# Enigmatisms/cuda-pt

Hardware: AMD Instinct MI355X
Metric: Msamples/sec (whole node), 1080p modern-kitchen (higher is better)
Workload: dtype fp32; 1 GPU; model=modern-kitchen-proc, global_batch=32, seq_len=2073600, width=1920, height=1080, renderer=pt, n_prims=131444, parallelism=dp1 (sample-split, RCCL all-reduce)

## Files before the change

csrc/bind.cpp:

```cpp
#include <pybind11/pybind11.h>
#include <pybind11/numpy.h>
#include <pybind11/stl.h>
#include <algorithm>
#include <cstring>
#include <stdexcept>

#include "core/scene_view.h"
#include "core/integrator.h"
#include "cpu/bvh_build.h"
#include "hip/kernels.h"
#include "hip/lds_plan.h"

namespace py = pybind11;
using namespace hippt;

namespace hippt {
void render_cpu(const SceneView& sv, float* accum, float* var,
                int spp0, int nspp, uint32_t seed, int renderer, int n_threads,
                int y0, int y1, const uint8_t* spp_map, float* aux);
void render_lt_cpu(const SceneView& sv, float* accum, int spp0, int nspp, uint32_t seed,
                   int spec_constraint, float caustic_scaling, int n_threads);
}

namespace {

using farr = py::array_t<float, py::array::c_style | py::array::forcecast>;
using iarr = py::array_t<int32_t, py::array::c_style | py::array::forcecast>;
using uarr = py::array_t<uint32_t, py::array::c_style | py::array::forcecast>;

#define HIP_OK(expr)                                                                   \
    do {                                                                               \
        int _e = (expr);                                                               \
        if (_e != 0) throw std::runtime_error(std::string("HIP error ") +              \
                                              std::to_string(_e) + " at " #expr);      \
    } while (0)

Vec3 to_vec3(const std::vector<float>& v) { return {v[0], v[1], v[2]}; }

int super_cell_voxels() {
    static const int SUP = [] {
        const char* e = getenv("HIPPT_SUPER_N");
        int v = e ? atoi(e) : 16;
        return v < 2 ? 2 : (v > 64 ? 64 : v);
    }();
    return SUP;
}

inline void super_splat(std::vector<float>& sup, const MediumParams& m, int SUP,
                        int ix, int iy, int iz, float v) {
    int cx0 = std::max(0, (ix - 1) / SUP), cx1 = std::min(m.sx - 1, (ix + 1) / SUP);
    int cy0 = std::max(0, (iy - 1) / SUP), cy1 = std::min(m.sy - 1, (iy + 1) / SUP);
    int cz0 = std::max(0, (iz - 1) / SUP), cz1 = std::min(m.sz - 1, (iz + 1) / SUP);
    for (int cz = cz0; cz <= cz1; ++cz)
        for (int cy = cy0; cy <= cy1; ++cy)
            for (int cx = cx0; cx <= cx1; ++cx) {
                float& s = sup[(size_t(cz) * m.sy + cy) * m.sx + cx];
                s = fmaxf(s, v);
            }
}

int bvh4_tree_depth(const BVH4Node* nodes, int n) {
    if (n <= 0) return 0;
    std::vector<std::pair<int, int>> stk{{0, 1}};
    int maxd = 1;
    while (!stk.empty()) {
        auto [idx, d] = stk.back();
        stk.pop_back();
        maxd = std::max(maxd, d);
        const BVH4Node& nd = nodes[idx];
        for (int c = 0; c < 4; ++c)
            if (nd.child[c] >= 0 && !(nd.child[c] == 0 && nd.cnt[c] == 0))
                stk.push_back({nd.child[c], d + 1});
    }
    return maxd;
}

static std::vector<uint64_t> host_lds_slots(int lds_n);

struct SceneHolder {
    farr np_prims, np_attrs, np_nodes, np_nodes4, np_nodes8;
    uarr np_prim_obj;
    iarr np_objs;
    std::vector<BsdfParams> bsdfs;
    std::vector<EmitterParams> emitters;
    std::vector<PhaseParams> phases;
    std::vector<MediumParams> media;
    std::vector<farr> media_density, media_temp;
    std::vector<std::vector<float>> media_super;
    std::vector<std::vector<int32_t>> media_bricks;
    std::vector<int> media_nbricks;
    std::vector<farr> tex_data;
    std::vector<TexView> tex_host;
    std::vector<int> emitter_prims;
    std::vector<float> emitter_cdf;
    std::vector<float> env_rows_h, env_cols_h;
    int env_w = 0, env_h = 0;
    std::vector<float> emitter_sel_h;
    Camera cam{};
    MaxDepthParams md{};
    int env_emitter = -1;
    int cam_medium = -1;

    bool has_dev = false;
    int device_id = 0;
    std::vector<void*> dev_bufs;
    std::vector<TexView> tex_dev;
    std::vector<MediumParams> media_dev;
    void* dev_bsdfs = nullptr;
    void* dev_emitters = nullptr;
    void* dev_media = nullptr;

    SceneView host_sv{};
    SceneView dev_sv{};
    WfState* wf = nullptr;

    ~SceneHolder() { release(); }

    void release() {
        if (wf) { wf_destroy(wf); wf = nullptr; }
        for (void* p : dev_bufs) dev_free(p);
        dev_bufs.clear();
        has_dev = false;
    }

    void set_geometry(farr prims, farr attrs, uarr prim_obj, farr nodes, farr nodes4,
                      farr nodes8) {
        if (prims.ndim() != 2 || prims.shape(1) != 12) throw std::runtime_error("prims must be (n,12)");
        if (attrs.ndim() != 2 || attrs.shape(1) != 16) throw std::runtime_error("attrs must be (n,16)");
        if (nodes.ndim() != 2 || nodes.shape(1) != 8) throw std::runtime_error("nodes must be (m,8)");
        if (nodes4.ndim() == 2 && nodes4.shape(0) > 0 && nodes4.shape(1) != 32)
            throw std::runtime_error("nodes4 must be (m,32)");
        np_prims = std::move(prims);
        np_attrs = std::move(attrs);
        np_prim_obj = std::move(prim_obj);
        np_nodes = std::move(nodes);
        np_nodes4 = std::move(nodes4);
        if (nodes8.ndim() == 2 && nodes8.shape(0) > 0 && nodes8.shape(1) != 64)
            throw std::runtime_error("nodes8 must be (m,64)");
        np_nodes8 = std::move(nodes8);
        bvh4_depth = np_nodes4.ndim() == 2 && np_nodes4.shape(0) > 0
            ? bvh4_tree_depth((const BVH4Node*)np_nodes4.data(), (int)np_nodes4.shape(0))
            : 0;
        nodes4q = np_nodes4.ndim() == 2 && np_nodes4.shape(0) > 0
            ? quantize_bvh4((const BVH4Node*)np_nodes4.data(), (int)np_nodes4.shape(0))
            : std::vector<BVH4NodeQ>();
        nodes4t = np_nodes4.ndim() == 2 && np_nodes4.shape(0) > 0
            ? tag_bvh4((const BVH4Node*)np_nodes4.data(), (int)np_nodes4.shape(0))
            : std::vector<BVH4NodeT>();
        const Prim* pr = (const Prim*)np_prims.data();
        const uint32_t* po = np_prim_obj.data();
        int n = (int)np_prims.shape(0);
        AABB sb;
        for (int i = 0; i < n; ++i) {
            if (po[i] & PRIM_SPHERE_BIT) {
                Vec3 c = pr[i].v0.xyz();
                float rad = pr[i].v0.w;
                sb.grow(c - Vec3(rad)); sb.grow(c + Vec3(rad));
            } else {
                Vec3 v0 = pr[i].v0.xyz();
                sb.grow(v0);
                sb.grow(v0 + pr[i].e1.xyz());
                sb.grow(v0 + pr[i].e2.xyz());
            }
        }
        Vec3 c = (sb.lo + sb.hi) * 0.5f;
        float rad = n > 0 ? (sb.hi - sb.lo).length() * 0.5f : 1.f;
        scene_bound = Vec4(c, rad);
        tri_only = 1;
        for (int i = 0; i < n; ++i)
            if (po[i] & PRIM_SPHERE_BIT) { tri_only = 0; break; }
    }

    int bvh4_depth = 0;
    Vec4 scene_bound{0.f, 0.f, 0.f, 1.f};
    int cache_nodes = 0;
    int tri_only = 0;
    std::vector<BVH4NodeQ> nodes4q;
    std::vector<BVH4NodeT> nodes4t;

    void set_cache_level(int level) {
        cache_nodes = level > 0 ? (1 << (level > 12 ? 12 : level)) : 0;
    }

    void set_objects(iarr objs) {
        if (objs.ndim() != 2 || objs.shape(1) != 8) throw std::runtime_error("objs must be (n,8)");
        np_objs = std::move(objs);
    }

    int add_bsdf(int type, std::vector<float> kd, std::vector<float> ks, std::vector<float> kg,
                 float ior, float extra0, float extra1, std::vector<int> tex) {
        BsdfParams b = BsdfParams::make(type);
        b.kd = Vec4(kd[0], kd[1], kd[2], kd.size() > 3 ? kd[3] : 0.f);
        b.ks = Vec4(ks[0], ks[1], ks[2], ks.size() > 3 ? ks[3] : 0.f);
        b.kg = Vec4(kg[0], kg[1], kg[2], kg.size() > 3 ? kg[3] : 0.f);
        b.ior = ior; b.extra0 = extra0; b.extra1 = extra1;
        for (size_t i = 0; i < tex.size() && i < 8; ++i) b.tex[i] = (int16_t)tex[i];
        bsdfs.push_back(b);
        return (int)bsdfs.size() - 1;
    }

    void update_bsdf(int i, int type, std::vector<float> kd, std::vector<float> ks,
                     std::vector<float> kg, float ior, float extra0, float extra1,
                     std::vector<int> tex) {
        if (i < 0 || i >= (int)bsdfs.size()) throw std::runtime_error("bad bsdf index");
        BsdfParams b = BsdfParams::make(type);
        b.kd = Vec4(kd[0], kd[1], kd[2], kd.size() > 3 ? kd[3] : 0.f);
        b.ks = Vec4(ks[0], ks[1], ks[2], ks.size() > 3 ? ks[3] : 0.f);
        b.kg = Vec4(kg[0], kg[1], kg[2], kg.size() > 3 ? kg[3] : 0.f);
        b.ior = ior; b.extra0 = extra0; b.extra1 = extra1;
        for (size_t k = 0; k < tex.size() && k < 8; ++k) b.tex[k] = (int16_t)tex[k];
        bsdfs[i] = b;
        if (has_dev && dev_bsdfs)
            HIP_OK(dev_upload((char*)dev_bsdfs + sizeof(BsdfParams) * i, &bsdfs[i], sizeof(BsdfParams)));
    }

    int add_emitter(int type, std::vector<float> emission, float scale, std::vector<float> aux,
                    int obj_id, int tex_id, int prim_base, int prim_cnt, float inv_area) {
        EmitterParams e{};
        e.emission = Vec4(emission[0], emission[1], emission[2], scale);
        e.aux = Vec4(aux[0], aux[1], aux[2], aux.size() > 3 ? aux[3] : 0.f);
        e.type = type; e.obj_id = obj_id; e.tex_id = tex_id;
        e.prim_base = prim_base; e.prim_cnt = prim_cnt; e.inv_area = inv_area;
        emitters.push_back(e);
        if (type == EM_ENVMAP) env_emitter = (int)emitters.size() - 1;
        return (int)emitters.size() - 1;
    }

    void update_emitter(int i, std::vector<float> emission, float scale, std::vector<float> aux) {
        if (i < 0 || i >= (int)emitters.size()) throw std::runtime_error("bad emitter index");
        emitters[i].emission = Vec4(emission[0], emission[1], emission[2], scale);
        emitters[i].aux = Vec4(aux[0], aux[1], aux[2], aux.size() > 3 ? aux[3] : 0.f);
        if (has_dev && dev_emitters)
            HIP_OK(dev_upload((char*)dev_emitters + sizeof(EmitterParams) * i, &emitters[i],
                              sizeof(EmitterParams)));
    }

    void set_emitter_prims(iarr eprims, farr ecdf) {
        emitter_prims.assign(eprims.data(), eprims.data() + eprims.size());
        emitter_cdf.assign(ecdf.data(), ecdf.data() + ecdf.size());
    }

    void set_emitter_sel(farr cdf) {
        emitter_sel_h.assign(cdf.data(), cdf.data() + cdf.size());
    }

    void set_env_cdf(farr rows, farr cols) {
        if (cols.ndim() != 2) throw std::runtime_error("env cols must be (h,w)");
        env_h = (int)cols.shape(0);
        env_w = (int)cols.shape(1);
        env_rows_h.assign(rows.data(), rows.data() + rows.size());
        env_cols_h.assign(cols.data(), cols.data() + cols.size());
        if ((int)env_rows_h.size() != env_h) throw std::runtime_error("env rows/cols mismatch");
    }

    int add_phase(int type, float g1, float g2, float wmix) {
        phases.push_back({type, g1, g2, wmix});
        return (int)phases.size() - 1;
    }

    int add_medium(int type, std::vector<float> sigma_a, std::vector<float> sigma_s,
                   int phase_id, std::vector<float> grid_lo, std::vector<float> grid_hi,
                   py::object density, py::object temperature,
                   float scale, float emission_scale, float temp_scale) {
        MediumParams m{};
        m.sigma_a = Vec4(sigma_a[0], sigma_a[1], sigma_a[2], 0.f);
        m.sigma_s = Vec4(sigma_s[0], sigma_s[1], sigma_s[2], 0.f);
        m.type = type; m.phase_id = phase_id;
        m.scale = scale; m.emission_scale = emission_scale; m.temp_scale = temp_scale;
        m.density = nullptr; m.temperature = nullptr;
        m.super = nullptr;
        m.nx = m.ny = m.nz = 0;
        m.sx = m.sy = m.sz = 0;
        if (type == MED_GRID) {
            farr d = density.cast<farr>();
            if (d.ndim() != 3) throw std::runtime_error("density must be (nz,ny,nx)");
            media_density.push_back(d);
            m.nz = (int)d.shape(0); m.ny = (int)d.shape(1); m.nx = (int)d.shape(2);
            m.density = media_density.back().data();
            float mx = 0.f; double sum = 0.0;
            const float* dd = m.density;
            size_t n = (size_t)m.nx * m.ny * m.nz;
            for (size_t i = 0; i < n; ++i) { mx = fmaxf(mx, dd[i]); sum += dd[i]; }
            m.majorant = mx * scale;
            m.avg_density = (float)(sum / std::max<size_t>(n, 1)) * scale;
            const int SUP = super_cell_voxels();
            if (getenv("HIPPT_NO_SUPER")) {
                m.sx = m.sy = m.sz = 0;
                m.super = nullptr;
                goto super_done;
            }
            m.sx = (m.nx + SUP - 1) / SUP;
            m.sy = (m.ny + SUP - 1) / SUP;
            m.sz = (m.nz + SUP - 1) / SUP;
            {
            std::vector<float> sup((size_t)m.sx * m.sy * m.sz, 0.f);
            for (int iz = 0; iz < m.nz; ++iz)
                for (int iy = 0; iy < m.ny; ++iy)
                    for (int ix = 0; ix < m.nx; ++ix) {
                        float v = dd[(size_t(iz) * m.ny + iy) * m.nx + ix];
                        if (v <= 0.f) continue;
                        super_splat(sup, m, SUP, ix, iy, iz, v);
                    }
            media_super.push_back(std::move(sup));
            m.super = media_super.back().data();
            }
            super_done:;
            Vec3 lo = to_vec3(grid_lo), hi = to_vec3(grid_hi);
            m.grid_lo = Vec4(lo, 0.f);
            Vec3 ext = hi - lo;
            m.grid_inv_extent = Vec4(1.f / ext.x, 1.f / ext.y, 1.f / ext.z, 0.f);
            if (!temperature.is_none()) {
                farr t = temperature.cast<farr>();
                media_temp.push_back(t);
                m.temperature = media_temp.back().data();
            }
        }
        media.push_back(m);
        media_nbricks.push_back(-1);
        return (int)media.size() - 1;
    }

    int add_medium_sparse(std::vector<float> sigma_a, std::vector<float> sigma_s,
                          int phase_id, std::vector<float> grid_lo, std::vector<float> grid_hi,
                          std::vector<int> shape, iarr coords, farr density,
                          py::object temperature,
                          float scale, float emission_scale, float temp_scale) {
        MediumParams m{};
        m.sigma_a = Vec4(sigma_a[0], sigma_a[1], sigma_a[2], 0.f);
        m.sigma_s = Vec4(sigma_s[0], sigma_s[1], sigma_s[2], 0.f);
        m.type = MED_GRID; m.phase_id = phase_id;
        m.scale = scale; m.emission_scale = emission_scale; m.temp_scale = temp_scale;
        if (shape.size() != 3 || shape[0] <= 0 || shape[1] <= 0 || shape[2] <= 0)
            throw std::runtime_error("sparse grid shape must be three positive dims (nz,ny,nx)");
        m.nz = shape[0]; m.ny = shape[1]; m.nx = shape[2];
        m.bnx = (m.nx + 7) / 8; m.bny = (m.ny + 7) / 8; m.bnz = (m.nz + 7) / 8;
        if (coords.ndim() != 2 || coords.shape(1) != 3)
            throw std::runtime_error("brick coords must be (n,3)");
        const size_t nb = (size_t)coords.shape(0);
        if ((size_t)density.size() != nb * 512)
            throw std::runtime_error("density bricks must hold 512 floats per brick coord");
        farr temp;
        if (!temperature.is_none()) {
            temp = temperature.cast<farr>();
            if ((size_t)temp.size() != nb * 512)
                throw std::runtime_error("temperature bricks must hold 512 floats per brick coord");
        }
        const size_t cells = (size_t)m.bnx * m.bny * m.bnz;
        if (cells > (size_t)INT32_MAX) throw std::runtime_error("brick table too large");
        std::vector<int32_t> table(cells, -1);
        const int32_t* cc = coords.data();
        for (size_t b = 0; b < nb; ++b) {
            int bz = cc[3 * b], by = cc[3 * b + 1], bx = cc[3 * b + 2];
            if (bz < 0 || bz >= m.bnz || by < 0 || by >= m.bny || bx < 0 || bx >= m.bnx)
                throw std::runtime_error("brick coord outside the brick table");
            int32_t& cell = table[(size_t(bz) * m.bny + by) * m.bnx + bx];
            if (cell >= 0) throw std::runtime_error("duplicate brick coord");
            cell = (int32_t)b;
        }
        const float* pool = density.data();
        float mx = 0.f; double sum = 0.0;
        for (size_t i = 0; i < nb * 512; ++i) mx = fmaxf(mx, pool[i]);
        std::vector<int32_t> row;
        for (int bz = 0; bz < m.bnz; ++bz)
            for (int z = 0; z < 8 && bz * 8 + z < m.nz; ++z)
                for (int by = 0; by < m.bny; ++by) {
                    row.clear();
                    const int32_t* trow = &table[(size_t(bz) * m.bny + by) * m.bnx];
                    for (int bx = 0; bx < m.bnx; ++bx)
                        if (trow[bx] >= 0) row.push_back(trow[bx]);
                    if (row.empty()) continue;
                    for (int y = 0; y < 8 && by * 8 + y < m.ny; ++y)
                        for (int32_t b : row) {
                            const float* v = pool + size_t(b) * 512 + (z << 6 | y << 3);
                            for (int x = 0; x < 8; ++x) sum += v[x];
                        }
                }
        const size_t n = (size_t)m.nx * m.ny * m.nz;
        m.majorant = mx * scale;
        m.avg_density = (float)(sum / std::max<size_t>(n, 1)) * scale;
        if (!getenv("HIPPT_NO_SUPER")) {
            const int SUP = super_cell_voxels();
            m.sx = (m.nx + SUP - 1) / SUP;
            m.sy = (m.ny + SUP - 1) / SUP;
            m.sz = (m.nz + SUP - 1) / SUP;
            std::vector<float> sup((size_t)m.sx * m.sy * m.sz, 0.f);
            for (size_t b = 0; b < nb; ++b) {
                int z0 = cc[3 * b] * 8, y0 = cc[3 * b + 1] * 8, x0 = cc[3 * b + 2] * 8;
                const float* v = pool + b * 512;
                for (int z = 0; z < 8 && z0 + z < m.nz; ++z)
                    for (int y = 0; y < 8 && y0 + y < m.ny; ++y)
                        for (int x = 0; x < 8 && x0 + x < m.nx; ++x) {
                            float d = v[z << 6 | y << 3 | x];
                            if (d <= 0.f) continue;
                            super_splat(sup, m, SUP, x0 + x, y0 + y, z0 + z, d);
                        }
            }
            media_super.push_back(std::move(sup));
            m.super = media_super.back().data();
        }
        Vec3 lo = to_vec3(grid_lo), hi = to_vec3(grid_hi);
        m.grid_lo = Vec4(lo, 0.f);
        Vec3 ext = hi - lo;
        m.grid_inv_extent = Vec4(1.f / ext.x, 1.f / ext.y, 1.f / ext.z, 0.f);
        media_bricks.push_back(std::move(table));
        m.bricks = media_bricks.back().data();
        if (nb > 0) {
            media_density.push_back(density);
            m.density = media_density.back().data();
            if (!temperature.is_none()) {
                media_temp.push_back(temp);
                m.temperature = media_temp.back().data();
            }
        }
        media.push_back(m);
        media_nbricks.push_back((int)nb);
        return (int)media.size() - 1;
    }

    py::tuple medium_super(int i) {
        if (i < 0 || i >= (int)media.size()) throw std::runtime_error("bad medium index");
        const MediumParams& m = media[i];
        farr out({(py::ssize_t)(m.super ? m.sz : 0), (py::ssize_t)m.sy, (py::ssize_t)m.sx});
        if (m.super) std::memcpy(out.mutable_data(), m.super, sizeof(float) * out.size());
        return py::make_tuple(out, m.majorant, m.avg_density);
    }

    py::list media_info() {
        py::list out;
        for (size_t i = 0; i < media.size(); ++i) {
            const MediumParams& m = media[i];
            py::dict d;
            size_t vox = (size_t)m.nx * m.ny * m.nz;
            size_t pools = (m.density ? 1 : 0) + (m.temperature ? 1 : 0);
            size_t bytes = 4 * (size_t)m.sx * m.sy * m.sz * (m.super ? 1 : 0);
            if (m.type != MED_GRID) {
                d["layout"] = "homogeneous";
                d["shape"] = py::none();
                d["n_bricks"] = 0;
                d["occupancy"] = 0.0;
            } else if (m.bricks) {
                size_t cells = (size_t)m.bnx * m.bny * m.bnz;
                size_t nb = (size_t)media_nbricks[i];
                d["layout"] = "bricks";
                d["shape"] = py::make_tuple(m.nz, m.ny, m.nx);
                d["n_bricks"] = nb;
                d["occupancy"] = (double)nb / (double)cells;
                bytes += 4 * cells + 2048 * nb * pools;
            } else {
                d["layout"] = "dense";
                d["shape"] = py::make_tuple(m.nz, m.ny, m.nx);
                d["n_bricks"] = 0;
                d["occupancy"] = 1.0;
                bytes += 4 * vox * pools;
            }
            d["bytes_host"] = bytes;
            d["bytes_device"] = has_dev ? bytes : (size_t)0;
            d["bytes_dense_equiv"] = 4 * vox;
            out.append(d);
        }
        return out;
    }

    void update_medium(int i, std::vector<float> sigma_a, std::vector<float> sigma_s,
                       float scale, float emission_scale) {
        if (i < 0 || i >= (int)media.size()) throw std::runtime_error("bad medium index");
        MediumParams& m = media[i];
        float old_scale = m.scale;
        m.sigma_a = Vec4(sigma_a[0], sigma_a[1], sigma_a[2], 0.f);
        m.sigma_s = Vec4(sigma_s[0], sigma_s[1], sigma_s[2], 0.f);
        if (m.type == MED_GRID && old_scale > 0.f) {
            m.majorant *= scale / old_scale;
            m.avg_density *= scale / old_scale;
        }
        m.scale = scale; m.emission_scale = emission_scale;
        if (has_dev && dev_media) {
            MediumParams md2 = media_dev[i];
            md2.sigma_a = m.sigma_a; md2.sigma_s = m.sigma_s;
            md2.scale = m.scale; md2.majorant = m.majorant;
            md2.avg_density = m.avg_density; md2.emission_scale = m.emission_scale;
            media_dev[i] = md2;
            HIP_OK(dev_upload((char*)dev_media + sizeof(MediumParams) * i, &media_dev[i],
                              sizeof(MediumParams)));
        }
    }

    int add_texture(farr rgba) {
        if (rgba.ndim() != 3 || rgba.shape(2) != 4) throw std::runtime_error("texture must be (h,w,4)");
        tex_data.push_back(std::move(rgba));
        const farr& t = tex_data.back();
        TexView v{};
        v.tex_obj = 0;
        v.data = t.data();
        v.w = (int)t.shape(1);
        v.h = (int)t.shape(0);
        tex_host.push_back(v);
        return (int)tex_host.size() - 1;
    }

    void set_camera(std::vector<float> pos, std::vector<float> R_rows, float focal,
                    int w, int h, float aperture, float focal_dist, int ortho, float ortho_scale) {
        cam.pos = to_vec3(pos);
        cam.R = Mat3({R_rows[0], R_rows[1], R_rows[2]},
                     {R_rows[3], R_rows[4], R_rows[5]},
                     {R_rows[6], R_rows[7], R_rows[8]});
        cam.focal = focal; cam.w = w; cam.h = h;
        cam.aperture = aperture; cam.focal_dist = focal_dist;
        cam.ortho = ortho; cam.ortho_scale = ortho_scale;
    }

    void set_depths(int max_depth, int max_diffuse, int max_specular, int max_transmit,
                    int max_volume, float min_time, float max_time, int use_tof,
                    float radiance_clamp = 0.f) {
        md = {max_depth, max_diffuse, max_specular, max_transmit, max_volume,
              min_time, max_time, use_tof, radiance_clamp};
    }

    void fill_common(SceneView& sv) {
        sv.n_nodes = (int)np_nodes.shape(0) - 1;
        sv.n_nodes4 = np_nodes4.ndim() == 2 ? (int)np_nodes4.shape(0) : 0;
        sv.n_nodes8 = np_nodes8.ndim() == 2 ? (int)np_nodes8.shape(0) : 0;
        sv.n_prims = (int)np_prims.shape(0);
        sv.n_objs = np_objs.ndim() == 2 ? (int)np_objs.shape(0) : 0;
        sv.n_bsdfs = (int)bsdfs.size();
        sv.n_emitters = (int)emitters.size();
        sv.n_textures = (int)tex_host.size();
        sv.n_media = (int)media.size();
        sv.env_emitter = env_emitter;
        sv.env_w = env_w;
        sv.env_h = env_h;
        sv.cam_medium = cam_medium;
        sv.media_bricks = 0;
        for (const MediumParams& m : media) if (m.bricks) sv.media_bricks = 1;
        sv.cam = cam;
        sv.md = md;
        sv.bvh4_depth = bvh4_depth;
        sv.scene_bound = scene_bound;
        sv.cache_nodes = cache_nodes;
        sv.tri_only = tri_only;
    }

    void finalize() {
        fill_common(host_sv);
        host_sv.nodes = (const BVHNode*)np_nodes.data();
        host_sv.nodes4 = host_sv.n_nodes4 > 0 ? (const BVH4Node*)np_nodes4.data() : nullptr;
        host_sv.nodes4q = nodes4q.empty() ? nullptr : nodes4q.data();
        host_sv.nodes4t = nodes4t.empty() ? nullptr : nodes4t.data();
        host_sv.nodes8 = host_sv.n_nodes8 > 0 ? (const BVH8Node*)np_nodes8.data() : nullptr;
        host_sv.prims = (const Prim*)np_prims.data();
        host_sv.attrs = (const PrimAttr*)np_attrs.data();
        host_sv.prim_obj = np_prim_obj.data();
        host_sv.objs = (const ObjInfo*)np_objs.data();
        host_sv.bsdfs = bsdfs.data();
        host_sv.emitters = emitters.data();
        host_sv.emitter_prims = emitter_prims.data();
        host_sv.emitter_cdf = emitter_cdf.data();
        host_sv.env_rows = env_rows_h.empty() ? nullptr : env_rows_h.data();
        host_sv.env_cols = env_cols_h.empty() ? nullptr : env_cols_h.data();
        host_sv.emitter_sel_cdf = emitter_sel_h.empty() ? nullptr : emitter_sel_h.data();
        host_sv.textures = tex_host.data();
        host_sv.media = media.data();
        host_sv.phases = phases.data();
    }

    template <typename T>
    T* upload_vec(const T* src, size_t count) {
        if (count == 0) return nullptr;
        void* p = nullptr;
        HIP_OK(dev_malloc(&p, sizeof(T) * count));
        dev_bufs.push_back(p);
        HIP_OK(dev_upload(p, src, sizeof(T) * count));
        return (T*)p;
    }

    void upload(int device) {
        release();
        device_id = device;
        HIP_OK(dev_set_device(device));
        finalize();
        fill_common(dev_sv);
        dev_sv.nodes = upload_vec((const BVHNode*)np_nodes.data(), np_nodes.shape(0));
        dev_sv.nodes4 = dev_sv.n_nodes4 > 0
            ? upload_vec((const BVH4Node*)np_nodes4.data(), np_nodes4.shape(0)) : nullptr;
        dev_sv.nodes4q = nodes4q.empty() ? nullptr
            : upload_vec(nodes4q.data(), nodes4q.size());
        dev_sv.nodes4t = nodes4t.empty() ? nullptr
            : upload_vec(nodes4t.data(), nodes4t.size());
        dev_sv.nodes8 = dev_sv.n_nodes8 > 0
            ? upload_vec((const BVH8Node*)np_nodes8.data(), np_nodes8.shape(0)) : nullptr;
        dev_sv.prims = upload_vec((const Prim*)np_prims.data(), np_prims.shape(0));
        dev_sv.attrs = upload_vec((const PrimAttr*)np_attrs.data(), np_attrs.shape(0));
        dev_sv.prim_obj = upload_vec(np_prim_obj.data(), np_prim_obj.size());
        dev_sv.objs = upload_vec((const ObjInfo*)np_objs.data(), np_objs.shape(0));
        dev_sv.emitter_prims = upload_vec(emitter_prims.data(), emitter_prims.size());
        dev_sv.emitter_cdf = upload_vec(emitter_cdf.data(), emitter_cdf.size());
        dev_sv.env_rows = upload_vec(env_rows_h.data(), env_rows_h.size());
        dev_sv.env_cols = upload_vec(env_cols_h.data(), env_cols_h.size());
        dev_sv.emitter_sel_cdf = upload_vec(emitter_sel_h.data(), emitter_sel_h.size());
        tex_dev.clear();
        for (size_t i = 0; i < tex_host.size(); ++i) {
            TexView v = tex_host[i];
            v.data = upload_vec(tex_data[i].data(), (size_t)v.w * v.h * 4);
            tex_dev.push_back(v);
        }
        dev_sv.textures = upload_vec(tex_dev.data(), tex_dev.size());
        media_dev = media;
        for (size_t i = 0; i < media.size(); ++i) {
            size_t n_vox = media[i].bricks
                ? (size_t)media_nbricks[i] * 512
                : (size_t)media[i].nx * media[i].ny * media[i].nz;
            if (media[i].bricks) {
                size_t cells = (size_t)media[i].bnx * media[i].bny * media[i].bnz;
                media_dev[i].bricks = upload_vec(media[i].bricks, cells);
            }
            if (media[i].density)
                media_dev[i].density = upload_vec(media[i].density, n_vox);
            if (media[i].temperature)
                media_dev[i].temperature = upload_vec(media[i].temperature, n_vox);
            if (media[i].super) {
                size_t n = (size_t)media[i].sx * media[i].sy * media[i].sz;
                media_dev[i].super = upload_vec(media[i].super, n);
            }
        }
        dev_sv.media = upload_vec(media_dev.data(), media_dev.size());
        dev_sv.phases = upload_vec(phases.data(), phases.size());
        dev_sv.bsdfs = upload_vec(bsdfs.data(), bsdfs.size());
        dev_sv.emitters = upload_vec(emitters.data(), emitters.size());
        dev_bsdfs = (void*)dev_sv.bsdfs;
        dev_emitters = (void*)dev_sv.emitters;
        dev_media = (void*)dev_sv.media;
        has_dev = true;
    }

    void render_host(farr accum, py::object var, int spp0, int nspp, uint32_t seed,
                     int renderer, int spec_constraint, float caustic_scaling, int n_threads,
                     int y0 = 0, int y1 = 0, py::object spp_map = py::none(),
                     py::object aux = py::none()) {
        finalize();
        float* vp = nullptr;
        farr var_arr;
        if (!var.is_none()) { var_arr = var.cast<farr>(); vp = var_arr.mutable_data(); }
        float* auxp = nullptr;
        farr aux_arr;
        if (!aux.is_none()) { aux_arr = aux.cast<farr>(); auxp = aux_arr.mutable_data(); }
        const uint8_t* smp = nullptr;
        py::array_t<uint8_t, py::array::c_style | py::array::forcecast> smp_arr;
        if (!spp_map.is_none()) {
            smp_arr = spp_map.cast<py::array_t<uint8_t, py::array::c_style | py::array::forcecast>>();
            smp = smp_arr.data();
        }
        py::gil_scoped_release rel;
        if (renderer == R_LIGHT_TRACE)
            render_lt_cpu(host_sv, accum.mutable_data(), spp0, nspp, seed,
                          spec_constraint, caustic_scaling, n_threads);
        else
            render_cpu(host_sv, accum.mutable_data(), vp, spp0, nspp, seed, renderer, n_threads,
                       y0, y1, smp, auxp);
    }

    void render_device(uintptr_t accum_ptr, uintptr_t var_ptr, int spp0, int nspp,
                       uint32_t seed, int renderer, int spec_constraint,
                       float caustic_scaling, uintptr_t stream, int y0 = 0, int y1 = 0,
                       uintptr_t spp_map_ptr = 0, uintptr_t aux_ptr = 0) {
        if (!has_dev) throw std::runtime_error("scene not uploaded to device");
        dev_sv.cam = cam;
        dev_sv.md = md;
        dev_sv.cam_medium = cam_medium;
        if (renderer == R_WAVEFRONT_PT) {
            if (!wf) {
                if ((long long)cam.w * cam.h > WF_MAX_PIXELS)
                    throw std::runtime_error(
                        "wavefront renderer: " + std::to_string(cam.w) + "x" +
                        std::to_string(cam.h) + " exceeds the limit of " +
                        std::to_string(WF_MAX_PIXELS) +
                        " pixels (2^24, the 24-bit payload id of a sort entry)");
                wf = wf_create(cam.w, cam.h);
                if (!wf) throw std::runtime_error("wavefront state allocation failed");
            }
            py::gil_scoped_release rel;
            HIP_OK(launch_render_wavefront(wf, dev_sv, (float*)accum_ptr, (float*)var_ptr,
                                           spp0, nspp, seed, 0, (void*)stream));
            return;
        }
        HIP_OK(launch_render(dev_sv, (float*)accum_ptr, (float*)var_ptr, spp0, nspp, seed,
                             renderer, spec_constraint, caustic_scaling, (void*)stream, y0, y1,
                             (const uint8_t*)spp_map_ptr, (float*)aux_ptr));
    }

    py::tuple trace_rays(farr o, farr d, farr tmax, int device, int lds_n, int n_cached) {
        if (o.ndim() != 2 || o.shape(1) != 3 || d.ndim() != 2 || d.shape(1) != 3 ||
            tmax.ndim() != 1 || d.shape(0) != o.shape(0) || tmax.shape(0) != o.shape(0))
            throw std::runtime_error("trace_rays: o (n,3), d (n,3), tmax (n,)");
        const int n = (int)o.shape(0);
        farr t_out(n), u_out(n), v_out(n);
        iarr p_out(n), occ_out(n);
        int plan[2] = {0, 0};
        if (n == 0) return py::make_tuple(t_out, p_out, u_out, v_out, occ_out,
                                          py::make_tuple(0, 0));
        if (device < 0) {
            finalize();
            if (host_sv.n_nodes4 <= 0) throw std::runtime_error("trace_rays: empty scene");
            std::vector<uint64_t> slots = host_lds_slots(lds_n > 0 ? lds_n : 0);
            TravCtx tc;
            if (lds_n > 0) { tc.lds_slot = bvh_host_slot(slots.data()); tc.lds_n = lds_n; }
            plan[0] = tc.lds_n;
            for (int i = 0; i < n; ++i) {
                Ray r;
                r.o = {o.at(i, 0), o.at(i, 1), o.at(i, 2)};
                r.d = {d.at(i, 0), d.at(i, 1), d.at(i, 2)};
                HitRecord h = scene_intersect(host_sv, r, tmax.at(i), tc);
                t_out.mutable_at(i) = h.t;
                u_out.mutable_at(i) = h.u;
                v_out.mutable_at(i) = h.v;
                p_out.mutable_at(i) = h.prim_idx;
                occ_out.mutable_at(i) = scene_occluded(host_sv, r, tmax.at(i), tc) ? 1 : 0;
            }
        } else {
            if (!has_dev) throw std::runtime_error("scene not uploaded to device");
            std::vector<float> ro((size_t)n * 4), rd((size_t)n * 4, 0.f), hit((size_t)n * 4);
            for (int i = 0; i < n; ++i) {
                for (int c = 0; c < 3; ++c) {
                    ro[(size_t)i * 4 + c] = o.at(i, c);
                    rd[(size_t)i * 4 + c] = d.at(i, c);
                }
                ro[(size_t)i * 4 + 3] = tmax.at(i);
            }
            HIP_OK(wf_trace_probe(dev_sv, ro.data(), rd.data(), n, lds_n, n_cached,
                                  hit.data(), occ_out.mutable_data(), plan));
            for (int i = 0; i < n; ++i) {
                t_out.mutable_at(i) = hit[(size_t)i * 4 + 0];
                u_out.mutable_at(i) = hit[(size_t)i * 4 + 1];
                v_out.mutable_at(i) = hit[(size_t)i * 4 + 2];
                int32_t pi;
                std::memcpy(&pi, &hit[(size_t)i * 4 + 3], 4);
                p_out.mutable_at(i) = pi;
            }
        }
        return py::make_tuple(t_out, p_out, u_out, v_out, occ_out,
                              py::make_tuple(plan[0], plan[1]));
    }

    py::dict info() {
        py::dict d;
        d["n_prims"] = np_prims.ndim() == 2 ? (int)np_prims.shape(0) : 0;
        d["n_nodes"] = np_nodes.ndim() == 2 ? (int)np_nodes.shape(0) : 0;
        d["n_bsdfs"] = (int)bsdfs.size();
        d["n_emitters"] = (int)emitters.size();
        d["n_media"] = (int)media.size();
        d["n_textures"] = (int)tex_host.size();
        d["has_dev"] = has_dev;
        return d;
    }
};

py::tuple py_build_bvh(farr prims, uarr prim_obj, int max_leaf, float overlap_w,
                       bool use_sbvh, bool ref_unsplit, float trav_cost) {
    int n = (int)prims.shape(0);
    BVHBuildConfig cfg;
    cfg.max_leaf_prims = max_leaf;
    cfg.overlap_w = overlap_w;
    cfg.use_sbvh = use_sbvh;
    cfg.ref_unsplit = ref_unsplit;
    cfg.trav_cost = trav_cost;
    BVHBuildResult res;
    {
        py::gil_scoped_release rel;
        res = use_sbvh ? build_sbvh((const Prim*)prims.data(), prim_obj.data(), n, cfg)
                       : build_bvh((const Prim*)prims.data(), prim_obj.data(), n, cfg);
    }
    farr nodes({(py::ssize_t)res.nodes.size(), (py::ssize_t)8});
    std::memcpy(nodes.mutable_data(), res.nodes.data(), res.nodes.size() * sizeof(BVHNode));
    iarr order((py::ssize_t)res.prim_order.size());
    std::memcpy(order.mutable_data(), res.prim_order.data(), res.prim_order.size() * sizeof(int));
    py::dict stats;
    stats["n_leaves"] = res.n_leaves;
    stats["max_depth"] = res.max_depth;
    stats["sah_cost"] = res.sah_cost;
    return py::make_tuple(nodes, order, stats);
}

py::tuple py_collapse_bvh8(farr nodes) {
    if (nodes.ndim() != 2 || nodes.shape(1) != 8) throw std::runtime_error("nodes must be (m,8)");
    std::vector<BVHNode> bin((size_t)nodes.shape(0));
    std::memcpy(bin.data(), nodes.data(), bin.size() * sizeof(BVHNode));
    int depth8 = 0;
    std::vector<BVH8Node> n8;
    {
        py::gil_scoped_release rel;
        n8 = collapse_bvh8(bin, &depth8);
    }
    if (7 * depth8 > BVH4_STACK)
        throw std::runtime_error("BVH8 depth exceeds traversal stack bound");
    farr out({(py::ssize_t)n8.size(), (py::ssize_t)64});
    std::memcpy(out.mutable_data(), n8.data(), n8.size() * sizeof(BVH8Node));
    return py::make_tuple(out, depth8);
}

py::tuple py_collapse_bvh4(farr nodes) {
    if (nodes.ndim() != 2 || nodes.shape(1) != 8) throw std::runtime_error("nodes must be (m,8)");
    std::vector<BVHNode> bin((size_t)nodes.shape(0));
    std::memcpy(bin.data(), nodes.data(), bin.size() * sizeof(BVHNode));
    int depth4 = 0;
    std::vector<BVH4Node> n4;
    {
        py::gil_scoped_release rel;
        n4 = collapse_bvh4(bin, &depth4);
    }
    if (3 * depth4 > BVH4_STACK)
        throw std::runtime_error("BVH4 depth exceeds traversal stack bound");
    farr out({(py::ssize_t)n4.size(), (py::ssize_t)32});
    std::memcpy(out.mutable_data(), n4.data(), n4.size() * sizeof(BVH4Node));
    return py::make_tuple(out, depth4);
}

static bool same_hit(const HitRecord& ref, const HitRecord& h) {
    return (h.prim_idx < 0) == (ref.prim_idx < 0) &&
           (ref.prim_idx < 0 || fabsf(h.t - ref.t) <= 1e-5f * fmaxf(1.f, ref.t));
}

static std::vector<uint64_t> host_lds_slots(int lds_n) {
    if (lds_n < 0) throw std::runtime_error("lds_n must be >= 0");
    return std::vector<uint64_t>((size_t)lds_n * BVH4_LDS_STRIDE);
}

int py_bvh4_selftest(farr prims, uarr prim_obj, farr nodes, farr nodes4,
                     farr ray_o, farr ray_d, float tmax, farr nodes8, int lds_n) {
    const BVH8Node* n8p = (nodes8.ndim() == 2 && nodes8.shape(0) > 0)
        ? (const BVH8Node*)nodes8.data() : nullptr;
    int n_nodes = (int)nodes.shape(0);
    const BVHNode* bn = (const BVHNode*)nodes.data();
    const BVH4Node* n4 = (const BVH4Node*)nodes4.data();
    const std::vector<BVH4NodeT> t4v = tag_bvh4(n4, (int)nodes4.shape(0));
    const BVH4NodeT* t4 = t4v.data();
    const Prim* pr = (const Prim*)prims.data();
    const uint32_t* po = prim_obj.data();
    std::vector<uint64_t> slots = host_lds_slots(lds_n);
    LdsSlot lds = bvh_host_slot(lds_n ? slots.data() : nullptr);
    const int lds_half = lds_n / 2;
    LdsSlot lds1 = lds_n ? lds + (size_t)lds_half * BVH4_LDS_STRIDE : nullptr;
    int bad = 0;
    int nr = (int)ray_o.shape(0);
    for (int i = 0; i < nr; ++i) {
        Ray r;
        r.o = {ray_o.at(i, 0), ray_o.at(i, 1), ray_o.at(i, 2)};
        r.d = {ray_d.at(i, 0), ray_d.at(i, 1), ray_d.at(i, 2)};
        HitRecord a = ray_intersect_bvh(bn, n_nodes, pr, po, r, tmax);
        HitRecord b = ray_intersect_bvh4(n4, pr, po, r, tmax, lds, lds_n);
        HitRecord w = ray_intersect_bvh4_ww(t4, pr, po, r, tmax, lds, lds_n);
        if (!same_hit(b, w)) { ++bad; continue; }
        {
            Bvh4Walk wk0, wk1;
            bvh4_walk_init(wk0, r, tmax);
            bvh4_walk_init(wk1, r, tmax);
            bool r0 = true, r1 = true;
            while (r0 || r1) {
                if (r0) r0 = bvh4_walk_step(wk0, t4, pr, po, lds, lds_half);
                if (r1) r1 = bvh4_walk_step(wk1, t4, pr, po, lds1, lds_half);
            }
            if (wk0.rec.prim_idx < 0) wk0.rec.t = MAX_DIST;
            if (wk1.rec.prim_idx < 0) wk1.rec.t = MAX_DIST;
            if (!same_hit(b, wk0.rec) || !same_hit(b, wk1.rec)) { ++bad; continue; }
        }
        if (n8p) {
            HitRecord w8 = ray_intersect_bvh8_ww(n8p, pr, po, r, tmax, lds, lds_n);
            bool occ8 = occlusion_test_bvh8(n8p, pr, po, r, tmax, lds, lds_n);
            bool occ_ref = occlusion_test_bvh4(n4, pr, po, r, tmax, lds, lds_n);
            if (!same_hit(b, w8) || occ8 != occ_ref) { ++bad; continue; }
        }
        bool occ_a = occlusion_test_bvh(bn, n_nodes, pr, po, r, tmax);
        bool occ_b = occlusion_test_bvh4(n4, pr, po, r, tmax, lds, lds_n);
        if (occlusion_test_bvh4_ww(t4, pr, po, r, tmax, lds, lds_n) != occ_b) { ++bad; continue; }
        if (!same_hit(a, b) || occ_a != occ_b) ++bad;
    }
    return bad;
}

int py_bvh4q_selftest(farr prims, uarr prim_obj, farr nodes4,
                      farr ray_o, farr ray_d, float tmax, int lds_n) {
    const BVH4Node* n4 = (const BVH4Node*)nodes4.data();
    int nn = (int)nodes4.shape(0);
    std::vector<BVH4NodeQ> q = quantize_bvh4(n4, nn);
    const std::vector<BVH4NodeT> t4v = tag_bvh4(n4, nn);
    const BVH4NodeT* t4 = t4v.data();
    const Prim* pr = (const Prim*)prims.data();
    const uint32_t* po = prim_obj.data();
    std::vector<uint64_t> slots = host_lds_slots(lds_n);
    LdsSlot lds = bvh_host_slot(lds_n ? slots.data() : nullptr);
    int bad = 0;
    int nr = (int)ray_o.shape(0);
    for (int i = 0; i < nr; ++i) {
        Ray r;
        r.o = {ray_o.at(i, 0), ray_o.at(i, 1), ray_o.at(i, 2)};
        r.d = {ray_d.at(i, 0), ray_d.at(i, 1), ray_d.at(i, 2)};
        HitRecord a = ray_intersect_bvh4_ww(t4, pr, po, r, tmax, lds, lds_n);
        HitRecord b = ray_intersect_bvh4q_ww(q.data(), pr, po, r, tmax, lds, lds_n);
        if (!same_hit(a, b)) { ++bad; continue; }
        bool oa = occlusion_test_bvh4_ww(t4, pr, po, r, tmax, lds, lds_n);
        bool ob = occlusion_test_bvh4q_ww(q.data(), pr, po, r, tmax, lds, lds_n);
        if (oa != ob) ++bad;
    }
    return bad;
}

uarr py_bvh4_tag(farr nodes4) {
    if (nodes4.ndim() != 2 || nodes4.shape(1) != 32) throw std::runtime_error("nodes4 must be (m,32)");
    const std::vector<BVH4NodeT> t4 =
        tag_bvh4((const BVH4Node*)nodes4.data(), (int)nodes4.shape(0));
    uarr out({(py::ssize_t)t4.size(), (py::ssize_t)32});
    std::memcpy(out.mutable_data(), t4.data(), t4.size() * sizeof(BVH4NodeT));
    return out;
}

int py_bvh4_visit_selftest(farr nodes4, farr ray_o, farr ray_d, float tmax) {
    if (nodes4.ndim() != 2 || nodes4.shape(1) != 32) throw std::runtime_error("nodes4 must be (m,32)");
    const BVH4Node* n4 = (const BVH4Node*)nodes4.data();
    const int nn = (int)nodes4.shape(0);
    const std::vector<BVH4NodeT> t4 = tag_bvh4(n4, nn);
    const LdsSlot no_lds = nullptr;
    int bad = 0;
    const int nr = (int)ray_o.shape(0);
    for (int i = 0; i < nr; ++i) {
        Ray r;
        r.o = {ray_o.at(i, 0), ray_o.at(i, 1), ray_o.at(i, 2)};
        r.d = {ray_d.at(i, 0), ray_d.at(i, 1), ray_d.at(i, 2)};
        const Vec3 inv_d = safe_rcp_dir(r.d);
        const Vec3 o_div = r.o * inv_d;
        for (int j = 0; j < nn; ++j) {
            uint64_t sa[4] = {0, 0, 0, 0}, sb[4] = {0, 0, 0, 0};
            int spa = 0, spb = 0;
            uint32_t na, nb;
            {
                const BVH4Node nd = n4[j];
                BVH_VISIT_ORDERED(BVH4Node, na, nd, inv_d, o_div, tmax, sa, spa, no_lds, 0)
            }
            {
                const BVH4NodeT nd = t4[j];
                BVH_VISIT_TAGGED4(nb, nd, inv_d, o_div, tmax, sb, spb, no_lds, 0)
            }
            if (na != nb || spa != spb || std::memcmp(sa, sb, sizeof(sa)) != 0) ++bad;
        }
    }
    return bad;
}

int py_bvh4_any_visit_selftest(farr nodes4, farr ray_o, farr ray_d, float tmax) {
    if (nodes4.ndim() != 2 || nodes4.shape(1) != 32) throw std::runtime_error("nodes4 must be (m,32)");
    const BVH4Node* n4 = (const BVH4Node*)nodes4.data();
    const int nn = (int)nodes4.shape(0);
    const std::vector<BVH4NodeT> t4 = tag_bvh4(n4, nn);
    const LdsSlot no_lds = nullptr;
    auto collect = [](uint32_t next, const uint64_t* st, int sp, uint32_t* out, int& n) {
        n = 0;
        if (next != BVH4_NONE_W) out[n++] = next;
        for (int k = 0; k < sp; ++k) {
            if (st[k] >> 32) return false;
            const uint32_t w = (uint32_t)st[k];
            if (w == BVH4_NONE_W || w == BVH4_ANY_MISS_W) return false;
            out[n++] = w;
        }
        std::sort(out, out + n);
        return std::adjacent_find(out, out + n) == out + n;
    };
    int bad = 0;
    const int nr = (int)ray_o.shape(0);
    for (int i = 0; i < nr; ++i) {
        Ray r;
        r.o = {ray_o.at(i, 0), ray_o.at(i, 1), ray_o.at(i, 2)};
        r.d = {ray_d.at(i, 0), ray_d.at(i, 1), ray_d.at(i, 2)};
        const Vec3 inv_d = safe_rcp_dir(r.d);
        const Vec3 o_div = r.o * inv_d;
        for (int j = 0; j < nn; ++j) {
            uint64_t sa[4] = {0, 0, 0, 0}, sb[4] = {0, 0, 0, 0};
            int spa = 0, spb = 0;
            uint32_t na = BVH4_NONE_W, nb = BVH4_NONE_W;
            {
                const BVH4Node nd = n4[j];
                BVH_VISIT_ANY_EACH(BVH4Node, na, nd, inv_d, o_div, tmax, sa, spa, no_lds, 0)
            }
            {
                const BVH4NodeT nd = t4[j];
                BVH_VISIT_ANY4(nb, nd, inv_d, o_div, tmax, sb, spb, no_lds, 0)
            }
            uint32_t wa[4], wb[4];
            int ca, cb;
            const bool oka = collect(na, sa, spa, wa, ca);
            const bool okb = collect(nb, sb, spb, wb, cb);
            const bool shape = (na != BVH4_NONE_W || spa == 0) && (nb != BVH4_NONE_W || spb == 0);
            if (!oka || !okb || !shape || ca != cb || !std::equal(wa, wa + ca, wb)) ++bad;
        }
    }
    return bad;
}

py::tuple py_bvh4_hit(farr prims, uarr prim_obj, farr nodes4,
                      farr ray_o, farr ray_d) {
    const std::vector<BVH4NodeT> t4v =
        tag_bvh4((const BVH4Node*)nodes4.data(), (int)nodes4.shape(0));
    const BVH4NodeT* n4 = t4v.data();
    const Prim* pr = (const Prim*)prims.data();
    const uint32_t* po = prim_obj.data();
    int nr = (int)ray_o.shape(0);
    farr t_out(nr);
    iarr p_out(nr);
    for (int i = 0; i < nr; ++i) {
        Ray r;
        r.o = {ray_o.at(i, 0), ray_o.at(i, 1), ray_o.at(i, 2)};
        r.d = {ray_d.at(i, 0), ray_d.at(i, 1), ray_d.at(i, 2)};
        HitRecord h = ray_intersect_bvh4_ww(n4, pr, po, r, MAX_DIST);
        t_out.mutable_at(i) = h.t;
        p_out.mutable_at(i) = h.prim_idx;
    }
    return py::make_tuple(t_out, p_out);
}

py::tuple py_bsdf_check(SceneHolder& h, int i, float cos_o, uint32_t seed, int n) {
    if (i < 0 || i >= (int)h.bsdfs.size()) throw std::runtime_error("bad bsdf index");
    h.finalize();
    const BsdfParams& b = h.bsdfs[i];
    Interaction it{};
    it.shading_n = Vec3(0.f, 0.f, 1.f);
    float so = sqrtf(fmaxf(0.f, 1.f - cos_o * cos_o));
    Vec3 wo(so, 0.f, cos_o);
    Sampler sp(911u, seed);
    Vec3 A(0.f), B(0.f);
    double Cp = 0.0;
    for (int k = 0; k < n; ++k) {
        BsdfSample s = bsdf_sample(b, wo, it, sp, h.host_sv.textures);
        if (s.pdf > 0.f) A += s.weight;
        Vec2 u = sp.next2f();
        float z = u.x, r = sqrtf(fmaxf(0.f, 1.f - z * z)), phi = 2.f * PI * u.y;
        Vec3 wi(r * cosf(phi), r * sinf(phi), z);
        B += bsdf_eval(b, wo, wi, it, h.host_sv.textures);
        Cp += (double)bsdf_pdf(b, wo, wi, it, h.host_sv.textures);
    }
    float inv_n = 1.f / (float)n;
    Vec3 a = A * inv_n;
    Vec3 bb = B * (2.f * PI * inv_n);
    double c = Cp * 2.0 * PI * inv_n;
    return py::make_tuple(py::make_tuple(a.x, a.y, a.z),
                          py::make_tuple(bb.x, bb.y, bb.z), c);
}

py::tuple py_env_check(SceneHolder& h, uint32_t seed, int n) {
    h.finalize();
    if (h.env_emitter < 0) throw std::runtime_error("no envmap emitter");
    const EmitterParams& e = h.emitters[h.env_emitter];
    EmitterGeom g = h.host_sv.emitter_geom();
    Sampler sp(417u, seed);
    Vec3 A(0.f), B(0.f);
    Vec3 sp_n(0.f, 0.f, 1.f), sp_pos(0.f);
    for (int k = 0; k < n; ++k) {
        EmitterSampleRec r = emitter_sample(e, g, sp_pos, sp_n, sp);
        if (r.pdf > 0.f) {
            Vec3 dir = (r.pos - sp_pos).normalized();
            if (dir.z > 0.f) A += r.radiance / r.pdf;
        }
        Vec2 u = sp.next2f();
        float z = u.x, rr = sqrtf(fmaxf(0.f, 1.f - z * z)), phi = 2.f * PI * u.y;
        Vec3 wi(rr * cosf(phi), rr * sinf(phi), z);
        B += envmap_eval(e, wi, h.host_sv.textures);
    }
    float inv_n = 1.f / (float)n;
    Vec3 a = A * inv_n;
    Vec3 b = B * (2.f * PI * inv_n);
    return py::make_tuple(py::make_tuple(a.x, a.y, a.z),
                          py::make_tuple(b.x, b.y, b.z));
}

}

PYBIND11_MODULE(_C, m) {
    m.doc() = "hippt native core: MI355X path tracing kernels + scene runtime";

    py::class_<SceneHolder>(m, "Scene")
        .def(py::init<>())
        .def("set_geometry", &SceneHolder::set_geometry)
        .def("set_objects", &SceneHolder::set_objects)
        .def("add_bsdf", &SceneHolder::add_bsdf)
        .def("update_bsdf", &SceneHolder::update_bsdf)
        .def("add_emitter", &SceneHolder::add_emitter)
        .def("update_emitter", &SceneHolder::update_emitter)
        .def("set_emitter_prims", &SceneHolder::set_emitter_prims)
        .def("set_env_cdf", &SceneHolder::set_env_cdf)
        .def("set_emitter_sel", &SceneHolder::set_emitter_sel)
        .def("add_phase", &SceneHolder::add_phase)
        .def("add_medium", &SceneHolder::add_medium)
        .def("add_medium_sparse", &SceneHolder::add_medium_sparse)
        .def("media_info", &SceneHolder::media_info)
        .def("medium_super", &SceneHolder::medium_super)
        .def("update_medium", &SceneHolder::update_medium)
        .def("add_texture", &SceneHolder::add_texture)
        .def("set_camera", &SceneHolder::set_camera)
        .def("set_depths", &SceneHolder::set_depths,
             py::arg("max_depth"), py::arg("max_diffuse"), py::arg("max_specular"),
             py::arg("max_transmit"), py::arg("max_volume"), py::arg("min_time"),
             py::arg("max_time"), py::arg("use_tof"), py::arg("radiance_clamp") = 0.f)
        .def("set_cache_level", &SceneHolder::set_cache_level)
        .def_readwrite("cam_medium", &SceneHolder::cam_medium)
        .def_readwrite("env_emitter", &SceneHolder::env_emitter)
        .def("finalize", &SceneHolder::finalize)
        .def("upload", &SceneHolder::upload)
        .def("release", &SceneHolder::release)
        .def("render_host", &SceneHolder::render_host,
             py::arg("accum"), py::arg("var"), py::arg("spp0"), py::arg("nspp"),
             py::arg("seed"), py::arg("renderer"), py::arg("spec_constraint"),
             py::arg("caustic_scaling"), py::arg("n_threads"),
             py::arg("y0") = 0, py::arg("y1") = 0, py::arg("spp_map") = py::none(),
             py::arg("aux") = py::none())
        .def("render_device", &SceneHolder::render_device,
             py::arg("accum_ptr"), py::arg("var_ptr"), py::arg("spp0"), py::arg("nspp"),
             py::arg("seed"), py::arg("renderer"), py::arg("spec_constraint"),
             py::arg("caustic_scaling"), py::arg("stream"),
             py::arg("y0") = 0, py::arg("y1") = 0, py::arg("spp_map_ptr") = 0,
             py::arg("aux_ptr") = 0)
        .def("trace_rays", &SceneHolder::trace_rays, py::arg("o"), py::arg("d"),
             py::arg("tmax"), py::arg("device"), py::arg("lds_n") = -1,
             py::arg("n_cached") = -1)
        .def("info", &SceneHolder::info);

    m.def("build_bvh", &py_build_bvh, py::arg("prims"), py::arg("prim_obj"),
          py::arg("max_leaf") = 4, py::arg("overlap_w") = 0.f,
          py::arg("use_sbvh") = false, py::arg("ref_unsplit") = true,
          py::arg("trav_cost") = 0.f);
    m.def("collapse_bvh4", &py_collapse_bvh4, py::arg("nodes"));
    m.def("collapse_bvh8", &py_collapse_bvh8, py::arg("nodes"));
    m.def("bvh4_hit", &py_bvh4_hit);
    m.def("bvh4_tag", &py_bvh4_tag, py::arg("nodes4"));
    m.def("bvh4_visit_selftest", &py_bvh4_visit_selftest, py::arg("nodes4"),
          py::arg("ray_o"), py::arg("ray_d"), py::arg("tmax"));
    m.def("bvh4_any_visit_selftest", &py_bvh4_any_visit_selftest, py::arg("nodes4"),
          py::arg("ray_o"), py::arg("ray_d"), py::arg("tmax"));
    m.def("bsdf_check", &py_bsdf_check);
    m.def("env_check", &py_env_check);
    m.def("bvh4q_selftest", &py_bvh4q_selftest,
          py::arg("prims"), py::arg("prim_obj"), py::arg("nodes4"),
          py::arg("ray_o"), py::arg("ray_d"), py::arg("tmax"), py::arg("lds_n") = 0);
    m.def("bvh4_selftest", &py_bvh4_selftest,
          py::arg("prims"), py::arg("prim_obj"), py::arg("nodes"), py::arg("nodes4"),
          py::arg("ray_o"), py::arg("ray_d"), py::arg("tmax"),
          py::arg("nodes8") = farr(), py::arg("lds_n") = 0);

    m.def("wf_sort_probe", [](uarr status, uarr gather, int mode) {
        if (status.ndim() != 1 || gather.ndim() != 1)
            throw std::runtime_error("wf_sort_probe: status (n,), gather (m,) or empty");
        const int n = (int)status.shape(0), m = (int)gather.shape(0);
        uarr out(n);
        int live = -1;
        HIP_OK(wf_sort_probe(status.data(), n, gather.data(), m, mode,
                             out.mutable_data(), &live));
        return py::make_tuple(out, live);
    }, py::arg("status"), py::arg("gather"), py::arg("mode"));
    m.def("lds_plan", [](int occ, bool stack_in_lds, bool scratch_drops_cache, int n_nodes4,
                         int node_bytes, int cache_req, int lds_req) {
        if (n_nodes4 < 0 || node_bytes <= 0) throw std::runtime_error("lds_plan: bad sizes");
        const LdsPlan p = lds_plan(occ, stack_in_lds, scratch_drops_cache, n_nodes4,
                                   node_bytes, cache_req, lds_req);
        return py::make_tuple(p.lds_n, p.n_cached, p.shmem);
    }, py::arg("occ"), py::arg("stack_in_lds"), py::arg("scratch_drops_cache"),
       py::arg("n_nodes4"), py::arg("node_bytes"), py::arg("cache_req"),
       py::arg("lds_req") = -1);
    m.def("dev_synchronize", [] { HIP_OK(dev_synchronize()); });
    m.def("dev_set_device", [](int d) { HIP_OK(dev_set_device(d)); });

    m.def("struct_sizes", [] {
        py::dict d;
        d["BVHNode"] = (int)sizeof(BVHNode);
        d["Prim"] = (int)sizeof(Prim);
        d["PrimAttr"] = (int)sizeof(PrimAttr);
        d["ObjInfo"] = (int)sizeof(ObjInfo);
        d["BsdfParams"] = (int)sizeof(BsdfParams);
        d["EmitterParams"] = (int)sizeof(EmitterParams);
        d["MediumParams"] = (int)sizeof(MediumParams);
        d["PhaseParams"] = (int)sizeof(PhaseParams);
        d["TexView"] = (int)sizeof(TexView);
        d["Camera"] = (int)sizeof(Camera);
        d["SceneView"] = (int)sizeof(SceneView);
        return d;
    });

    m.attr("R_MEGAKERNEL_PT") = (int)R_MEGAKERNEL_PT;
    m.attr("R_WAVEFRONT_PT") = (int)R_WAVEFRONT_PT;
    m.attr("R_VOLUME_PT") = (int)R_VOLUME_PT;
    m.attr("R_LIGHT_TRACE") = (int)R_LIGHT_TRACE;
    m.attr("R_DEPTH") = (int)R_DEPTH;
    m.attr("R_BVH_COST") = (int)R_BVH_COST;
    m.attr("R_MEGAKERNEL_PT_DYN") = (int)R_MEGAKERNEL_PT_DYN;
    m.attr("WAVE_SIZE") = 64;
}
```

csrc/core/emitter.h:

```cpp
#pragma once
#include "geometry.h"
#include "texture.h"
#include "rng.h"
#include "sampling.h"

namespace hippt {

enum EmitterType : int {
    EM_NONE = 0,
    EM_POINT,
    EM_AREA,
    EM_AREA_SPOT,
    EM_ENVMAP,
};

struct alignas(16) EmitterParams {
    Vec4 emission;
    Vec4 aux;
    int32_t type;
    int32_t obj_id;
    int32_t tex_id;
    int32_t prim_base;
    int32_t prim_cnt;
    float inv_area;
    float extra0, extra1;
};

struct EmitterSampleRec {
    Vec3 pos;
    Vec3 normal;
    Vec3 radiance;
    float pdf;
    bool delta;
};

struct EmitterGeom {
    const Prim* prims;
    const PrimAttr* attrs;
    const uint32_t* prim_obj;
    const int* emitter_prims;
    const float* emitter_cdf;
    const TexView* textures;
    const float* env_rows;
    const float* env_cols;
    int env_w, env_h;
    Vec3 scene_center;
    float scene_radius;
};

HD int cdf_find(const float* cdf, int n, float u) {
    int lo = 0, hi = n - 1;
    while (lo < hi) {
        int mid = (lo + hi) >> 1;
        if (cdf[mid] > u) hi = mid;
        else lo = mid + 1;
    }
    return lo;
}

HD Vec3 emitter_radiance_tex(const EmitterParams& e, const TexView* textures, Vec2 uv) {
    Vec3 rad = e.emission.xyz() * e.emission.w;
    if (e.tex_id >= 0) rad *= textures[e.tex_id].sample(uv).xyz();
    return rad;
}

HD Vec3 emitter_eval_le(const EmitterParams& e, const Vec3& light_n, const Vec3& to_viewer,
                        Vec2 uv, const TexView* textures) {
    float c = light_n.dot(to_viewer);
    if (c <= 0.f) return Vec3(0.f);
    if (e.type == EM_AREA_SPOT) {
        if (c < e.aux.w) return Vec3(0.f);
    }
    return emitter_radiance_tex(e, textures, uv);
}

HD Vec3 envmap_eval(const EmitterParams& e, const Vec3& dir, const TexView* textures) {
    Vec3 d = dir;
    float az = e.aux.x, ze = e.aux.y;
    if (az != 0.f || ze != 0.f) {
        Quat q = Quat::angle_axis(-az, Vec3(0.f, 1.f, 0.f)) * Quat::angle_axis(-ze, Vec3(1.f, 0.f, 0.f));
        d = q.rotate(d);
    }
    Vec3 rad = e.emission.xyz() * e.emission.w;
    if (e.tex_id >= 0) rad *= textures[e.tex_id].sample(dir_to_latlong(d)).xyz();
    return rad;
}

HD Vec3 envmap_sample_dir(const EmitterParams& e, const EmitterGeom& g,
                          Sampler& sampler, float& pdf) {
    const int w = g.env_w, h = g.env_h;
    int row = cdf_find(g.env_rows, h, sampler.next1f());
    const float* crow = g.env_cols + (size_t)row * w;
    int col = cdf_find(crow, w, sampler.next1f());
    float pr = g.env_rows[row] - (row ? g.env_rows[row - 1] : 0.f);
    float pc = crow[col] - (col ? crow[col - 1] : 0.f);
    float uu = (col + sampler.next1f()) / w;
    float vv = (row + sampler.next1f()) / h;
    float theta = vv * PI, phi = (uu - 0.5f) * 2.f * PI;
    float st = sinf(theta);
    Vec3 dl(st * sinf(phi), cosf(theta), -st * cosf(phi));
    Vec3 dir = dl;
    float az = e.aux.x, ze = e.aux.y;
    if (az != 0.f || ze != 0.f) {
        Quat qi = Quat::angle_axis(ze, Vec3(1.f, 0.f, 0.f)) *
                  Quat::angle_axis(az, Vec3(0.f, 1.f, 0.f));
        dir = qi.rotate(dl);
    }
    pdf = pr * pc * (float)w * (float)h / (2.f * PI * PI * fmaxf(st, 1e-5f));
    return dir;
}

HD EmitterSampleRec emitter_sample(const EmitterParams& e, const EmitterGeom& g,
                                   const Vec3& sp_pos, const Vec3& sp_n, Sampler& sampler) {
    EmitterSampleRec r{};
    switch (e.type) {
    case EM_POINT: {
        r.pos = e.aux.xyz();
        Vec3 d = r.pos - sp_pos;
        float d2 = fmaxf(d.length2(), 1e-8f);
        r.normal = (sp_pos - r.pos) * (1.f / sqrtf(d2));
        r.radiance = e.emission.xyz() * (e.emission.w / d2);
        r.pdf = 1.f;
        r.delta = true;
        return r;
    }
    case EM_AREA:
    case EM_AREA_SPOT: {
        int cnt = e.prim_cnt;
        if (cnt <= 0) { r.pdf = 0.f; return r; }
        float xi = sampler.next1f();
        const float* cdf = g.emitter_cdf + e.prim_base;
        int lo = 0, hi = cnt - 1;
        while (lo < hi) { int mid = (lo + hi) >> 1; if (cdf[mid] < xi) lo = mid + 1; else hi = mid; }
        int pid = g.emitter_prims[e.prim_base + lo];
        const Prim p = g.prims[pid];
        bool sph = (g.prim_obj[pid] & PRIM_SPHERE_BIT) != 0;
        Vec3 lpos, ln; Vec2 uv{0.f, 0.f};
        if (sph) {
            float pdf_dir;
            Vec3 dir = sample_uniform_sphere(sampler.next2f(), pdf_dir);
            lpos = p.v0.xyz() + dir * p.v0.w;
            ln = dir;
        } else {
            Vec3 bc = sample_triangle_bary(sampler.next2f());
            lpos = p.v0.xyz() + p.e1.xyz() * bc.y + p.e2.xyz() * bc.z;
            const PrimAttr a = g.attrs[pid];
            Vec3 nsum = a.n0.xyz() * bc.x + a.n1.xyz() * bc.y + a.n2.xyz() * bc.z;
            ln = nsum.length2() > 1e-16f ? nsum.normalized()
                                         : p.e1.xyz().cross(p.e2.xyz()).normalized();
            Vec2 uv0{a.n0.w, a.n1.w}, uv1{a.n2.w, a.uvrest.x}, uv2{a.uvrest.y, a.uvrest.z};
            uv = uv0 * bc.x + uv1 * bc.y + uv2 * bc.z;
        }
        Vec3 to_sp = sp_pos - lpos;
        float d2 = fmaxf(to_sp.length2(), 1e-9f);
        float dist = sqrtf(d2);
        Vec3 wo_light = to_sp * (1.f / dist);
        float cos_l = ln.dot(wo_light);
        r.pos = lpos;
        r.normal = ln;
        r.radiance = emitter_eval_le(e, ln, wo_light, uv, g.textures);
        r.pdf = cos_l > 1e-6f ? e.inv_area * d2 / cos_l : 0.f;
        r.delta = false;
        return r;
    }
    case EM_ENVMAP: {
        if (g.env_rows && e.tex_id >= 0) {
            float pdf;
            Vec3 dir = envmap_sample_dir(e, g, sampler, pdf);
            r.pos = sp_pos + dir * ENVMAP_DIST;
            r.normal = -dir;
            r.radiance = envmap_eval(e, dir, g.textures);
            r.pdf = pdf;
            r.delta = false;
            return r;
        }
        float pdf;
        Vec3 nn = sp_n;
        Vec3 local = sample_cosine_hemisphere(sampler.next2f(), pdf);
        Vec3 dir = Frame::from_n(nn).to_world(local);
        r.pos = sp_pos + dir * ENVMAP_DIST;
        r.normal = -dir;
        r.radiance = envmap_eval(e, dir, g.textures);
        r.pdf = pdf;
        r.delta = false;
        return r;
    }
    default:
        r.pdf = 0.f;
        return r;
    }
}

HD float emitter_pdf_hit(const EmitterParams& e, const Vec3& dir, float dist,
                         const Vec3& light_n, const Vec3& sp_n,
                         const EmitterGeom& g) {
    if (e.type == EM_AREA || e.type == EM_AREA_SPOT) {
        float cos_l = light_n.dot(-dir);
        if (cos_l <= 1e-6f) return 0.f;
        return e.inv_area * dist * dist / cos_l;
    }
    if (e.type == EM_ENVMAP) {
        if (g.env_rows && e.tex_id >= 0) {
            Vec3 d = dir;
            float az = e.aux.x, ze = e.aux.y;
            if (az != 0.f || ze != 0.f) {
                Quat q = Quat::angle_axis(-az, Vec3(0.f, 1.f, 0.f)) *
                         Quat::angle_axis(-ze, Vec3(1.f, 0.f, 0.f));
                d = q.rotate(d);
            }
            Vec2 uv = dir_to_latlong(d);
            const int w = g.env_w, h = g.env_h;
            int col = (int)(uv.x * w);
            int row = (int)(uv.y * h);
            col = col < 0 ? 0 : (col >= w ? w - 1 : col);
            row = row < 0 ? 0 : (row >= h ? h - 1 : row);
            const float* crow = g.env_cols + (size_t)row * w;
            float pr = g.env_rows[row] - (row ? g.env_rows[row - 1] : 0.f);
            float pc = crow[col] - (col ? crow[col - 1] : 0.f);
            float st = sinf(uv.y * PI);
            return pr * pc * (float)w * (float)h /
                   (2.f * PI * PI * fmaxf(st, 1e-5f));
        }
        float c = sp_n.dot(dir);
        return c > 0.f ? c * INV_PI : 0.f;
    }
    return 0.f;
}

struct EmitterLeRec {
    Ray ray;
    Vec3 normal;
    Vec3 throughput;
    Vec2 uv;
    bool valid;
};

HD EmitterLeRec emitter_sample_le(const EmitterParams& e, const EmitterGeom& g, Sampler& sampler) {
    EmitterLeRec r{};
    switch (e.type) {
    case EM_POINT: {
        float pdf_dir;
        Vec3 d = sample_uniform_sphere(sampler.next2f(), pdf_dir);
        r.ray = Ray(e.aux.xyz(), d);
        r.normal = d;
        r.throughput = e.emission.xyz() * (e.emission.w / pdf_dir);
        r.valid = true;
        return r;
    }
    case EM_AREA:
    case EM_AREA_SPOT: {
        int cnt = e.prim_cnt;
        if (cnt <= 0) return r;
        float xi = sampler.next1f();
        const float* cdf = g.emitter_cdf + e.prim_base;
        int lo = 0, hi = cnt - 1;
        while (lo < hi) { int mid = (lo + hi) >> 1; if (cdf[mid] < xi) lo = mid + 1; else hi = mid; }
        int pid = g.emitter_prims[e.prim_base + lo];
        const Prim p = g.prims[pid];
        bool sph = (g.prim_obj[pid] & PRIM_SPHERE_BIT) != 0;
        Vec3 lpos, ln; Vec2 uv{0.f, 0.f};
        if (sph) {
            float pdf_sph;
            Vec3 dirn = sample_uniform_sphere(sampler.next2f(), pdf_sph);
            lpos = p.v0.xyz() + dirn * p.v0.w;
            ln = dirn;
        } else {
            Vec3 bc = sample_triangle_bary(sampler.next2f());
            lpos = p.v0.xyz() + p.e1.xyz() * bc.y + p.e2.xyz() * bc.z;
            const PrimAttr a = g.attrs[pid];
            Vec3 nsum = a.n0.xyz() * bc.x + a.n1.xyz() * bc.y + a.n2.xyz() * bc.z;
            ln = nsum.length2() > 1e-16f ? nsum.normalized()
                                         : p.e1.xyz().cross(p.e2.xyz()).normalized();
        }
        float pdf_dir;
        Vec3 local = (e.type == EM_AREA_SPOT)
                         ? sample_uniform_cone(sampler.next2f(), e.aux.w, pdf_dir)
                         : sample_cosine_hemisphere(sampler.next2f(), pdf_dir);
        Vec3 dir = Frame::from_n(ln).to_world(local);
        float cos_l = ln.dot(dir);
        if (cos_l <= 0.f || pdf_dir <= 0.f) return r;
        r.ray = Ray(fmadd(ln, EPSILON, lpos), dir);
        r.normal = ln;
        r.uv = uv;
        Vec3 rad = emitter_radiance_tex(e, g.textures, uv);
        r.throughput = rad * (cos_l / fmaxf(e.inv_area * pdf_dir, 1e-12f));
        r.valid = true;
        return r;
    }
    case EM_ENVMAP: {
        float pdf_dir;
        Vec3 dir;
        if (g.env_rows && e.tex_id >= 0) {
            dir = envmap_sample_dir(e, g, sampler, pdf_dir);
        } else {
            dir = sample_uniform_sphere(sampler.next2f(), pdf_dir);
        }
        if (pdf_dir <= 0.f) return r;
        float R = fmaxf(g.scene_radius, 1e-4f);
        Vec2 u = sampler.next2f();
        float rr = sqrtf(u.x), phi = 2.f * PI * u.y;
        Frame f = Frame::from_n(dir);
        Vec3 offset = f.to_world(Vec3(rr * cosf(phi), rr * sinf(phi), 0.f)) * R;
        Vec3 origin = g.scene_center + dir * (2.f * R) + offset;
        r.ray = Ray(origin, -dir);
        r.normal = -dir;
        r.throughput = envmap_eval(e, dir, g.textures) * (PI * R * R / pdf_dir);
        r.valid = true;
        return r;
    }
    default:
        return r;
    }
}

}
```

csrc/core/hd.h:

```cpp
#pragma once

#include <cstdint>
#include <cmath>
#include <cstring>

#if defined(__HIPCC__)
#include <hip/hip_runtime.h>
#define HD __host__ __device__ __forceinline__
#define HOSTFN __host__ inline
#else
#define HD inline
#define HOSTFN inline
#endif

#if defined(__HIP_DEVICE_COMPILE__)
#define HIPPT_ON_DEVICE 1
#else
#define HIPPT_ON_DEVICE 0
#endif

namespace hippt {

constexpr float EPSILON      = 1e-3f;
constexpr float THP_EPS      = 1e-5f;
constexpr float MAX_DIST     = 1e7f;
constexpr float ENVMAP_DIST  = 5e3f;
constexpr float PI           = 3.14159265358979323846f;
constexpr float INV_PI       = 0.31830988618379067154f;
constexpr float TWO_PI       = 6.28318530717958647692f;
constexpr uint32_t WAVE_SIZE = 64;

HD float f_as_u(float f, uint32_t* u) {
    std::memcpy(u, &f, 4); return f;
}
HD uint32_t float_as_uint(float f) { uint32_t u; std::memcpy(&u, &f, 4); return u; }
HD float uint_as_float(uint32_t u) { float f; std::memcpy(&f, &u, 4); return f; }
HD int32_t float_as_int(float f) { int32_t i; std::memcpy(&i, &f, 4); return i; }
HD float int_as_float(int32_t i) { float f; std::memcpy(&f, &i, 4); return f; }

template <typename T> HD T clampv(T v, T lo, T hi) { return v < lo ? lo : (v > hi ? hi : v); }
HD float saturatef(float v) { return clampv(v, 0.f, 1.f); }

template <typename T> HD T select(bool c, T a, T b) { return c ? a : b; }

}
```

csrc/core/integrator.h:

```cpp
#pragma once
#include "scene_view.h"

namespace hippt {

struct PathStats {
    int n_diffuse = 0, n_specular = 0, n_transmit = 0, n_volume = 0;
};

HD bool tof_in_range(const MaxDepthParams& md, float time) {
    return !md.use_tof || (time >= md.min_time && time <= md.max_time);
}

struct PathState {
    Ray ray;
    Vec3 L, thp;
    float prev_pdf;
    bool prev_delta;
    Vec3 prev_n;
    float path_time;
    PathStats st;
    int b, iter;
    Vec3 aov_n, aov_alb;
    float aov_t;
    float lambda;

    HD void reset(const Ray& r) {
        ray = r;
        L = Vec3(0.f); thp = Vec3(1.f);
        prev_pdf = 0.f;
        prev_delta = true;
        prev_n = Vec3(0.f, 0.f, 1.f);
        path_time = 0.f;
        st = PathStats();
        b = 0; iter = 0;
        aov_n = Vec3(0.f); aov_alb = Vec3(0.f); aov_t = 0.f;
        lambda = 0.f;
    }
};

HD Vec3 bsdf_aov_albedo(const BsdfParams& b, Vec2 uv, const TexView* textures) {
    switch (b.type) {
    case BSDF_LAMBERTIAN:
    case BSDF_PLASTIC:
    case BSDF_PLASTIC_FORWARD:
        return bsdf_albedo(b, uv, textures);
    case BSDF_GGX_CONDUCTOR:
        return tex_or(textures, b.tex[TEX_SPECULAR], uv, b.kg.xyz());
    case BSDF_SPECULAR:
    case BSDF_TRANSLUCENT:
    case BSDF_DISPERSION:
        return tex_or(textures, b.tex[TEX_SPECULAR], uv, b.ks.xyz());
    default:
        return Vec3(1.f);
    }
}

HD bool path_shade_hit(const SceneView& sv, PathState& ps, Sampler& sp, TravCtx tc,
                       const HitRecord& hit) {
    Ray& ray = ps.ray;
    Vec3& L = ps.L;
    Vec3& thp = ps.thp;
    float& prev_pdf = ps.prev_pdf;
    bool& prev_delta = ps.prev_delta;
    Vec3& prev_n = ps.prev_n;
    float& path_time = ps.path_time;
    PathStats& st = ps.st;
    int& b = ps.b;
    {
        if (hit.prim_idx < 0) {
            if (sv.env_emitter >= 0) {
                const EmitterParams& env = sv.emitters[sv.env_emitter];
                Vec3 le = envmap_eval(env, ray.d, sv.textures);
                float w = 1.f;
                if (!prev_delta) {
                    float light_pdf = emitter_pdf_hit(env, ray.d, ENVMAP_DIST, ray.d, prev_n, sv.emitter_geom()) *
                                      emitter_sel_pdf(sv, sv.env_emitter);
                    w = mis_weight(prev_pdf, light_pdf);
                }
                if (tof_in_range(sv.md, path_time + ENVMAP_DIST)) L += thp * le * w;
            }
            return true;
        }
        Vec3 pos = ray.at(hit.t);
        path_time += hit.t;
        uint32_t po = sv.prim_obj[hit.prim_idx];
        bool is_sphere = (po & PRIM_SPHERE_BIT) != 0;
        const ObjInfo& obj = sv.objs[po & PRIM_OBJ_MASK];
        const Prim prim = sv.prims[hit.prim_idx];
        Interaction it = get_interaction(prim, sv.attrs[hit.prim_idx], is_sphere, pos, hit.u, hit.v);
        const BsdfParams& bsdf = sv.bsdfs[obj.bsdf_id];
        if (bsdf.tex[TEX_NORMAL] >= 0)
            it.shading_n = apply_normal_map(sv.textures, bsdf.tex[TEX_NORMAL], it.uv, it.shading_n);
        if (ps.iter == 1) {
            ps.aov_n = it.shading_n;
            ps.aov_t = hit.t;
            ps.aov_alb = bsdf_aov_albedo(bsdf, it.uv, sv.textures);
        }

        if (obj.emitter_id >= 0) {
            const EmitterParams& em = sv.emitters[obj.emitter_id];
            Vec3 le = emitter_eval_le(em, it.shading_n, -ray.d, it.uv, sv.textures);
            if (!le.is_zero()) {
                float w = 1.f;
                if (!prev_delta) {
                    float light_pdf = emitter_pdf_hit(em, ray.d, hit.t, it.shading_n, prev_n, sv.emitter_geom()) *
                                   emitter_sel_pdf(sv, obj.emitter_id);
                    w = mis_weight(prev_pdf, light_pdf);
                }
                if (tof_in_range(sv.md, path_time)) L += thp * le * w;
            }
        }

        if (!bsdf_is_delta(bsdf) && sv.n_emitters > 0) {
            float epdf;
            int ei = pick_emitter(sv, sp, epdf);
            EmitterSampleRec er = emitter_sample(sv.emitters[ei], sv.emitter_geom(), pos, it.shading_n, sp);
            if (er.pdf > 0.f && !er.radiance.is_zero()) {
                Vec3 to_l = er.pos - pos;
                float dist = to_l.length();
                Vec3 wi = to_l * (1.f / fmaxf(dist, 1e-9f));
                Vec3 f = bsdf_eval(bsdf, -ray.d, wi, it, sv.textures);
                if (!f.is_zero()) {
                    Ray sh_ray(fmadd(wi, EPSILON, pos), wi);
                    float sh_max = (sv.emitters[ei].type == EM_ENVMAP ? ENVMAP_DIST : dist) - 2.f * EPSILON;
                    if (!scene_occluded(sv, sh_ray, sh_max, tc)) {
                        float light_pdf = er.pdf * epdf;
                        float w = er.delta ? 1.f
                                           : mis_weight(light_pdf, bsdf_pdf(bsdf, -ray.d, wi, it, sv.textures));
                        if (tof_in_range(sv.md, path_time + dist))
                            L += thp * f * er.radiance * (w / light_pdf);
                    }
                }
            }
        }

        BsdfSample bs = bsdf_sample(bsdf, -ray.d, it, sp, sv.textures, &ps.lambda);
        if (bs.pdf <= 0.f || bs.weight.is_zero()) return true;
        if (bs.weight.has_nan() || bs.wi.has_nan()) return true;
        thp *= bs.weight;

        if (!(bs.lobe & LOBE_NULL)) {
            if (bs.lobe & LOBE_DIFFUSE)  { if (++st.n_diffuse  > sv.md.max_diffuse)  return true; }
            if (bs.lobe & LOBE_SPECULAR) { if (++st.n_specular > sv.md.max_specular) return true; }
            if (bs.lobe & LOBE_TRANSMIT) { if (++st.n_transmit > sv.md.max_transmit) return true; }
            ++b;
        }
        prev_delta = (bs.lobe & LOBE_DELTA) != 0;
        prev_pdf = bs.pdf;
        prev_n = it.shading_n;
        ray = Ray(fmadd(bs.wi, EPSILON, pos), bs.wi);

        if (b > 1) {
            float p = clampv(thp.max_elem(), 0.f, 1.f);
            if (p < 0.1f) {
                if (sp.next1f() >= p * 10.f) return true;
                thp *= (1.f / (p * 10.f));
            }
        }
    }
    return false;
}

HD bool path_step(const SceneView& sv, PathState& ps, Sampler& sp, TravCtx tc) {
    if (ps.iter >= sv.md.max_depth * 2 + 8 || ps.b >= sv.md.max_depth) return true;
    ++ps.iter;
    HitRecord hit = scene_intersect(sv, ps.ray, MAX_DIST, tc);
    return path_shade_hit(sv, ps, sp, tc, hit);
}

HD Vec3 clamp_radiance(const SceneView& sv, Vec3 L) {
    float c = sv.md.radiance_clamp;
    if (c > 0.f) L = L.minv(Vec3(c));
    return L;
}

HD Vec3 trace_path(const SceneView& sv, Ray ray, Sampler& sp, TravCtx tc = {}) {
    PathState ps;
    ps.reset(ray);
    while (!path_step(sv, ps, sp, tc)) {}
    if (ps.L.has_nan()) return Vec3(0.f);
    return clamp_radiance(sv, ps.L);
}

HD float trace_depth(const SceneView& sv, const Ray& ray, TravCtx tc = {}) {
    HitRecord hit = scene_intersect(sv, ray, MAX_DIST, tc);
    return hit.prim_idx >= 0 ? hit.t : 0.f;
}

HD Vec2 trace_bvh_cost(const SceneView& sv, const Ray& ray) {
    return bvh4_cost(sv.nodes4, sv.prims, sv.prim_obj, ray);
}
HD Vec2 trace_bvh_cost_binary(const SceneView& sv, const Ray& ray) {
    Vec3 inv_d = safe_rcp_dir(ray.d);
    Vec3 o_div = ray.o * inv_d;
    float best_t = MAX_DIST;
    int node_visits = 0, prim_tests = 0;
    int i = 0;
    while (i < sv.n_nodes) {
        const BVHNode nd = sv.nodes[i];
        ++node_visits;
        float t_near;
        bool hit_box = nd.aabb().intersect(inv_d, o_div, best_t, t_near);
        int cnt = float_as_int(nd.hi.w);
        if (hit_box) {
            if (cnt > 0) {
                int base = nd.prim_base();
                for (int k = 0; k < cnt; ++k) {
                    ++prim_tests;
                    float u, v;
                    bool sph = (sv.prim_obj[base + k] & PRIM_SPHERE_BIT) != 0;
                    float t = intersect_prim(sv.prims[base + k], sph, ray, u, v);
                    if (t > EPSILON && t < best_t) best_t = t;
                }
            }
            ++i;
        } else {
            i = cnt > 0 ? i + 1 : -cnt;
        }
    }
    return {(float)node_visits, (float)prim_tests};
}

}
```

csrc/core/light_tracer.h:

```cpp
#pragma once
#include "scene_view.h"
#include "integrator.h"

namespace hippt {

template <typename SPLAT_FN>
HD void trace_light_path_impl(const SceneView& sv, Sampler& sp, SPLAT_FN&& splat, TravCtx tc,
                              int spec_constraint, float caustic_scaling) {
    if (sv.n_emitters <= 0) return;
    float epdf;
    int ei = pick_emitter(sv, sp, epdf);
    const EmitterParams& em = sv.emitters[ei];
    EmitterLeRec le = emitter_sample_le(em, sv.emitter_geom(), sp);
    if (!le.valid) return;

    const float inv_npix = 1.f / (float(sv.cam.w) * float(sv.cam.h));
    float path_lambda = 0.f;
    const Vec3 cam_fwd = sv.cam.R * Vec3(0.f, 0.f, 1.f);

    auto connect = [&](const Vec3& pos, const Vec3& f_times_cos, int n_spec) {
        if (f_times_cos.is_zero()) return;
        if (n_spec < spec_constraint) return;
        int px, py;
        if (!sv.cam.get_splat_pixel(pos, px, py)) return;
        Vec3 to_cam = sv.cam.pos - pos;
        float d2 = fmaxf(to_cam.length2(), 1e-9f);
        float dist = sqrtf(d2);
        Vec3 wc = to_cam * (1.f / dist);
        float cos_c = fmaxf(1e-6f, (-wc).dot(cam_fwd));
        Ray sh(fmadd(wc, EPSILON, pos), wc);
        if (scene_occluded(sv, sh, dist - 2.f * EPSILON, tc))
            return;
        float W = sv.cam.focal * sv.cam.focal / (cos_c * cos_c * cos_c);
        Vec3 val = f_times_cos * (W / d2) * inv_npix * caustic_scaling;
        if (!val.has_nan()) splat(py * sv.cam.w + px, val);
    };

    if (em.type == EM_AREA || em.type == EM_AREA_SPOT) {
        Vec3 to_cam = sv.cam.pos - le.ray.o;
        float dist = to_cam.length();
        Vec3 wc = to_cam * (1.f / fmaxf(dist, 1e-9f));
        Vec3 l_emit = emitter_eval_le(em, le.normal, wc, le.uv, sv.textures);
        float cos_l = le.normal.dot(wc);
        if (cos_l > 0.f && !l_emit.is_zero())
            connect(le.ray.o, l_emit * (cos_l / fmaxf(em.inv_area * epdf, 1e-12f)), 0);
    }

    Vec3 thp = le.throughput / epdf;
    Ray ray = le.ray;
    int n_spec = 0;
    PathStats st;
    int b = 0;
    for (int iter = 0; iter < sv.md.max_depth * 2 + 8 && b < sv.md.max_depth; ++iter) {
        HitRecord hit = scene_intersect(sv, ray, MAX_DIST, tc);
        if (hit.prim_idx < 0) break;
        Vec3 pos = ray.at(hit.t);
        uint32_t po = sv.prim_obj[hit.prim_idx];
        bool is_sphere = (po & PRIM_SPHERE_BIT) != 0;
        const ObjInfo& obj = sv.objs[po & PRIM_OBJ_MASK];
        const Prim prim = sv.prims[hit.prim_idx];
        Interaction it = get_interaction(prim, sv.attrs[hit.prim_idx], is_sphere, pos, hit.u, hit.v);
        const BsdfParams& bsdf = sv.bsdfs[obj.bsdf_id];

        if (!bsdf_is_delta(bsdf)) {
            Vec3 to_cam = (sv.cam.pos - pos).normalized();
            Vec3 f = bsdf_eval(bsdf, -ray.d, to_cam, it, sv.textures);
            connect(pos, thp * f, n_spec);
        }

        BsdfSample bs = bsdf_sample(bsdf, -ray.d, it, sp, sv.textures, &path_lambda);
        if (bs.pdf <= 0.f || bs.weight.is_zero() || bs.weight.has_nan() || bs.wi.has_nan()) break;
        thp *= bs.weight;
        if (bs.lobe & (LOBE_SPECULAR | LOBE_TRANSMIT)) ++n_spec;
        if (!(bs.lobe & LOBE_NULL)) {
            if (bs.lobe & LOBE_DIFFUSE)  { if (++st.n_diffuse  > sv.md.max_diffuse)  break; }
            if (bs.lobe & LOBE_SPECULAR) { if (++st.n_specular > sv.md.max_specular) break; }
            if (bs.lobe & LOBE_TRANSMIT) { if (++st.n_transmit > sv.md.max_transmit) break; }
            ++b;
        }
        ray = Ray(fmadd(bs.wi, EPSILON, pos), bs.wi);
        if (b > 1) {
            float p = clampv(thp.max_elem(), 0.f, 1.f);
            if (p < 0.1f) {
                if (sp.next1f() >= p * 10.f) break;
                thp *= (1.f / (p * 10.f));
            }
        }
    }
}

inline void trace_light_path(const SceneView& sv, Sampler& sp, float* img, int w, int h,
                             int spec_constraint, float caustic_scaling) {
    trace_light_path_impl(sv, sp, [&](int pix, Vec3 v) {
        img[pix * 4 + 0] += v.x;
        img[pix * 4 + 1] += v.y;
        img[pix * 4 + 2] += v.z;
    }, TravCtx{}, spec_constraint, caustic_scaling);
}

}
```

csrc/core/scene_view.h:

```cpp
#pragma once
#include "bvh.h"
#include "bvh4.h"
#include "bvh8.h"
#include "bsdf.h"
#include "emitter.h"
#include "camera.h"
#include "medium.h"

namespace hippt {

struct alignas(16) ObjInfo {
    int32_t prim_base;
    int32_t prim_cnt;
    int32_t bsdf_id;
    int32_t emitter_id;
    int32_t medium_in;
    int32_t medium_out;
    uint32_t flags;
    float inv_area;
};
constexpr uint32_t OBJ_CULLABLE = 1u;

struct MaxDepthParams {
    int max_depth;
    int max_diffuse;
    int max_specular;
    int max_transmit;
    int max_volume;
    float min_time;
    float max_time;
    int use_tof;
    float radiance_clamp;
};

struct SceneView {
    const BVHNode* nodes; int n_nodes;
    const BVH4Node* nodes4; int n_nodes4;
    const BVH4NodeT* nodes4t;
    const BVH4NodeQ* nodes4q;
    const BVH8Node* nodes8; int n_nodes8;
    const Prim* prims; const PrimAttr* attrs; const uint32_t* prim_obj; int n_prims;
    const ObjInfo* objs; int n_objs;
    const BsdfParams* bsdfs; int n_bsdfs;
    const EmitterParams* emitters; int n_emitters;
    const int* emitter_prims;
    const float* emitter_cdf;
    const float* env_rows; const float* env_cols; int env_w, env_h;
    const float* emitter_sel_cdf;
    const TexView* textures; int n_textures;
    int env_emitter;
    const MediumParams* media; int n_media;
    const PhaseParams* phases;
    int cam_medium;
    int media_bricks;
    Camera cam;
    MaxDepthParams md;
    int bvh4_depth;
    Vec4 scene_bound;
    int tri_only;
    int cache_nodes;

    HD EmitterGeom emitter_geom() const {
        return {prims, attrs, prim_obj, emitter_prims, emitter_cdf, textures,
                env_rows, env_cols, env_w, env_h,
                scene_bound.xyz(), scene_bound.w};
    }
    HD uint32_t obj_of_prim(int pid) const { return prim_obj[pid] & PRIM_OBJ_MASK; }
    HD bool prim_is_sphere(int pid) const { return (prim_obj[pid] & PRIM_SPHERE_BIT) != 0; }
};

HD float emitter_sel_pdf(const SceneView& sv, int i) {
    if (sv.n_emitters <= 0) return 0.f;
    if (!sv.emitter_sel_cdf) return 1.f / sv.n_emitters;
    return sv.emitter_sel_cdf[i] - (i ? sv.emitter_sel_cdf[i - 1] : 0.f);
}

HD int pick_emitter(const SceneView& sv, Sampler& sp, float& pdf) {
    if (sv.n_emitters <= 0) { pdf = 0.f; return -1; }
    if (sv.emitter_sel_cdf) {
        int i = cdf_find(sv.emitter_sel_cdf, sv.n_emitters, sp.next1f());
        pdf = emitter_sel_pdf(sv, i);
        return i;
    }
    int i = (int)(sp.next1f() * sv.n_emitters);
    i = i >= sv.n_emitters ? sv.n_emitters - 1 : i;
    pdf = 1.f / sv.n_emitters;
    return i;
}

#ifdef HIPPT_QBVH
using TravNode = BVH4NodeQ;
#else
using TravNode = BVH4NodeT;
#endif

struct TravCtx {
    LdsSlot lds_slot = nullptr;
    int lds_n = 0;
    const TravNode* top_cache = nullptr;
    int n_cached = 0;
};

HD const TravNode* trav_nodes(const SceneView& sv) {
#ifdef HIPPT_QBVH
    return sv.nodes4q;
#else
    return sv.nodes4t;
#endif
}

HD HitRecord scene_intersect(const SceneView& sv, const Ray& ray,
                             float tmax = MAX_DIST, TravCtx tc = {}) {
#ifdef HIPPT_QBVH
    return ray_intersect_bvh4q_ww(sv.nodes4q, sv.prims, sv.prim_obj, ray, tmax,
                                  tc.lds_slot, tc.lds_n, tc.top_cache, tc.n_cached);
#else
    return ray_intersect_bvh4_ww(sv.nodes4t, sv.prims, sv.prim_obj, ray, tmax,
                                 tc.lds_slot, tc.lds_n, tc.top_cache, tc.n_cached,
                                 sv.tri_only != 0);
#endif
}
HD bool scene_occluded(const SceneView& sv, const Ray& ray, float tmax,
                       TravCtx tc = {}) {
#ifdef HIPPT_QBVH
    return occlusion_test_bvh4q_ww(sv.nodes4q, sv.prims, sv.prim_obj, ray, tmax,
                                   tc.lds_slot, tc.lds_n, tc.top_cache, tc.n_cached);
#else
    return occlusion_test_bvh4_ww(sv.nodes4t, sv.prims, sv.prim_obj, ray, tmax,
                                  tc.lds_slot, tc.lds_n, tc.top_cache, tc.n_cached,
                                  sv.tri_only != 0);
#endif
}

}
```

csrc/hip/kernels.h:

```cpp
#pragma once
#include <cstdint>
#include "../core/scene_view.h"

namespace hippt {

enum RendererKind : int {
    R_MEGAKERNEL_PT = 0,
    R_WAVEFRONT_PT = 1,
    R_VOLUME_PT = 2,
    R_LIGHT_TRACE = 3,
    R_DEPTH = 4,
    R_BVH_COST = 5,
    R_MEGAKERNEL_PT_DYN = 6,
};

int launch_render(const SceneView& sv, float* accum, float* var,
                  int spp0, int nspp, uint32_t seed, int renderer,
                  int spec_constraint, float caustic_scaling,
                  void* stream, int y0 = 0, int y1 = 0,
                  const uint8_t* spp_map = nullptr,
                  float* aux = nullptr);

struct WfState;
constexpr int WF_MAX_PIXELS = 1 << 24;
WfState* wf_create(int width, int height);
void wf_destroy(WfState* s);
int launch_render_wavefront(WfState* st, const SceneView& sv, float* accum, float* var,
                            int spp0, int nspp, uint32_t seed, int sort_mode, void* stream);

int wf_sort_probe(const uint32_t* status, int n, const uint32_t* gather, int m,
                  int mode, uint32_t* out, int* live);
int wf_trace_probe(const SceneView& sv, const float* ray_o_tmax, const float* ray_d,
                   int n, int lds_n, int n_cached, float* hit_out, int* occ_out,
                   int* plan_out);

int dev_malloc(void** p, size_t n);
int dev_free(void* p);
int dev_upload(void* dst, const void* src, size_t n);
int dev_memset(void* dst, int v, size_t n, void* stream);
int dev_synchronize();
int dev_set_device(int d);

}
```

csrc/hip/wf_kernels.hip:

```cpp
#include <hip/hip_runtime.h>
#include "kernels.h"
#include "trav_lds.h"
#include "../core/integrator.h"

namespace hippt {

constexpr int WF_BLOCK = 256;
constexpr int SORT_BLOCK = 256;
constexpr int SORT_ITEMS = 16;
constexpr uint32_t DEAD = 0x80u;

struct WfState {
    int w = 0, h = 0, n = 0;
    int nb_sort = 0;
    float4* ray_o = nullptr;
    float4* ray_d = nullptr;
    float4* thp = nullptr;
    float4* L = nullptr;
    float4* hit = nullptr;
    float4* prevn = nullptr;
    unsigned long long* rng = nullptr;
    uint32_t* status = nullptr;
    uint32_t* order = nullptr;
    uint32_t* order2 = nullptr;
    uint32_t* hist = nullptr;
    int* live_dev = nullptr;
    int* live_host = nullptr;
    float4* sh_od = nullptr;
    float4* sh_dir = nullptr;
    float4* sh_val = nullptr;
    int* sh_cnt = nullptr;
};

__device__ __forceinline__ uint32_t pack_counts(int d, int s, int t, int b) {
    return (uint32_t)(d | (s << 8) | (t << 16) | (b << 24));
}

template <int MINW>
__global__ __launch_bounds__(256)
__attribute__((amdgpu_waves_per_eu(MINW, MINW)))
void k_wf_raygen(SceneView sv, WfState st, int spp_idx, uint32_t seed, int lds_n,
                 int n_cached) {
    extern __shared__ uint64_t s_stk[];
    TravCtx tc = trav_lds_ctx(sv, s_stk, threadIdx.x, lds_n, n_cached);
    int i = blockIdx.x * blockDim.x + threadIdx.x;
    if (i >= st.n) return;
    int px = i % st.w, py = i / st.w;
    Sampler sp(uint32_t(i), uint32_t(spp_idx) * SEED_SCALER + seed);
    Ray ray = sv.cam.gen_ray(px, py, sp, spp_idx);
    HitRecord hit = scene_intersect(sv, ray, MAX_DIST, tc);
    st.ray_o[i] = make_float4(ray.o.x, ray.o.y, ray.o.z, 0.f);
    st.ray_d[i] = make_float4(ray.d.x, ray.d.y, ray.d.z, 0.f);
    st.thp[i] = make_float4(1.f, 1.f, 1.f, uint_as_float(1u));
    st.L[i] = make_float4(0.f, 0.f, 0.f, 0.f);
    st.hit[i] = make_float4(hit.t, hit.u, hit.v, int_as_float(hit.prim_idx));
    st.prevn[i] = make_float4(0.f, 0.f, 1.f, uint_as_float(pack_counts(0, 0, 0, 0)));
    st.rng[i] = sp.state;
    uint32_t status;
    if (hit.prim_idx < 0) {
        status = DEAD;
        if (sv.env_emitter >= 0) {
            Vec3 le = envmap_eval(sv.emitters[sv.env_emitter], ray.d, sv.textures);
            st.L[i] = make_float4(le.x, le.y, le.z, 0.f);
        }
    } else {
        uint32_t oi = sv.prim_obj[hit.prim_idx] & PRIM_OBJ_MASK;
        status = (uint32_t)(sv.objs[oi].bsdf_id & 0x3F);
    }
    st.status[i] = (status << 24) | (uint32_t)i;
}

__device__ inline uint32_t sort_key(uint32_t status, int mode) {
    uint32_t b = status >> 24;
    return mode ? (b >= DEAD ? (uint32_t)DEAD : 0u) : b;
}

__device__ __forceinline__ uint32_t sort_load(const uint32_t* in, const uint32_t* gather, int i) {
    return gather ? in[gather[i] & 0x00FFFFFFu] : in[i];
}

__global__ __launch_bounds__(SORT_BLOCK)
void k_sort_hist(const uint32_t* __restrict__ in, const uint32_t* __restrict__ gather,
                 int n, uint32_t* __restrict__ hist, int mode) {
    __shared__ uint32_t lh[256];
    for (int t = threadIdx.x; t < 256; t += blockDim.x) lh[t] = 0;
    __syncthreads();
    int base = blockIdx.x * SORT_BLOCK * SORT_ITEMS;
    for (int k = 0; k < SORT_ITEMS; ++k) {
        int i = base + k * SORT_BLOCK + threadIdx.x;
        if (i < n) atomicAdd(&lh[sort_key(sort_load(in, gather, i), mode)], 1u);
    }
    __syncthreads();
    for (int t = threadIdx.x; t < 256; t += blockDim.x)
        if (lh[t]) atomicAdd(&hist[t], lh[t]);
}

__global__ __launch_bounds__(256)
void k_sort_scan(uint32_t* __restrict__ hist, int* __restrict__ live_out) {
    __shared__ uint32_t base[256];
    int b = threadIdx.x;
    uint32_t x = hist[b];
    base[b] = x;
    __syncthreads();
    for (int off = 1; off < 256; off <<= 1) {
        uint32_t v = (b >= off) ? base[b - off] : 0;
        __syncthreads();
        base[b] += v;
        __syncthreads();
    }
    uint32_t excl = base[b] - x;
    hist[b] = excl;
    if (b == (int)DEAD - 1 && live_out) *live_out = (int)base[b];
}

__global__ __launch_bounds__(SORT_BLOCK)
void k_sort_scatter(const uint32_t* __restrict__ in, const uint32_t* __restrict__ gather,
                    int n, uint32_t* __restrict__ hist, uint32_t* __restrict__ out, int mode) {
    __shared__ uint32_t lbase[256];
    __shared__ uint32_t lcnt[256];
    for (int t = threadIdx.x; t < 256; t += blockDim.x) lcnt[t] = 0;
    __syncthreads();
    int base = blockIdx.x * SORT_BLOCK * SORT_ITEMS;
    uint32_t rank[SORT_ITEMS];
    uint32_t ent[SORT_ITEMS];
    for (int k = 0; k < SORT_ITEMS; ++k) {
        int i = base + k * SORT_BLOCK + threadIdx.x;
        if (i < n) {
            ent[k] = sort_load(in, gather, i);
            rank[k] = atomicAdd(&lcnt[sort_key(ent[k], mode)], 1u);
        }
    }
    __syncthreads();
    for (int t = threadIdx.x; t < 256; t += blockDim.x)
        lbase[t] = lcnt[t] ? atomicAdd(&hist[t], lcnt[t]) : 0;
    __syncthreads();
    for (int k = 0; k < SORT_ITEMS; ++k) {
        int i = base + k * SORT_BLOCK + threadIdx.x;
        if (i < n) {
            uint32_t key = sort_key(ent[k], mode);
            if (key < DEAD) out[lbase[key] + rank[k]] = ent[k];
        }
    }
}

static void wf_sort_launch(const uint32_t* status, const uint32_t* gather, int scan_n,
                           uint32_t* hist, int* live_dev, uint32_t* out, int sort_mode,
                           hipStream_t hs) {
    const int nb = (scan_n + SORT_BLOCK * SORT_ITEMS - 1) / (SORT_BLOCK * SORT_ITEMS);
    (void)hipMemsetAsync(hist, 0, 256 * sizeof(uint32_t), hs);
    hipLaunchKernelGGL(k_sort_hist, dim3(nb), dim3(SORT_BLOCK), 0, hs,
                       status, gather, scan_n, hist, sort_mode);
    hipLaunchKernelGGL(k_sort_scan, dim3(1), dim3(256), 0, hs, hist, live_dev);
    hipLaunchKernelGGL(k_sort_scatter, dim3(nb), dim3(SORT_BLOCK), 0, hs,
                       status, gather, scan_n, hist, out, sort_mode);
}

__global__ __launch_bounds__(256)
void k_wf_shade(SceneView sv, WfState st, const uint32_t* __restrict__ order,
                int live, int bounce) {
    int k = blockIdx.x * blockDim.x + threadIdx.x;
    if (k >= live) return;
    uint32_t entry = order[k];
    int i = (int)(entry & 0x00FFFFFFu);
    float4 h4 = st.hit[i];
    int prim_idx = float_as_int(h4.w);
    float4 ro4 = st.ray_o[i], rd4 = st.ray_d[i], thp4 = st.thp[i], l4 = st.L[i];
    Ray ray(Vec3(ro4.x, ro4.y, ro4.z), Vec3(rd4.x, rd4.y, rd4.z));
    Vec3 thp(thp4.x, thp4.y, thp4.z), L(l4.x, l4.y, l4.z);
    float prev_pdf = rd4.w;
    bool prev_delta = (float_as_uint(thp4.w) & 1u) != 0;
    float4 pn4 = st.prevn[i];
    Vec3 prev_n(pn4.x, pn4.y, pn4.z);
    uint32_t counts = float_as_uint(pn4.w);
    Sampler sp(st.rng[i]);

    Vec3 pos = ray.at(h4.x);
    uint32_t po = sv.prim_obj[prim_idx];
    bool is_sphere = (po & PRIM_SPHERE_BIT) != 0;
    const ObjInfo& obj = sv.objs[po & PRIM_OBJ_MASK];
    const Prim prim = sv.prims[prim_idx];
    Interaction it = get_interaction(prim, sv.attrs[prim_idx], is_sphere, pos, h4.y, h4.z);
    const BsdfParams& bsdf = sv.bsdfs[obj.bsdf_id];
    if (bsdf.tex[TEX_NORMAL] >= 0)
        it.shading_n = apply_normal_map(sv.textures, bsdf.tex[TEX_NORMAL], it.uv, it.shading_n);

    if (obj.emitter_id >= 0) {
        const EmitterParams& em = sv.emitters[obj.emitter_id];
        Vec3 le = emitter_eval_le(em, it.shading_n, -ray.d, it.uv, sv.textures);
        if (!le.is_zero()) {
            float w = 1.f;
            if (!prev_delta) {
                float light_pdf = emitter_pdf_hit(em, ray.d, h4.x, it.shading_n, prev_n, sv.emitter_geom()) *
                                emitter_sel_pdf(sv, obj.emitter_id);
                w = mis_weight(prev_pdf, light_pdf);
            }
            L += thp * le * w;
        }
    }

    if (!bsdf_is_delta(bsdf) && sv.n_emitters > 0) {
        float epdf;
        int ei = pick_emitter(sv, sp, epdf);
        EmitterSampleRec er = emitter_sample(sv.emitters[ei], sv.emitter_geom(), pos,
                                             it.shading_n, sp);
        if (er.pdf > 0.f && !er.radiance.is_zero()) {
            Vec3 to_l = er.pos - pos;
            float dist = to_l.length();
            Vec3 wi = to_l * (1.f / fmaxf(dist, 1e-9f));
            Vec3 f = bsdf_eval(bsdf, -ray.d, wi, it, sv.textures);
            if (!f.is_zero()) {
                float sh_max = (sv.emitters[ei].type == EM_ENVMAP ? ENVMAP_DIST : dist) - 2.f * EPSILON;
                float light_pdf = er.pdf * epdf;
                float w = er.delta ? 1.f
                                   : mis_weight(light_pdf, bsdf_pdf(bsdf, -ray.d, wi, it, sv.textures));
                Vec3 val = thp * f * er.radiance * (w / light_pdf);
                if (!val.is_zero() && !val.has_nan()) {
                    int slot = atomicAdd(st.sh_cnt, 1);
                    Vec3 so = fmadd(wi, EPSILON, pos);
                    st.sh_od[slot] = make_float4(so.x, so.y, so.z, sh_max);
                    st.sh_dir[slot] = make_float4(wi.x, wi.y, wi.z, uint_as_float((uint32_t)i));
                    st.sh_val[slot] = make_float4(val.x, val.y, val.z, 0.f);
                }
            }
        }
    }

    uint32_t status = DEAD;
    float path_lambda = ro4.w;
    BsdfSample bs = bsdf_sample(bsdf, -ray.d, it, sp, sv.textures, &path_lambda);
    if (bs.pdf > 0.f && !bs.weight.is_zero() && !bs.weight.has_nan() && !bs.wi.has_nan()) {
        thp *= bs.weight;
        int nd = counts & 0xFF, ns = (counts >> 8) & 0xFF, nt = (counts >> 16) & 0xFF,
            nb = (counts >> 24) & 0xFF;
        bool over = false;
        if (!(bs.lobe & LOBE_NULL)) {
            if (bs.lobe & LOBE_DIFFUSE)  over |= (++nd > sv.md.max_diffuse);
            if (bs.lobe & LOBE_SPECULAR) over |= (++ns > sv.md.max_specular);
            if (bs.lobe & LOBE_TRANSMIT) over |= (++nt > sv.md.max_transmit);
            ++nb;
        }
        over |= (nb >= sv.md.max_depth);
        if (!over && nb > 1) {
            float p = clampv(thp.max_elem(), 0.f, 1.f);
            if (p < 0.1f) {
                if (sp.next1f() >= p * 10.f) over = true;
                else thp *= (1.f / (p * 10.f));
            }
        }
        if (!over) {
            status = 0;
            counts = pack_counts(nd, ns, nt, nb);
            prev_delta = (bs.lobe & LOBE_DELTA) != 0;
            prev_pdf = bs.pdf;
            prev_n = it.shading_n;
            Vec3 no = fmadd(bs.wi, EPSILON, pos);
            st.ray_o[i] = make_float4(no.x, no.y, no.z, path_lambda);
            st.ray_d[i] = make_float4(bs.wi.x, bs.wi.y, bs.wi.z, prev_pdf);
        }
    }
    st.thp[i] = make_float4(thp.x, thp.y, thp.z, uint_as_float(prev_delta ? 1u : 0u));
    st.L[i] = make_float4(L.x, L.y, L.z, l4.w);
    st.prevn[i] = make_float4(prev_n.x, prev_n.y, prev_n.z, uint_as_float(counts));
    st.rng[i] = sp.state;
    st.status[i] = (status << 24) | (uint32_t)i;
}

template <int MINW>
__global__ __launch_bounds__(256)
__attribute__((amdgpu_waves_per_eu(MINW, MINW)))
void k_wf_shadow(SceneView sv, WfState st, int lds_n, int n_cached) {
    extern __shared__ uint64_t s_stk[];
    TravCtx tc = trav_lds_ctx(sv, s_stk, threadIdx.x, lds_n, n_cached);
    int k = blockIdx.x * blockDim.x + threadIdx.x;
    if (k >= *st.sh_cnt) return;
    float4 od = st.sh_od[k];
    float4 dir = st.sh_dir[k];
    Ray ray(Vec3(od.x, od.y, od.z), Vec3(dir.x, dir.y, dir.z));
    if (scene_occluded(sv, ray, od.w, tc)) return;
    int i = (int)float_as_uint(dir.w);
    float4 v = st.sh_val[k];
    float4 l4 = st.L[i];
    st.L[i] = make_float4(l4.x + v.x, l4.y + v.y, l4.z + v.z, l4.w);
}

__device__ inline void wf_trace_finish(const SceneView& sv, WfState& st, int i,
                                       const Ray& ray, float prev_pdf,
                                       HitRecord hit) {
    if (hit.prim_idx < 0) hit.t = MAX_DIST;
    st.hit[i] = make_float4(hit.t, hit.u, hit.v, int_as_float(hit.prim_idx));
    uint32_t status;
    if (hit.prim_idx < 0) {
        status = DEAD;
        if (sv.env_emitter >= 0) {
            float4 thp4 = st.thp[i];
            float4 pn4 = st.prevn[i];
            bool prev_delta = (float_as_uint(thp4.w) & 1u) != 0;
            const EmitterParams& env = sv.emitters[sv.env_emitter];
            Vec3 le = envmap_eval(env, ray.d, sv.textures);
            float w = 1.f;
            if (!prev_delta) {
                float light_pdf = emitter_pdf_hit(env, ray.d, ENVMAP_DIST, ray.d,
                                                  Vec3(pn4.x, pn4.y, pn4.z),
                                                  sv.emitter_geom()) *
                                  emitter_sel_pdf(sv, sv.env_emitter);
                w = mis_weight(prev_pdf, light_pdf);
            }
            float4 l4 = st.L[i];
            Vec3 L = Vec3(l4.x, l4.y, l4.z) + Vec3(thp4.x, thp4.y, thp4.z) * le * w;
            st.L[i] = make_float4(L.x, L.y, L.z, l4.w);
        }
    } else {
        uint32_t oi = sv.prim_obj[hit.prim_idx] & PRIM_OBJ_MASK;
        status = (uint32_t)(sv.objs[oi].bsdf_id & 0x3F);
    }
    st.status[i] = (status << 24) | (uint32_t)i;
}

template <int MINW>
__global__ __launch_bounds__(256)
__attribute__((amdgpu_waves_per_eu(MINW, MINW)))
void k_wf_trace(SceneView sv, WfState st, const uint32_t* __restrict__ order,
                int live, int lds_n, int n_cached) {
    extern __shared__ uint64_t s_stk[];
    TravCtx tc = trav_lds_ctx(sv, s_stk, threadIdx.x, lds_n, n_cached);
    int k = blockIdx.x * blockDim.x + threadIdx.x;
    if (k >= live) return;
    int i = (int)(order[k] & 0x00FFFFFFu);
    if (st.status[i] >> 24 >= DEAD) return;
    float4 ro4 = st.ray_o[i], rd4 = st.ray_d[i];
    Ray ray(Vec3(ro4.x, ro4.y, ro4.z), Vec3(rd4.x, rd4.y, rd4.z));
    HitRecord hit = scene_intersect(sv, ray, MAX_DIST, tc);
    wf_trace_finish(sv, st, i, ray, rd4.w, hit);
}

__global__ __launch_bounds__(256)
__attribute__((amdgpu_waves_per_eu(4, 4)))
void k_wf_trace_dual(SceneView sv, WfState st, const uint32_t* __restrict__ order,
                     int live, int lds_n) {
    extern __shared__ uint64_t s_stk[];
    const int tid = threadIdx.x;
    const int half = (live + 1) >> 1;
    const int k0 = blockIdx.x * blockDim.x + tid;
    const int k1 = k0 + half;
    const int lds_half = lds_n >> 1;
    LdsSlot slot0 = (LdsSlot)&s_stk[tid];
    LdsSlot slot1 = (LdsSlot)&s_stk[tid + (size_t)lds_half * BVH4_LDS_STRIDE];
    const int i0 = k0 < half ? (int)(order[k0] & 0x00FFFFFFu) : 0;
    const int i1 = k1 < live ? (int)(order[k1] & 0x00FFFFFFu) : 0;
    bool a0 = k0 < half && (st.status[i0] >> 24) < DEAD;
    bool a1 = k1 < live && (st.status[i1] >> 24) < DEAD;
    if (!a0 && !a1) return;
    Ray ray0, ray1;
    float pdf0 = 0.f, pdf1 = 0.f;
    Bvh4Walk w0, w1;
    if (a0) {
        float4 ro = st.ray_o[i0], rd = st.ray_d[i0];
        ray0 = Ray(Vec3(ro.x, ro.y, ro.z), Vec3(rd.x, rd.y, rd.z));
        pdf0 = rd.w;
        bvh4_walk_init(w0, ray0, MAX_DIST);
    }
    if (a1) {
        float4 ro = st.ray_o[i1], rd = st.ray_d[i1];
        ray1 = Ray(Vec3(ro.x, ro.y, ro.z), Vec3(rd.x, rd.y, rd.z));
        pdf1 = rd.w;
        bvh4_walk_init(w1, ray1, MAX_DIST);
    }
    bool r0 = a0, r1 = a1;
    while (r0 | r1) {
        if (r0) r0 = bvh4_walk_step(w0, sv.nodes4t, sv.prims, sv.prim_obj, slot0, lds_half);
        if (r1) r1 = bvh4_walk_step(w1, sv.nodes4t, sv.prims, sv.prim_obj, slot1, lds_half);
    }
    if (a0) wf_trace_finish(sv, st, i0, ray0, pdf0, w0.rec);
    if (a1) wf_trace_finish(sv, st, i1, ray1, pdf1, w1.rec);
}

__device__ __forceinline__ void wf_load_ps(const WfState& st, int i, PathState& ps,
                                           Sampler& sp, HitRecord& hit) {
    float4 ro4 = st.ray_o[i], rd4 = st.ray_d[i], thp4 = st.thp[i], l4 = st.L[i];
    float4 h4 = st.hit[i], pn4 = st.prevn[i];
    ps.ray = Ray(Vec3(ro4.x, ro4.y, ro4.z), Vec3(rd4.x, rd4.y, rd4.z));
    ps.L = Vec3(l4.x, l4.y, l4.z);
    ps.thp = Vec3(thp4.x, thp4.y, thp4.z);
    ps.prev_pdf = rd4.w;
    ps.prev_delta = (float_as_uint(thp4.w) & 1u) != 0;
    ps.prev_n = Vec3(pn4.x, pn4.y, pn4.z);
    ps.path_time = 0.f;
    uint32_t counts = float_as_uint(pn4.w);
    ps.st.n_diffuse = (int)(counts & 0xFF);
    ps.st.n_specular = (int)((counts >> 8) & 0xFF);
    ps.st.n_transmit = (int)((counts >> 16) & 0xFF);
    ps.st.n_volume = 0;
    ps.b = (int)((counts >> 24) & 0xFF);
    ps.iter = ps.b + 1;
    ps.aov_n = Vec3(0.f); ps.aov_alb = Vec3(0.f); ps.aov_t = 0.f;
    ps.lambda = ro4.w;
    sp = Sampler(st.rng[i]);
    hit.t = h4.x; hit.u = h4.y; hit.v = h4.z;
    hit.prim_idx = float_as_int(h4.w);
}

__device__ __forceinline__ void wf_store_ps(WfState& st, int i, const PathState& ps,
                                            const Sampler& sp) {
    st.ray_o[i] = make_float4(ps.ray.o.x, ps.ray.o.y, ps.ray.o.z, ps.lambda);
    st.ray_d[i] = make_float4(ps.ray.d.x, ps.ray.d.y, ps.ray.d.z, ps.prev_pdf);
    st.thp[i] = make_float4(ps.thp.x, ps.thp.y, ps.thp.z,
                            uint_as_float(ps.prev_delta ? 1u : 0u));
    st.L[i] = make_float4(ps.L.x, ps.L.y, ps.L.z, 0.f);
    st.prevn[i] = make_float4(ps.prev_n.x, ps.prev_n.y, ps.prev_n.z,
                              uint_as_float(pack_counts(ps.st.n_diffuse, ps.st.n_specular,
                                                        ps.st.n_transmit, ps.b)));
    st.rng[i] = sp.state;
}

__device__ __forceinline__ void wf_step_core(const SceneView& sv, WfState& st, int i,
                                             PathState& ps, Sampler& sp, TravCtx tc,
                                             const HitRecord& hit, int extra_bounces,
                                             int do_trace) {
    bool done = path_shade_hit(sv, ps, sp, tc, hit);
    for (int b = 0; b < extra_bounces && !done; ++b)
        done = path_step(sv, ps, sp, tc);
    if (!done && ps.b >= sv.md.max_depth) done = true;
    uint32_t status = DEAD;
    if (!done && do_trace) {
        HitRecord nh = scene_intersect(sv, ps.ray, MAX_DIST, tc);
        if (nh.prim_idx < 0) {
            nh.t = MAX_DIST;
            path_shade_hit(sv, ps, sp, tc, nh);
        } else {
            uint32_t oi = sv.prim_obj[nh.prim_idx] & PRIM_OBJ_MASK;
            status = (uint32_t)(sv.objs[oi].bsdf_id & 0x3F);
        }
        st.hit[i] = make_float4(nh.t, nh.u, nh.v, int_as_float(nh.prim_idx));
    }
    wf_store_ps(st, i, ps, sp);
    st.status[i] = (status << 24) | (uint32_t)i;
}

template <int MINW>
__global__ __launch_bounds__(256)
__attribute__((amdgpu_waves_per_eu(MINW, MINW)))
void k_wf_step(SceneView sv, WfState st, const uint32_t* __restrict__ order,
               int live, int extra_bounces, int do_trace, int lds_n, int n_cached) {
    extern __shared__ uint64_t s_stk[];
    TravCtx tc = trav_lds_ctx(sv, s_stk, threadIdx.x, lds_n, n_cached);
    int k = blockIdx.x * blockDim.x + threadIdx.x;
    if (k >= live) return;
    int i = (int)(order[k] & 0x00FFFFFFu);
    PathState ps;
    Sampler sp(0, 0);
    HitRecord hit;
    wf_load_ps(st, i, ps, sp, hit);
    wf_step_core(sv, st, i, ps, sp, tc, hit, extra_bounces, do_trace);
}

template <int MINW>
__global__ __launch_bounds__(256)
__attribute__((amdgpu_waves_per_eu(MINW, MINW)))
void k_wf_primary(SceneView sv, WfState st, int spp_idx, uint32_t seed,
                  int extra_bounces, int do_trace, int lds_n, int n_cached) {
    extern __shared__ uint64_t s_stk[];
    TravCtx tc = trav_lds_ctx(sv, s_stk, threadIdx.x, lds_n, n_cached);
    int i = blockIdx.x * blockDim.x + threadIdx.x;
    if (i >= st.n) return;
    int px = i % st.w, py = i / st.w;
    Sampler sp(uint32_t(i), uint32_t(spp_idx) * SEED_SCALER + seed);
    Ray ray = sv.cam.gen_ray(px, py, sp, spp_idx);
    PathState ps;
    ps.reset(ray);
    ps.iter = 1;
    HitRecord hit = scene_intersect(sv, ray, MAX_DIST, tc);
    if (hit.prim_idx < 0) hit.t = MAX_DIST;
    wf_step_core(sv, st, i, ps, sp, tc, hit, extra_bounces, do_trace);
}

template <int MINW>
__global__ __launch_bounds__(256)
__attribute__((amdgpu_waves_per_eu(MINW, MINW)))
void k_wf_tail(SceneView sv, WfState st, const uint32_t* __restrict__ order,
               int live, int lds_n, int n_cached) {
    extern __shared__ uint64_t s_stk[];
    TravCtx tc = trav_lds_ctx(sv, s_stk, threadIdx.x, lds_n, n_cached);
    int k = blockIdx.x * blockDim.x + threadIdx.x;
    if (k >= live) return;
    int i = (int)(order[k] & 0x00FFFFFFu);
    PathState ps;
    Sampler sp(0, 0);
    HitRecord hit;
    wf_load_ps(st, i, ps, sp, hit);
    bool done = path_shade_hit(sv, ps, sp, tc, hit);
    while (!done) done = path_step(sv, ps, sp, tc);
    float lw = st.L[i].w;
    st.L[i] = make_float4(ps.L.x, ps.L.y, ps.L.z, lw);
    st.status[i] = (DEAD << 24) | (uint32_t)i;
}

__global__ __launch_bounds__(256)
void k_wf_splat(SceneView sv, WfState st, float* __restrict__ accum, float* __restrict__ var, int nspp_done) {
    int i = blockIdx.x * blockDim.x + threadIdx.x;
    if (i >= st.n) return;
    float4 l4 = st.L[i];
    Vec3 L(l4.x, l4.y, l4.z);
    if (L.has_nan()) L = Vec3(0.f);
    L = clamp_radiance(sv, L);
    float* a = accum + (size_t)i * 4;
    a[0] += L.x; a[1] += L.y; a[2] += L.z; a[3] += 1.f;
    if (var) {
        float lum = (L.x + L.y + L.z) * (1.f / 3.f);
        var[(size_t)i * 2 + 0] += lum;
        var[(size_t)i * 2 + 1] += lum * lum;
    }
    (void)nspp_done;
}

template <typename T>
static int wf_alloc(T** p, size_t count) { return (int)hipMalloc((void**)p, count * sizeof(T)); }

WfState* wf_create(int width, int height) {
    if ((long long)width * height > WF_MAX_PIXELS) return nullptr;
    WfState* s = new WfState();
    s->w = width; s->h = height; s->n = width * height;
    s->nb_sort = (s->n + SORT_BLOCK * SORT_ITEMS - 1) / (SORT_BLOCK * SORT_ITEMS);
    int e = 0;
    e |= wf_alloc(&s->ray_o, s->n);
    e |= wf_alloc(&s->ray_d, s->n);
    e |= wf_alloc(&s->thp, s->n);
    e |= wf_alloc(&s->L, s->n);
    e |= wf_alloc(&s->hit, s->n);
    e |= wf_alloc(&s->prevn, s->n);
    e |= wf_alloc(&s->rng, s->n);
    e |= wf_alloc(&s->status, s->n);
    e |= wf_alloc(&s->order, s->n);
    e |= wf_alloc(&s->order2, s->n);
    e |= wf_alloc(&s->hist, (size_t)s->nb_sort * 256);
    e |= wf_alloc(&s->live_dev, 1);
    e |= wf_alloc(&s->sh_od, s->n);
    e |= wf_alloc(&s->sh_dir, s->n);
    e |= wf_alloc(&s->sh_val, s->n);
    e |= wf_alloc(&s->sh_cnt, 1);
    e |= (int)hipHostMalloc((void**)&s->live_host, sizeof(int));
    if (e) { wf_destroy(s); return nullptr; }
    return s;
}

void wf_destroy(WfState* s) {
    if (!s) return;
    (void)hipFree(s->ray_o); (void)hipFree(s->ray_d); (void)hipFree(s->thp); (void)hipFree(s->L);
    (void)hipFree(s->hit); (void)hipFree(s->prevn); (void)hipFree(s->rng);
    (void)hipFree(s->status); (void)hipFree(s->order); (void)hipFree(s->order2);
    (void)hipFree(s->hist);
    (void)hipFree(s->live_dev);
    (void)hipFree(s->sh_od); (void)hipFree(s->sh_dir); (void)hipFree(s->sh_val); (void)hipFree(s->sh_cnt);
    if (s->live_host) (void)hipHostFree(s->live_host);
    delete s;
}

static int wf_occ() {
    static const int occ = env_int("HIPPT_WF_OCC", 4);
    return occ < 3 ? 3 : (occ > 6 ? 6 : occ);
}
#define WF_BY_OCC(k) (wf_occ() == 3 ? k<3> : wf_occ() == 4 ? k<4> : wf_occ() == 5 ? k<5> : k<6>)

static LdsPlan wf_lds_plan(const SceneView& sv, int lds_req = -1, int cache_in = -1) {
    static const bool stack_in_lds = !env_is("HIPPT_WF_STACK", "scratch");
    return lds_plan(wf_occ(), stack_in_lds, true, sv.n_nodes4, (int)sizeof(TravNode),
                    top_cache_request(sv, cache_in), lds_req);
}

int launch_render_wavefront(WfState* st, const SceneView& sv, float* accum, float* var,
                            int spp0, int nspp, uint32_t seed, int sort_mode, void* stream) {
    if (sort_mode < 0 || sort_mode > 1) sort_mode = 0;
    static const int env_mode = env_is("HIPPT_WF_SORT", "compact") ? 1 : -1;
    if (env_mode >= 0) sort_mode = env_mode;
    hipStream_t hs = (hipStream_t)stream;
    const int n = st->n;
    dim3 blk(WF_BLOCK);
    dim3 grd_n((n + WF_BLOCK - 1) / WF_BLOCK);
    static const auto f_raygen = WF_BY_OCC(k_wf_raygen);
    static const auto f_primary = WF_BY_OCC(k_wf_primary);
    static const auto f_trace = WF_BY_OCC(k_wf_trace);
    static const auto f_tail = WF_BY_OCC(k_wf_tail);
    static const auto f_step = WF_BY_OCC(k_wf_step);
    static const auto f_shadow = WF_BY_OCC(k_wf_shadow);
    static const int prim_fuse = env_int("HIPPT_WF_PRIMARY_FUSE", 1);
    static const int wf_fuse = env_int("HIPPT_WF_FUSE", 1);
    static const int span_env = env_int("HIPPT_WF_SPAN", 8);
    static const int wf_span = span_env < 1 ? 1 : (span_env > 16 ? 16 : span_env);
    const LdsPlan plan = wf_lds_plan(sv);
    const int n_cached = plan.n_cached;
    const int lds_n = plan.lds_n;
    const uint32_t shmem = plan.shmem;
    static int wf_dual = env_int("HIPPT_WF_DUAL", 0);
    if (wf_dual && 3 * sv.bvh4_depth > BVH4_STACK / 2 + lds_n / 2) wf_dual = 0;
    static const int tail_thresh = env_int("HIPPT_WF_TAIL", 1500 * 1024);
    static const int wf_log = env_int("HIPPT_WF_LOG", 0);
    for (int s = 0; s < nspp; ++s) {
        int bounce0;
        const int n_stage = sv.md.max_depth + 1;
        if (prim_fuse && wf_fuse) {
            int cnt = wf_span < n_stage ? wf_span : n_stage;
            hipLaunchKernelGGL(f_primary, grd_n, blk, shmem, hs, sv, *st, spp0 + s,
                               seed, cnt - 1, cnt < n_stage ? 1 : 0, lds_n, n_cached);
            bounce0 = cnt;
        } else {
            hipLaunchKernelGGL(f_raygen, grd_n, blk, shmem, hs, sv, *st, spp0 + s, seed,
                               lds_n, n_cached);
            bounce0 = 0;
        }
        const uint32_t* gather = nullptr;
        int prev_live = n;
        uint32_t* order_cur = st->order;
        uint32_t* order_prev = st->order2;
        for (int bounce = bounce0; bounce < n_stage; bounce += (wf_fuse ? wf_span : 1)) {
            const int scan_n = prev_live;
            wf_sort_launch(st->status, gather, scan_n, st->hist, st->live_dev,
                           order_cur, sort_mode, hs);
            (void)hipMemcpyAsync(st->live_host, st->live_dev, sizeof(int),
                                 hipMemcpyDeviceToHost, hs);
            int err = (int)hipStreamSynchronize(hs);
            if (err) return err;
            const int live = *st->live_host;
            if (wf_log && s == 0)
                printf("[wf] spp %d bounce %d live %d (%.1f%%)\n", spp0 + s, bounce,
                       live, 100.0 * live / n);
            if (live == 0) break;
            dim3 grd_live((live + WF_BLOCK - 1) / WF_BLOCK);
            if (live <= tail_thresh) {
                hipLaunchKernelGGL(f_tail, grd_live, blk, shmem, hs, sv, *st,
                                   order_cur, live, lds_n, n_cached);
                break;
            }
            if (wf_fuse) {
                int cnt = wf_span < n_stage - bounce ? wf_span : n_stage - bounce;
                hipLaunchKernelGGL(f_step, grd_live, blk, shmem, hs, sv, *st, order_cur,
                                   live, cnt - 1, bounce + cnt < n_stage ? 1 : 0,
                                   lds_n, n_cached);
            } else {
            (void)hipMemsetAsync(st->sh_cnt, 0, sizeof(int), hs);
            hipLaunchKernelGGL(k_wf_shade, grd_live, blk, 0, hs, sv, *st, order_cur,
                               live, bounce);
            hipLaunchKernelGGL(f_shadow, grd_live, blk, shmem, hs, sv, *st,
                               lds_n, n_cached);
            if (bounce < sv.md.max_depth) {
                if (wf_dual) {
                    dim3 grd_h(((live + 1) / 2 + WF_BLOCK - 1) / WF_BLOCK);
                    hipLaunchKernelGGL(k_wf_trace_dual, grd_h, blk,
                                       (uint32_t)(lds_n * WF_BLOCK * 8), hs, sv, *st,
                                       order_cur, live, lds_n);
                } else {
                    hipLaunchKernelGGL(f_trace, grd_live, blk, shmem, hs, sv, *st,
                                       order_cur, live, lds_n, n_cached);
                }
            }
            }
            gather = order_cur;
            prev_live = live;
            uint32_t* t = order_cur; order_cur = order_prev; order_prev = t;
        }
        hipLaunchKernelGGL(k_wf_splat, grd_n, blk, 0, hs, sv, *st, accum, var, 1);
    }
    return (int)hipGetLastError();
}

template <typename T>
struct DevBuf {
    T* p = nullptr;
    ~DevBuf() { if (p) (void)hipFree(p); }
    int alloc(size_t count) { return (int)hipMalloc((void**)&p, (count ? count : 1) * sizeof(T)); }
};

int wf_sort_probe(const uint32_t* status, int n, const uint32_t* gather, int m,
                  int mode, uint32_t* out, int* live) {
    if (n <= 0 || n > WF_MAX_PIXELS || m < 0 || m > n || (mode != 0 && mode != 1))
        return (int)hipErrorInvalidValue;
    for (int k = 0; k < m; ++k)
        if ((gather[k] & 0x00FFFFFFu) >= (uint32_t)n) return (int)hipErrorInvalidValue;
    DevBuf<uint32_t> d_status, d_gather, d_out, d_hist;
    DevBuf<int> d_live;
    int e = 0;
    e |= d_status.alloc(n);
    e |= d_gather.alloc(m);
    e |= d_out.alloc(n);
    e |= d_hist.alloc(256);
    e |= d_live.alloc(1);
    if (e) return e;
    e |= (int)hipMemcpy(d_status.p, status, (size_t)n * 4, hipMemcpyHostToDevice);
    if (m > 0) e |= (int)hipMemcpy(d_gather.p, gather, (size_t)m * 4, hipMemcpyHostToDevice);
    e |= (int)hipMemset(d_out.p, 0xFF, (size_t)n * 4);
    e |= (int)hipMemset(d_live.p, 0xFF, sizeof(int));
    if (e) return e;
    wf_sort_launch(d_status.p, m > 0 ? d_gather.p : nullptr, m > 0 ? m : n, d_hist.p,
                   d_live.p, d_out.p, mode, nullptr);
    e |= (int)hipGetLastError();
    e |= (int)hipDeviceSynchronize();
    if (e) return e;
    e |= (int)hipMemcpy(out, d_out.p, (size_t)n * 4, hipMemcpyDeviceToHost);
    e |= (int)hipMemcpy(live, d_live.p, sizeof(int), hipMemcpyDeviceToHost);
    return e;
}

__global__ __launch_bounds__(256)
void k_wf_ray_probe(SceneView sv, const float4* __restrict__ ray_o,
                    const float4* __restrict__ ray_d, int n,
                    float4* __restrict__ hit_out, int* __restrict__ occ_out,
                    int lds_n, int n_cached) {
    extern __shared__ uint64_t s_stk[];
    TravCtx tc = trav_lds_ctx(sv, s_stk, threadIdx.x, lds_n, n_cached);
    int i = blockIdx.x * blockDim.x + threadIdx.x;
    if (i >= n) return;
    float4 o4 = ray_o[i], d4 = ray_d[i];
    Ray ray(Vec3(o4.x, o4.y, o4.z), Vec3(d4.x, d4.y, d4.z));
    HitRecord hit = scene_intersect(sv, ray, o4.w, tc);
    hit_out[i] = make_float4(hit.t, hit.u, hit.v, int_as_float(hit.prim_idx));
    occ_out[i] = scene_occluded(sv, ray, o4.w, tc) ? 1 : 0;
}

int wf_trace_probe(const SceneView& sv, const float* ray_o_tmax, const float* ray_d,
                   int n, int lds_n, int n_cached, float* hit_out, int* occ_out,
                   int* plan_out) {
    if (n <= 0 || sv.n_nodes4 <= 0) return (int)hipErrorInvalidValue;
    const LdsPlan plan = wf_lds_plan(sv, lds_n, n_cached);
    plan_out[0] = plan.lds_n;
    plan_out[1] = plan.n_cached;
    DevBuf<float4> d_o, d_d, d_hit;
    DevBuf<int> d_occ;
    int e = 0;
    e |= d_o.alloc(n);
    e |= d_d.alloc(n);
    e |= d_hit.alloc(n);
    e |= d_occ.alloc(n);
    if (e) return e;
    e |= (int)hipMemcpy(d_o.p, ray_o_tmax, (size_t)n * 16, hipMemcpyHostToDevice);
    e |= (int)hipMemcpy(d_d.p, ray_d, (size_t)n * 16, hipMemcpyHostToDevice);
    if (e) return e;
    hipLaunchKernelGGL(k_wf_ray_probe, dim3((n + WF_BLOCK - 1) / WF_BLOCK), dim3(WF_BLOCK),
                       plan.shmem, nullptr, sv, d_o.p, d_d.p, n, d_hit.p, d_occ.p,
                       plan.lds_n, plan.n_cached);
    e |= (int)hipGetLastError();
    e |= (int)hipDeviceSynchronize();
    if (e) return e;
    e |= (int)hipMemcpy(hit_out, d_hit.p, (size_t)n * 16, hipMemcpyDeviceToHost);
    e |= (int)hipMemcpy(occ_out, d_occ.p, (size_t)n * 4, hipMemcpyDeviceToHost);
    return e;
}

}
```

hippt/scene/scene.py:

```python
from __future__ import annotations

import math
import os
from dataclasses import dataclass, field
from typing import Dict, List, Optional, Tuple

import numpy as np

from .. import C
from .sparse_grid import SparseGrid, union_coords

BSDF_TYPES = {
    "lambertian": 0, "diffuse": 0,
    "specular": 1, "mirror": 1,
    "translucent": 2, "glass": 2, "dielectric": 2,
    "plastic": 3,
    "plastic-forward": 4, "plastic_forward": 4,
    "ggx": 5, "conductor": 5, "metal": 5, "roughconductor": 5,
    "dispersion": 6,
    "forward": 7, "null": 7,
}
EM_POINT, EM_AREA, EM_AREA_SPOT, EM_ENVMAP = 1, 2, 3, 4
PHASE_TYPES = {"isotropic": 0, "hg": 1, "duo-hg": 2, "duohg": 2, "rayleigh": 3, "sggx": 4}
PRIM_SPHERE_BIT = np.uint32(0x80000000)

METALS = {
    "Au": ((0.143, 0.375, 1.442), (3.983, 2.386, 1.603)),
    "Ag": ((0.155, 0.116, 0.138), (4.818, 3.115, 2.140)),
    "Al": ((1.345, 0.965, 0.617), (7.475, 6.400, 5.303)),
    "Cu": ((0.200, 0.924, 1.102), (3.910, 2.447, 2.137)),
    "Cr": ((4.361, 2.910, 1.650), (5.198, 4.222, 3.560)),
    "W":  ((3.660, 3.480, 3.310), (2.950, 2.710, 2.560)),
    "Ni": ((2.361, 1.663, 1.467), (4.498, 3.051, 2.344)),
    "TiO2": ((2.741, 2.542, 2.267), (0.001, 0.001, 0.001)),
    "MgO": ((1.737, 1.737, 1.737), (0.0, 0.0, 0.0)),
    "Na": ((0.048, 0.054, 0.063), (2.610, 2.214, 1.867)),
    "SiC": ((2.649, 2.676, 2.744), (0.0, 0.0, 0.0)),
    "V":  ((3.512, 3.671, 3.219), (2.902, 3.064, 3.303)),
    "CuO": ((2.955, 2.608, 2.385), (0.617, 0.557, 0.736)),
    "Hg": ((1.864, 1.442, 1.104), (5.120, 4.613, 3.968)),
    "Ir": ((2.540, 2.170, 1.870), (4.690, 4.240, 3.790)),
}
DISPERSION_PRESETS = {
    "diamond": (2.3818, 0.0121),
    "sapphire": (1.7522, 0.0055),
    "fused-silica": (1.4580, 0.00354),
    "bk7": (1.5046, 0.0042),
    "sf11": (1.7377, 0.0138),
    "dense-flint": (1.7280, 0.01342),
    "moissanite": (2.5610, 0.0340),
    "water-ice": (1.3049, 0.00317),
}


@dataclass
class BsdfDesc:
    type: str = "lambertian"
    kd: Tuple[float, ...] = (0.8, 0.8, 0.8)
    ks: Tuple[float, ...] = (1.0, 1.0, 1.0)
    kg: Tuple[float, ...] = (0.0, 0.0, 0.0)
    ior: float = 1.5
    roughness_x: float = 0.1
    roughness_y: float = 0.1
    trans_scaler: float = 1.0
    thickness: float = 0.0
    metal: Optional[str] = None
    preset: Optional[str] = None
    textures: Dict[str, int] = field(default_factory=dict)


@dataclass
class EmitterDesc:
    type: str = "area"
    emission: Tuple[float, ...] = (1.0, 1.0, 1.0)
    scale: float = 1.0
    pos: Tuple[float, ...] = (0.0, 0.0, 0.0)
    cos_max: float = 0.5
    azimuth: float = 0.0
    zenith: float = 0.0
    tex_id: int = -1


@dataclass
class MediumDesc:
    type: str = "homogeneous"
    sigma_a: Tuple[float, ...] = (0.1, 0.1, 0.1)
    sigma_s: Tuple[float, ...] = (1.0, 1.0, 1.0)
    phase: str = "isotropic"
    g1: float = 0.0
    g2: float = 0.0
    wmix: float = 0.5
    density: Optional[object] = None
    temperature: Optional[object] = None
    grid_lo: Tuple[float, ...] = (0, 0, 0)
    grid_hi: Tuple[float, ...] = (1, 1, 1)
    scale: float = 1.0
    emission_scale: float = 0.0
    temp_scale: float = 1.0


@dataclass
class ObjectDesc:
    tris: Optional[np.ndarray] = None
    normals: Optional[np.ndarray] = None
    uvs: Optional[np.ndarray] = None
    spheres: Optional[np.ndarray] = None
    bsdf: int = 0
    emitter: int = -1
    medium_in: int = -1
    medium_out: int = -1
    cullable: bool = False


@dataclass
class CameraDesc:
    pos: Tuple[float, ...] = (0.0, 0.0, 0.0)
    lookat: Tuple[float, ...] = (0.0, 0.0, 1.0)
    up: Tuple[float, ...] = (0.0, 1.0, 0.0)
    fov: float = 60.0
    width: int = 512
    height: int = 512
    aperture: float = 0.0
    focal_dist: float = 1.0
    ortho: bool = False
    ortho_scale: float = 0.01
    hflip: bool = False


@dataclass
class RenderConfig:
    spp: int = 64
    max_depth: int = 16
    max_diffuse: int = 8
    max_specular: int = 16
    max_transmit: int = 16
    max_volume: int = 16
    min_time: float = 0.0
    max_time: float = 0.0
    use_tof: bool = False
    renderer: str = "pt"
    max_leaf: int = 8
    overlap_w: float = 0.6
    bvh_trav_cost: float = 1.0
    use_sbvh: bool = False
    ref_unsplit: bool = True
    cache_level: int = 6
    radiance_clamp: float = 0.0
    spec_constraint: int = 0
    caustic_scaling: float = 1.0
    bidirectional: bool = False


@dataclass
class SceneDesc:
    objects: List[ObjectDesc] = field(default_factory=list)
    bsdfs: List[BsdfDesc] = field(default_factory=list)
    emitters: List[EmitterDesc] = field(default_factory=list)
    media: List[MediumDesc] = field(default_factory=list)
    textures: List[np.ndarray] = field(default_factory=list)
    camera: CameraDesc = field(default_factory=CameraDesc)
    config: RenderConfig = field(default_factory=RenderConfig)
    cam_medium: int = -1
    env_emitter_id: int = -1


def camera_matrix(desc: CameraDesc) -> np.ndarray:
    f = np.asarray(desc.lookat, np.float64) - np.asarray(desc.pos, np.float64)
    f = f / np.linalg.norm(f)
    u = np.asarray(desc.up, np.float64)
    r = np.cross(u, f)
    r = r / np.linalg.norm(r)
    if desc.hflip:
        r = -r
    tu = np.cross(f, r if not desc.hflip else -r)
    R = np.stack([r, tu, f], axis=1)
    return R.astype(np.float32)


def _tex_slots(b: BsdfDesc) -> List[int]:
    slots = [-1] * 8
    names = {"diffuse": 0, "specular": 1, "glossy": 2, "normal": 3, "roughness": 4}
    for k, v in b.textures.items():
        slots[names[k]] = v
    return slots


class Scene:

    def __init__(self, desc: SceneDesc):
        self.desc = desc
        self.native = C.Scene()
        self._uploaded_device = None
        self._build()

    def _build(self):
        d = self.desc
        cfg = d.config

        for t in d.textures:
            t4 = np.ascontiguousarray(t, np.float32)
            assert t4.ndim == 3 and t4.shape[2] == 4
            self.native.add_texture(t4)

        for b in d.bsdfs:
            ty = BSDF_TYPES[b.type]
            kd, ks, kg = list(b.kd), list(b.ks), list(b.kg)
            ior, e0, e1 = b.ior, 0.0, 0.0
            if ty == 5:
                eta, kk = METALS.get(b.metal or "Au", METALS["Au"])
                kd, ks = list(eta), list(kk)
                if not any(kg):
                    kg = [1.0, 1.0, 1.0]
                e0, e1 = b.roughness_x, b.roughness_y
            elif ty == 3 or ty == 4:
                e0, e1 = b.trans_scaler, b.thickness
            elif ty == 6:
                A, B = DISPERSION_PRESETS.get(b.preset or "diamond", DISPERSION_PRESETS["diamond"])
                e0, e1 = A, B
            self.native.add_bsdf(ty, kd, ks, kg, ior, e0, e1, _tex_slots(b))

        force_bricks = os.environ.get("HIPPT_SPARSE_GRID", "0") not in ("", "0")
        for m in d.media:
            pid = self.native.add_phase(PHASE_TYPES[m.phase], m.g1, m.g2, m.wmix)
            mty = 0 if m.type == "homogeneous" else 1
            if mty == 1 and m.density is not None and (
                    force_bricks or isinstance(m.density, SparseGrid)
                    or isinstance(m.temperature, SparseGrid)):
                self._add_medium_bricks(m, pid)
                continue
            dens = None if m.density is None else np.ascontiguousarray(m.density, np.float32)
            temp = None if m.temperature is None else np.ascontiguousarray(m.temperature, np.float32)
            self.native.add_medium(mty, list(m.sigma_a), list(m.sigma_s), pid,
                                   list(m.grid_lo), list(m.grid_hi), dens, temp,
                                   m.scale, m.emission_scale, m.temp_scale)

        prim_blocks, attr_blocks, pobj_blocks = [], [], []
        obj_rows = []
        obj_prim_ranges = []
        base = 0
        for oi, o in enumerate(d.objects):
            if o.spheres is not None:
                s = np.asarray(o.spheres, np.float32).reshape(-1, 4)
                n = len(s)
                pr = np.zeros((n, 12), np.float32)
                pr[:, 0:4] = s
                at = np.zeros((n, 16), np.float32)
                po = np.full(n, oi, np.uint32) | PRIM_SPHERE_BIT
                areas = 4.0 * math.pi * s[:, 3] ** 2
            else:
                v = np.asarray(o.tris, np.float32).reshape(-1, 3, 3)
                n = len(v)
                pr = np.zeros((n, 12), np.float32)
                pr[:, 0:3] = v[:, 0]
                pr[:, 4:7] = v[:, 1] - v[:, 0]
                pr[:, 8:11] = v[:, 2] - v[:, 0]
                at = np.zeros((n, 16), np.float32)
                if o.normals is not None:
                    nm = np.asarray(o.normals, np.float32).reshape(-1, 3, 3)
                else:
                    gn = np.cross(pr[:, 4:7], pr[:, 8:11])
                    gl = np.linalg.norm(gn, axis=1, keepdims=True)
                    gn = gn / np.maximum(gl, 1e-20)
                    nm = np.repeat(gn[:, None, :], 3, axis=1)
                at[:, 0:3] = nm[:, 0]
                at[:, 4:7] = nm[:, 1]
                at[:, 8:11] = nm[:, 2]
                if o.uvs is not None:
                    uv = np.asarray(o.uvs, np.float32).reshape(-1, 3, 2)
                    at[:, 3] = uv[:, 0, 0]; at[:, 7] = uv[:, 0, 1]
                    at[:, 11] = uv[:, 1, 0]; at[:, 12] = uv[:, 1, 1]
                    at[:, 13] = uv[:, 2, 0]; at[:, 14] = uv[:, 2, 1]
                po = np.full(n, oi, np.uint32)
                areas = 0.5 * np.linalg.norm(np.cross(pr[:, 4:7], pr[:, 8:11]), axis=1)
            prim_blocks.append(pr)
            attr_blocks.append(at)
            pobj_blocks.append(po)
            total_area = float(areas.sum())
            inv_area = 1.0 / total_area if total_area > 0 else 0.0
            flags = 1 if o.cullable else 0
            row = np.zeros(8, np.int32)
            row[0] = base; row[1] = n
            row[2] = o.bsdf; row[3] = o.emitter
            row[4] = o.medium_in; row[5] = o.medium_out
            row[6] = flags
            row.view(np.float32)[7] = inv_area
            obj_rows.append(row)
            obj_prim_ranges.append((base, n, areas))
            base += n

        prims = np.concatenate(prim_blocks, axis=0) if prim_blocks else np.zeros((0, 12), np.float32)
        attrs = np.concatenate(attr_blocks, axis=0) if attr_blocks else np.zeros((0, 16), np.float32)
        prim_obj = np.concatenate(pobj_blocks, axis=0) if pobj_blocks else np.zeros(0, np.uint32)
        objs = np.stack(obj_rows, axis=0) if obj_rows else np.zeros((0, 8), np.int32)

        import os as _os
        max_leaf = int(_os.environ.get("HIPPT_MAX_LEAF", cfg.max_leaf))
        overlap_w = float(_os.environ.get("HIPPT_OVERLAP_W", cfg.overlap_w))
        trav_cost = float(_os.environ.get("HIPPT_BVH_CT", cfg.bvh_trav_cost))
        nodes, order, stats = C.build_bvh(prims, prim_obj, max_leaf, overlap_w,
                                          cfg.use_sbvh, cfg.ref_unsplit, trav_cost)
        self.bvh_stats = stats
        nodes4, depth4 = C.collapse_bvh4(nodes)
        nodes8 = np.zeros((0, 64), np.float32)
        self.bvh_stats = dict(stats, n_nodes4=int(nodes4.shape[0]), depth4=int(depth4))
        nodes = np.concatenate([nodes, np.zeros((1, 8), np.float32)])
        prims = np.ascontiguousarray(prims[order])
        attrs = np.ascontiguousarray(attrs[order])
        prim_obj = np.ascontiguousarray(prim_obj[order])
        new_of_old = np.empty(len(order), np.int64)
        new_of_old[order] = np.arange(len(order))

        self.native.set_geometry(prims, attrs, prim_obj, nodes, nodes4, nodes8)
        self.native.set_objects(objs)
        self._np = dict(prims=prims, attrs=attrs, prim_obj=prim_obj, nodes=nodes,
                        nodes4=nodes4, objs=objs, order=np.asarray(order))

        eprims: List[int] = []
        ecdf: List[float] = []
        emitter_areas = {}
        for ei, e in enumerate(d.emitters):
            etype = {"point": EM_POINT, "area": EM_AREA, "area-spot": EM_AREA_SPOT,
                     "envmap": EM_ENVMAP}[e.type]
            aux = [0.0, 0.0, 0.0, 0.0]
            obj_id, prim_base, prim_cnt, inv_area = -1, 0, 0, 0.0
            if etype == EM_POINT:
                aux[:3] = list(e.pos)
            elif etype == EM_ENVMAP:
                aux[0], aux[1] = e.azimuth, e.zenith
            else:
                for oi, o in enumerate(d.objects):
                    if o.emitter == ei:
                        obj_id = oi
                        b0, n, areas = obj_prim_ranges[oi]
                        prim_base = len(eprims)
                        prim_cnt = n
                        old_ids = np.arange(b0, b0 + n)
                        eprims.extend(new_of_old[old_ids].tolist())
                        tot = float(areas.sum())
                        emitter_areas[ei] = tot
                        inv_area = 1.0 / tot if tot > 0 else 0.0
                        cdf = np.cumsum(areas) / max(tot, 1e-30)
                        ecdf.extend(cdf.tolist())
                        break
                if etype == EM_AREA_SPOT:
                    aux[3] = e.cos_max
            self.native.add_emitter(etype, list(e.emission), e.scale, aux, obj_id,
                                    -1 if e.tex_id is None else e.tex_id,
                                    prim_base, prim_cnt, inv_area)
        self.native.set_emitter_prims(np.asarray(eprims, np.int32),
                                      np.asarray(ecdf, np.float32))

        if len(d.emitters) > 1 and os.environ.get("HIPPT_LIGHT_POWER") != "0":
            powers = []
            for ei, e in enumerate(d.emitters):
                mean_e = float(np.mean(e.emission)) * float(e.scale)
                if e.type == "point":
                    p_ = mean_e * 4.0 * math.pi
                elif e.type == "envmap":
                    lum = 1.0
                    if e.tex_id is not None and 0 <= e.tex_id < len(d.textures):
                        lum = float(d.textures[e.tex_id][..., :3].mean())
                    p_ = mean_e * lum * 4.0 * math.pi
                else:
                    area = emitter_areas.get(ei, 1.0)
                    p_ = mean_e * area * math.pi
                    if e.type == "area-spot":
                        p_ *= max(1.0 - e.cos_max, 1e-3)
                powers.append(max(p_, 1e-9))
            w = np.asarray(powers, np.float64)
            w = np.maximum(w, 0.05 * w.mean())
            cdf = np.cumsum(w) / w.sum()
            self.native.set_emitter_sel(cdf.astype(np.float32))

        for e in d.emitters:
            if os.environ.get("HIPPT_ENV_IS") == "0":
                break
            if e.type == "envmap" and e.tex_id is not None and e.tex_id >= 0 \
                    and e.tex_id < len(d.textures):
                img = d.textures[e.tex_id]
                lum = img[..., :3].mean(axis=2).astype(np.float64)
                h, w = lum.shape
                sin_t = np.sin((np.arange(h) + 0.5) * np.pi / h)[:, None]
                wgt = np.maximum(lum * sin_t, 1e-12)
                row_sum = wgt.sum(axis=1)
                rows = np.cumsum(row_sum)
                rows /= rows[-1]
                cols = np.cumsum(wgt, axis=1)
                cols /= cols[:, -1:]
                self.native.set_env_cdf(rows.astype(np.float32),
                                        np.ascontiguousarray(cols, np.float32))
                break

        self._set_camera_native()
        self.native.set_depths(cfg.max_depth, cfg.max_diffuse, cfg.max_specular,
                               cfg.max_transmit, cfg.max_volume,
                               cfg.min_time, cfg.max_time, int(cfg.use_tof),
                               cfg.radiance_clamp)
        self.native.set_cache_level(int(cfg.cache_level))
        self.native.cam_medium = d.cam_medium
        self.native.finalize()

    def _add_medium_bricks(self, m: MediumDesc, pid: int):
        def as_sparse(g):
            return g if isinstance(g, SparseGrid) else SparseGrid.from_dense(g)
        dens = as_sparse(m.density)
        temp = None if m.temperature is None else as_sparse(m.temperature)
        coords, dvals, tvals = dens.coords, dens.values, None
        if temp is not None:
            if temp.shape != dens.shape:
                raise ValueError(f"density grid {dens.shape} and temperature grid "
                                 f"{temp.shape} must have the same shape")
            coords = union_coords(dens, temp)
            dvals, tvals = dens.reindexed(coords), temp.reindexed(coords)
            tvals = tvals.reshape(-1, 512)
        self.native.add_medium_sparse(list(m.sigma_a), list(m.sigma_s), pid,
                                      list(m.grid_lo), list(m.grid_hi),
                                      list(dens.shape), coords, dvals.reshape(-1, 512),
                                      tvals, m.scale, m.emission_scale, m.temp_scale)

    def _set_camera_native(self):
        c = self.desc.camera
        R = camera_matrix(c)
        focal = 0.5 * c.width / math.tan(0.5 * math.radians(c.fov))
        self.native.set_camera(list(np.asarray(c.pos, np.float32)),
                               [float(x) for x in R.reshape(-1)], float(focal),
                               c.width, c.height, c.aperture, c.focal_dist,
                               int(c.ortho), c.ortho_scale)

    def upload(self, device: int = 0):
        self.native.upload(device)
        self._uploaded_device = device

    def trace_rays(self, o, d, tmax, device: int = -1, lds_n: int = -1,
                   n_cached: int = -1):
        o = np.ascontiguousarray(o, np.float32).reshape(-1, 3)
        d = np.ascontiguousarray(d, np.float32).reshape(-1, 3)
        tmax = np.ascontiguousarray(tmax, np.float32).reshape(-1)
        if device >= 0 and self._uploaded_device != device:
            self.upload(device)
        t, prim, u, v, occ, plan = self.native.trace_rays(o, d, tmax, device,
                                                          lds_n, n_cached)
        self.last_trace_plan = tuple(plan)
        return t, prim, u, v, occ.astype(bool)

    def update_camera(self, pos=None, lookat=None, up=None, fov=None):
        c = self.desc.camera
        if pos is not None:
            c.pos = tuple(pos)
        if lookat is not None:
            c.lookat = tuple(lookat)
        if up is not None:
            c.up = tuple(up)
        if fov is not None:
            c.fov = fov
        self._set_camera_native()
        self.native.finalize()

    def set_bsdf(self, i: int, b: BsdfDesc):
        from .scene import BSDF_TYPES
        self.desc.bsdfs[i] = b
        ty = BSDF_TYPES[b.type]
        kd, ks, kg = list(b.kd), list(b.ks), list(b.kg)
        ior, e0, e1 = b.ior, 0.0, 0.0
        if ty == 5:
            eta, kk = METALS.get(b.metal or "Au", METALS["Au"])
            kd, ks = list(eta), list(kk)
            if not any(kg):
                kg = [1.0, 1.0, 1.0]
            e0, e1 = b.roughness_x, b.roughness_y
        elif ty in (3, 4):
            e0, e1 = b.trans_scaler, b.thickness
        elif ty == 6:
            A, B = DISPERSION_PRESETS.get(b.preset or "diamond",
                                          DISPERSION_PRESETS["diamond"])
            e0, e1 = A, B
        self.native.update_bsdf(i, ty, kd, ks, kg, ior, e0, e1, _tex_slots(b))
        self.native.finalize()

    def set_emitter(self, i: int, emission=None, scale=None, cos_max=None,
                    azimuth=None, zenith=None, pos=None):
        e = self.desc.emitters[i]
        if emission is not None:
            e.emission = tuple(emission)
        if scale is not None:
            e.scale = float(scale)
        if cos_max is not None:
            e.cos_max = float(cos_max)
        if azimuth is not None:
            e.azimuth = float(azimuth)
        if zenith is not None:
            e.zenith = float(zenith)
        if pos is not None:
            e.pos = tuple(pos)
        aux = [0.0, 0.0, 0.0, 0.0]
        if e.type == "point":
            aux[:3] = list(e.pos)
        elif e.type == "envmap":
            aux[0], aux[1] = e.azimuth, e.zenith
        elif e.type == "area-spot":
            aux[3] = e.cos_max
        self.native.update_emitter(i, list(e.emission), e.scale, aux)
        self.native.finalize()

    def set_medium(self, i: int, sigma_a=None, sigma_s=None, scale=None,
                   emission_scale=None):
        m = self.desc.media[i]
        if sigma_a is not None:
            m.sigma_a = tuple(sigma_a)
        if sigma_s is not None:
            m.sigma_s = tuple(sigma_s)
        if scale is not None:
            m.scale = float(scale)
        if emission_scale is not None:
            m.emission_scale = float(emission_scale)
        self.native.update_medium(i, list(m.sigma_a), list(m.sigma_s), m.scale,
                                  m.emission_scale)
        self.native.finalize()

    def set_depths(self, **kw):
        cfg = self.desc.config
        for k, v in kw.items():
            setattr(cfg, k, v)
        self.native.set_depths(cfg.max_depth, cfg.max_diffuse, cfg.max_specular,
                               cfg.max_transmit, cfg.max_volume,
                               cfg.min_time, cfg.max_time, int(cfg.use_tof),
                               cfg.radiance_clamp)
        self.native.finalize()

    @property
    def width(self):
        return self.desc.camera.width

    @property
    def height(self):
        return self.desc.camera.height

    def info(self):
        i = dict(self.native.info())
        i.update(self.bvh_stats)
        i["renderer"] = self.desc.config.renderer
        i["resolution"] = (self.width, self.height)
        i["media"] = [dict(mi) for mi in self.native.media_info()]
        return i
```

Baseline: 294.1 Msamples/s.

## Pack per-primitive shading word and contiguous light-primitive records for shading

Precomputes a packed per-primitive shading word (bsdf id, emitter id, sphere bit) so hit shading reads one word instead of chasing prim_obj and then the object table. It also builds 128-byte LightPrim records holding prim, attributes and the sphere flag, so emitter sampling does one contiguous load instead of indirecting through emitter_prims into the prims, attrs and prim_obj arrays. Shading now goes through load_hit_shade, load_bsdf and load_emitter helpers, and the device copy uses asm register pinning to keep the loads wide. In exchange it adds host preprocessing, extra device memory, and limits on the bsdf and emitter counts that fit in the packed word.

```diff
diff --git a/csrc/bind.cpp b/csrc/bind.cpp
--- a/csrc/bind.cpp
+++ b/csrc/bind.cpp
@@ -76,6 +76,18 @@
 }
 
 static std::vector<uint64_t> host_lds_slots(int lds_n);
+
+std::vector<uint32_t> make_prim_shade(const uint32_t* prim_obj, size_t n_prims,
+                                      const int32_t* objs, size_t n_objs) {
+    std::vector<uint32_t> out(n_prims);
+    int bad = -1;
+    if (!build_prim_shade(prim_obj, (int)n_prims, objs, (int)n_objs, out.data(), &bad))
+        throw std::runtime_error(
+            "build_prim_shade: primitive " + std::to_string(bad) +
+            " needs object < n_objs, 0 <= bsdf_id < " + std::to_string(SHADE_MAX_BSDFS) +
+            " and emitter_id < " + std::to_string(SHADE_MAX_EMITTERS));
+    return out;
+}
 
 struct SceneHolder {
     farr np_prims, np_attrs, np_nodes, np_nodes4, np_nodes8;
@@ -93,6 +105,9 @@
     std::vector<TexView> tex_host;
     std::vector<int> emitter_prims;
     std::vector<float> emitter_cdf;
+    std::vector<uint32_t> prim_shade;
+    std::vector<LightPrim> light_prims;
+    bool shade_stale = true;
     std::vector<float> env_rows_h, env_cols_h;
     int env_w = 0, env_h = 0;
     std::vector<float> emitter_sel_h;
@@ -133,6 +148,7 @@
         np_prims = std::move(prims);
         np_attrs = std::move(attrs);
         np_prim_obj = std::move(prim_obj);
+        shade_stale = true;
         np_nodes = std::move(nodes);
         np_nodes4 = std::move(nodes4);
         if (nodes8.ndim() == 2 && nodes8.shape(0) > 0 && nodes8.shape(1) != 64)
@@ -185,6 +201,7 @@
     void set_objects(iarr objs) {
         if (objs.ndim() != 2 || objs.shape(1) != 8) throw std::runtime_error("objs must be (n,8)");
         np_objs = std::move(objs);
+        shade_stale = true;
     }
 
     int add_bsdf(int type, std::vector<float> kd, std::vector<float> ks, std::vector<float> kg,
@@ -237,6 +254,7 @@
 
     void set_emitter_prims(iarr eprims, farr ecdf) {
         emitter_prims.assign(eprims.data(), eprims.data() + eprims.size());
+        shade_stale = true;
         emitter_cdf.assign(ecdf.data(), ecdf.data() + ecdf.size());
     }
 
@@ -540,6 +558,20 @@
     }
 
     void finalize() {
+        if (shade_stale) {
+            prim_shade = make_prim_shade(np_prim_obj.data(), (size_t)np_prim_obj.size(),
+                                         np_objs.data(),
+                                         np_objs.ndim() == 2 ? (size_t)np_objs.shape(0) : 0);
+            const int n_prims = np_prims.ndim() == 2 ? (int)np_prims.shape(0) : 0;
+            for (int pid : emitter_prims)
+                if (pid < 0 || pid >= n_prims)
+                    throw std::runtime_error("emitter_prims entry outside the primitive array");
+            light_prims.resize(emitter_prims.size());
+            build_light_prims((const Prim*)np_prims.data(), (const PrimAttr*)np_attrs.data(),
+                              np_prim_obj.data(), emitter_prims.data(), emitter_prims.size(),
+                              light_prims.data());
+            shade_stale = false;
+        }
         fill_common(host_sv);
         host_sv.nodes = (const BVHNode*)np_nodes.data();
         host_sv.nodes4 = host_sv.n_nodes4 > 0 ? (const BVH4Node*)np_nodes4.data() : nullptr;
@@ -550,10 +582,12 @@
         host_sv.attrs = (const PrimAttr*)np_attrs.data();
         host_sv.prim_obj = np_prim_obj.data();
         host_sv.objs = (const ObjInfo*)np_objs.data();
+        host_sv.prim_shade = prim_shade.data();
         host_sv.bsdfs = bsdfs.data();
         host_sv.emitters = emitters.data();
         host_sv.emitter_prims = emitter_prims.data();
         host_sv.emitter_cdf = emitter_cdf.data();
+        host_sv.light_prims = light_prims.data();
         host_sv.env_rows = env_rows_h.empty() ? nullptr : env_rows_h.data();
         host_sv.env_cols = env_cols_h.empty() ? nullptr : env_cols_h.data();
         host_sv.emitter_sel_cdf = emitter_sel_h.empty() ? nullptr : emitter_sel_h.data();
@@ -591,8 +625,10 @@
         dev_sv.attrs = upload_vec((const PrimAttr*)np_attrs.data(), np_attrs.shape(0));
         dev_sv.prim_obj = upload_vec(np_prim_obj.data(), np_prim_obj.size());
         dev_sv.objs = upload_vec((const ObjInfo*)np_objs.data(), np_objs.shape(0));
+        dev_sv.prim_shade = upload_vec(prim_shade.data(), prim_shade.size());
         dev_sv.emitter_prims = upload_vec(emitter_prims.data(), emitter_prims.size());
         dev_sv.emitter_cdf = upload_vec(emitter_cdf.data(), emitter_cdf.size());
+        dev_sv.light_prims = upload_vec(light_prims.data(), light_prims.size());
         dev_sv.env_rows = upload_vec(env_rows_h.data(), env_rows_h.size());
         dev_sv.env_cols = upload_vec(env_cols_h.data(), env_cols_h.size());
         dev_sv.emitter_sel_cdf = upload_vec(emitter_sel_h.data(), emitter_sel_h.size());
@@ -737,6 +773,53 @@
         }
         return py::make_tuple(t_out, p_out, u_out, v_out, occ_out,
                               py::make_tuple(plan[0], plan[1]));
+    }
+
+    py::tuple shade_probe_py(iarr prim_idx, int device) {
+        const int n = (int)prim_idx.size();
+        finalize();
+        const int n_prims = host_sv.n_prims;
+        for (int i = 0; i < n; ++i)
+            if (prim_idx.data()[i] < 0 || prim_idx.data()[i] >= n_prims)
+                throw std::runtime_error("shade_probe: primitive index out of range");
+        std::vector<uint32_t> raw((size_t)n * SHADE_PROBE_WORDS, 0u);
+        if (n > 0) {
+            if (device < 0) {
+                for (int i = 0; i < n; ++i)
+                    shade_probe_record(host_sv, prim_idx.data()[i],
+                                       raw.data() + (size_t)i * SHADE_PROBE_WORDS);
+            } else {
+                if (!has_dev) throw std::runtime_error("scene not uploaded to device");
+                HIP_OK(shade_probe(dev_sv, prim_idx.data(), n, raw.data()));
+            }
+        }
+        uarr attr({n, 16}), word(n), bsdf({n, 20}), em({n, 16});
+        for (int i = 0; i < n; ++i) {
+            const uint32_t* r = raw.data() + (size_t)i * SHADE_PROBE_WORDS;
+            std::memcpy(attr.mutable_data() + (size_t)i * 16, r, 64);
+            word.mutable_data()[i] = r[16];
+            std::memcpy(bsdf.mutable_data() + (size_t)i * 20, r + 17, 80);
+            std::memcpy(em.mutable_data() + (size_t)i * 16, r + 37, 64);
+        }
+        return py::make_tuple(attr, word, bsdf, em);
+    }
+
+    py::dict tables() {
+        finalize();
+        auto rows = [](const void* src, size_t n, int words) {
+            uarr a({(py::ssize_t)n, (py::ssize_t)words});
+            if (n) std::memcpy(a.mutable_data(), src, n * words * 4);
+            return a;
+        };
+        py::dict d;
+        d["bsdfs"] = rows(bsdfs.data(), bsdfs.size(), sizeof(BsdfParams) / 4);
+        d["emitters"] = rows(emitters.data(), emitters.size(), sizeof(EmitterParams) / 4);
+        d["light_prims"] = rows(light_prims.data(), light_prims.size(), sizeof(LightPrim) / 4);
+        uarr w((py::ssize_t)prim_shade.size());
+        if (!prim_shade.empty())
+            std::memcpy(w.mutable_data(), prim_shade.data(), prim_shade.size() * 4);
+        d["prim_shade"] = w;
+        return d;
     }
 
     py::dict info() {
@@ -1115,6 +1198,9 @@
         .def("trace_rays", &SceneHolder::trace_rays, py::arg("o"), py::arg("d"),
              py::arg("tmax"), py::arg("device"), py::arg("lds_n") = -1,
              py::arg("n_cached") = -1)
+        .def("shade_probe", &SceneHolder::shade_probe_py, py::arg("prim_idx"),
+             py::arg("device"))
+        .def("tables", &SceneHolder::tables)
         .def("info", &SceneHolder::info);
 
     m.def("build_bvh", &py_build_bvh, py::arg("prims"), py::arg("prim_obj"),
@@ -1129,6 +1215,30 @@
           py::arg("ray_o"), py::arg("ray_d"), py::arg("tmax"));
     m.def("bvh4_any_visit_selftest", &py_bvh4_any_visit_selftest, py::arg("nodes4"),
           py::arg("ray_o"), py::arg("ray_d"), py::arg("tmax"));
+    m.def("build_prim_shade", [](uarr prim_obj, iarr objs) {
+        if (objs.ndim() != 2 || objs.shape(1) != 8) throw std::runtime_error("objs must be (n,8)");
+        std::vector<uint32_t> w = make_prim_shade(prim_obj.data(), (size_t)prim_obj.size(),
+                                                  objs.data(), (size_t)objs.shape(0));
+        uarr out((py::ssize_t)w.size());
+        if (!w.empty()) std::memcpy(out.mutable_data(), w.data(), w.size() * 4);
+        return out;
+    }, py::arg("prim_obj"), py::arg("objs"));
+    m.def("build_light_prims", [](farr prims, farr attrs, uarr prim_obj, iarr emitter_prims) {
+        if (prims.ndim() != 2 || prims.shape(1) != 12) throw std::runtime_error("prims must be (n,12)");
+        if (attrs.ndim() != 2 || attrs.shape(1) != 16) throw std::runtime_error("attrs must be (n,16)");
+        const py::ssize_t n_prims = prims.shape(0);
+        if (attrs.shape(0) != n_prims || prim_obj.size() != n_prims)
+            throw std::runtime_error("prims, attrs and prim_obj must have one row per primitive");
+        const py::ssize_t n = emitter_prims.size();
+        for (py::ssize_t k = 0; k < n; ++k)
+            if (emitter_prims.data()[k] < 0 || emitter_prims.data()[k] >= n_prims)
+                throw std::runtime_error("emitter_prims entry outside the primitive array");
+        uarr out({n, (py::ssize_t)32});
+        build_light_prims((const Prim*)prims.data(), (const PrimAttr*)attrs.data(),
+                          prim_obj.data(), emitter_prims.data(), (size_t)n,
+                          (LightPrim*)out.mutable_data());
+        return out;
+    }, py::arg("prims"), py::arg("attrs"), py::arg("prim_obj"), py::arg("emitter_prims"));
     m.def("bsdf_check", &py_bsdf_check);
     m.def("env_check", &py_env_check);
     m.def("bvh4q_selftest", &py_bvh4q_selftest,
diff --git a/csrc/core/emitter.h b/csrc/core/emitter.h
--- a/csrc/core/emitter.h
+++ b/csrc/core/emitter.h
@@ -34,11 +34,42 @@
     bool delta;
 };
 
+struct alignas(16) LightPrim {
+    Prim prim;
+    PrimAttr attr;
+    uint32_t sphere;
+    uint32_t pad[3];
+};
+static_assert(sizeof(LightPrim) == 128, "LightPrim is one 128-byte record");
+
+inline void build_light_prims(const Prim* prims, const PrimAttr* attrs,
+                              const uint32_t* prim_obj, const int32_t* emitter_prims,
+                              size_t n, LightPrim* out) {
+    for (size_t k = 0; k < n; ++k) {
+        const int32_t pid = emitter_prims[k];
+        LightPrim& lp = out[k];
+        lp.prim = prims[pid];
+        lp.attr = attrs[pid];
+        lp.sphere = prim_obj[pid] & PRIM_SPHERE_BIT;
+        lp.pad[0] = lp.pad[1] = lp.pad[2] = 0u;
+    }
+}
+
+#if !HIPPT_ON_DEVICE
+HD const LightPrim& load_light_prim(const LightPrim* light_prims, int k) { return light_prims[k]; }
+#else
+HD LightPrim load_light_prim(const LightPrim* light_prims, int k) {
+    const LightPrim lp = light_prims[k];
+    asm volatile("" :: HIPPT_LANDED_VEC4(lp.prim.v0), HIPPT_LANDED_VEC4(lp.prim.e1),
+                       HIPPT_LANDED_VEC4(lp.prim.e2), HIPPT_LANDED_VEC4(lp.attr.n0),
+                       HIPPT_LANDED_VEC4(lp.attr.n1), HIPPT_LANDED_VEC4(lp.attr.n2),
+                       HIPPT_LANDED_VEC4(lp.attr.uvrest), "v"(lp.sphere));
+    return lp;
+}
+#endif
+
 struct EmitterGeom {
-    const Prim* prims;
-    const PrimAttr* attrs;
-    const uint32_t* prim_obj;
-    const int* emitter_prims;
+    const LightPrim* light_prims;
     const float* emitter_cdf;
     const TexView* textures;
     const float* env_rows;
@@ -132,9 +163,9 @@
         const float* cdf = g.emitter_cdf + e.prim_base;
         int lo = 0, hi = cnt - 1;
         while (lo < hi) { int mid = (lo + hi) >> 1; if (cdf[mid] < xi) lo = mid + 1; else hi = mid; }
-        int pid = g.emitter_prims[e.prim_base + lo];
-        const Prim p = g.prims[pid];
-        bool sph = (g.prim_obj[pid] & PRIM_SPHERE_BIT) != 0;
+        const auto& lp = load_light_prim(g.light_prims, e.prim_base + lo);
+        const Prim p = lp.prim;
+        bool sph = lp.sphere != 0;
         Vec3 lpos, ln; Vec2 uv{0.f, 0.f};
         if (sph) {
             float pdf_dir;
@@ -144,7 +175,7 @@
         } else {
             Vec3 bc = sample_triangle_bary(sampler.next2f());
             lpos = p.v0.xyz() + p.e1.xyz() * bc.y + p.e2.xyz() * bc.z;
-            const PrimAttr a = g.attrs[pid];
+            const PrimAttr a = lp.attr;
             Vec3 nsum = a.n0.xyz() * bc.x + a.n1.xyz() * bc.y + a.n2.xyz() * bc.z;
             ln = nsum.length2() > 1e-16f ? nsum.normalized()
                                          : p.e1.xyz().cross(p.e2.xyz()).normalized();
@@ -255,9 +286,9 @@
         const float* cdf = g.emitter_cdf + e.prim_base;
         int lo = 0, hi = cnt - 1;
         while (lo < hi) { int mid = (lo + hi) >> 1; if (cdf[mid] < xi) lo = mid + 1; else hi = mid; }
-        int pid = g.emitter_prims[e.prim_base + lo];
-        const Prim p = g.prims[pid];
-        bool sph = (g.prim_obj[pid] & PRIM_SPHERE_BIT) != 0;
+        const auto& lp = load_light_prim(g.light_prims, e.prim_base + lo);
+        const Prim p = lp.prim;
+        bool sph = lp.sphere != 0;
         Vec3 lpos, ln; Vec2 uv{0.f, 0.f};
         if (sph) {
             float pdf_sph;
@@ -267,7 +298,7 @@
         } else {
             Vec3 bc = sample_triangle_bary(sampler.next2f());
             lpos = p.v0.xyz() + p.e1.xyz() * bc.y + p.e2.xyz() * bc.z;
-            const PrimAttr a = g.attrs[pid];
+            const PrimAttr a = lp.attr;
             Vec3 nsum = a.n0.xyz() * bc.x + a.n1.xyz() * bc.y + a.n2.xyz() * bc.z;
             ln = nsum.length2() > 1e-16f ? nsum.normalized()
                                          : p.e1.xyz().cross(p.e2.xyz()).normalized();
diff --git a/csrc/core/hd.h b/csrc/core/hd.h
--- a/csrc/core/hd.h
+++ b/csrc/core/hd.h
@@ -17,6 +17,10 @@
 #define HIPPT_ON_DEVICE 1
 #else
 #define HIPPT_ON_DEVICE 0
+#endif
+
+#if HIPPT_ON_DEVICE
+#define HIPPT_LANDED_VEC4(a) "v"((a).x), "v"((a).y), "v"((a).z), "v"((a).w)
 #endif
 
 namespace hippt {
diff --git a/csrc/core/integrator.h b/csrc/core/integrator.h
--- a/csrc/core/integrator.h
+++ b/csrc/core/integrator.h
@@ -83,12 +83,12 @@
         }
         Vec3 pos = ray.at(hit.t);
         path_time += hit.t;
-        uint32_t po = sv.prim_obj[hit.prim_idx];
-        bool is_sphere = (po & PRIM_SPHERE_BIT) != 0;
-        const ObjInfo& obj = sv.objs[po & PRIM_OBJ_MASK];
-        const Prim prim = sv.prims[hit.prim_idx];
-        Interaction it = get_interaction(prim, sv.attrs[hit.prim_idx], is_sphere, pos, hit.u, hit.v);
-        const BsdfParams& bsdf = sv.bsdfs[obj.bsdf_id];
+        const HitShade hs = load_hit_shade(sv, hit.prim_idx);
+        const bool is_sphere = shade_is_sphere(hs.word);
+        const int bsdf_id = shade_bsdf_id(hs.word);
+        const int emitter_id = shade_emitter_id(hs.word);
+        const auto& bsdf = load_bsdf(sv.bsdfs, bsdf_id);
+        Interaction it = get_interaction(sv.prims[hit.prim_idx], hs.attr, is_sphere, pos, hit.u, hit.v);
         if (bsdf.tex[TEX_NORMAL] >= 0)
             it.shading_n = apply_normal_map(sv.textures, bsdf.tex[TEX_NORMAL], it.uv, it.shading_n);
         if (ps.iter == 1) {
@@ -97,14 +97,14 @@
             ps.aov_alb = bsdf_aov_albedo(bsdf, it.uv, sv.textures);
         }
 
-        if (obj.emitter_id >= 0) {
-            const EmitterParams& em = sv.emitters[obj.emitter_id];
+        if (emitter_id >= 0) {
+            const auto& em = load_emitter(sv.emitters, emitter_id);
             Vec3 le = emitter_eval_le(em, it.shading_n, -ray.d, it.uv, sv.textures);
             if (!le.is_zero()) {
                 float w = 1.f;
                 if (!prev_delta) {
                     float light_pdf = emitter_pdf_hit(em, ray.d, hit.t, it.shading_n, prev_n, sv.emitter_geom()) *
-                                   emitter_sel_pdf(sv, obj.emitter_id);
+                                   emitter_sel_pdf(sv, emitter_id);
                     w = mis_weight(prev_pdf, light_pdf);
                 }
                 if (tof_in_range(sv.md, path_time)) L += thp * le * w;
@@ -112,9 +112,10 @@
         }
 
         if (!bsdf_is_delta(bsdf) && sv.n_emitters > 0) {
-            float epdf;
-            int ei = pick_emitter(sv, sp, epdf);
-            EmitterSampleRec er = emitter_sample(sv.emitters[ei], sv.emitter_geom(), pos, it.shading_n, sp);
+            const EmitterPick pick = pick_emitter_rec(sv, sp);
+            const auto& nee = pick.e;
+            const float epdf = pick.pdf;
+            EmitterSampleRec er = emitter_sample(nee, sv.emitter_geom(), pos, it.shading_n, sp);
             if (er.pdf > 0.f && !er.radiance.is_zero()) {
                 Vec3 to_l = er.pos - pos;
                 float dist = to_l.length();
@@ -122,11 +123,11 @@
                 Vec3 f = bsdf_eval(bsdf, -ray.d, wi, it, sv.textures);
                 if (!f.is_zero()) {
                     Ray sh_ray(fmadd(wi, EPSILON, pos), wi);
-                    float sh_max = (sv.emitters[ei].type == EM_ENVMAP ? ENVMAP_DIST : dist) - 2.f * EPSILON;
+                    float sh_max = (nee.type == EM_ENVMAP ? ENVMAP_DIST : dist) - 2.f * EPSILON;
+                    const float pdf_b = er.delta ? 0.f : bsdf_pdf(bsdf, -ray.d, wi, it, sv.textures);
                     if (!scene_occluded(sv, sh_ray, sh_max, tc)) {
                         float light_pdf = er.pdf * epdf;
-                        float w = er.delta ? 1.f
-                                           : mis_weight(light_pdf, bsdf_pdf(bsdf, -ray.d, wi, it, sv.textures));
+                        float w = er.delta ? 1.f : mis_weight(light_pdf, pdf_b);
                         if (tof_in_range(sv.md, path_time + dist))
                             L += thp * f * er.radiance * (w / light_pdf);
                     }
@@ -134,7 +135,8 @@
             }
         }
 
-        BsdfSample bs = bsdf_sample(bsdf, -ray.d, it, sp, sv.textures, &ps.lambda);
+        BsdfSample bs = bsdf_sample(load_bsdf(sv.bsdfs, bsdf_id), -ray.d, it, sp, sv.textures,
+                                    &ps.lambda);
         if (bs.pdf <= 0.f || bs.weight.is_zero()) return true;
         if (bs.weight.has_nan() || bs.wi.has_nan()) return true;
         thp *= bs.weight;
diff --git a/csrc/core/light_tracer.h b/csrc/core/light_tracer.h
--- a/csrc/core/light_tracer.h
+++ b/csrc/core/light_tracer.h
@@ -8,9 +8,9 @@
 HD void trace_light_path_impl(const SceneView& sv, Sampler& sp, SPLAT_FN&& splat, TravCtx tc,
                               int spec_constraint, float caustic_scaling) {
     if (sv.n_emitters <= 0) return;
-    float epdf;
-    int ei = pick_emitter(sv, sp, epdf);
-    const EmitterParams& em = sv.emitters[ei];
+    const EmitterPick pick = pick_emitter_rec(sv, sp);
+    const auto& em = pick.e;
+    const float epdf = pick.pdf;
     EmitterLeRec le = emitter_sample_le(em, sv.emitter_geom(), sp);
     if (!le.valid) return;
 
@@ -55,12 +55,12 @@
         HitRecord hit = scene_intersect(sv, ray, MAX_DIST, tc);
         if (hit.prim_idx < 0) break;
         Vec3 pos = ray.at(hit.t);
-        uint32_t po = sv.prim_obj[hit.prim_idx];
-        bool is_sphere = (po & PRIM_SPHERE_BIT) != 0;
-        const ObjInfo& obj = sv.objs[po & PRIM_OBJ_MASK];
+        const HitShade hs = load_hit_shade(sv, hit.prim_idx);
+        const bool is_sphere = shade_is_sphere(hs.word);
+        const int bsdf_id = shade_bsdf_id(hs.word);
+        const auto& bsdf = load_bsdf(sv.bsdfs, bsdf_id);
         const Prim prim = sv.prims[hit.prim_idx];
-        Interaction it = get_interaction(prim, sv.attrs[hit.prim_idx], is_sphere, pos, hit.u, hit.v);
-        const BsdfParams& bsdf = sv.bsdfs[obj.bsdf_id];
+        Interaction it = get_interaction(prim, hs.attr, is_sphere, pos, hit.u, hit.v);
 
         if (!bsdf_is_delta(bsdf)) {
             Vec3 to_cam = (sv.cam.pos - pos).normalized();
@@ -68,7 +68,8 @@
             connect(pos, thp * f, n_spec);
         }
 
-        BsdfSample bs = bsdf_sample(bsdf, -ray.d, it, sp, sv.textures, &path_lambda);
+        BsdfSample bs = bsdf_sample(load_bsdf(sv.bsdfs, bsdf_id), -ray.d, it, sp, sv.textures,
+                                    &path_lambda);
         if (bs.pdf <= 0.f || bs.weight.is_zero() || bs.weight.has_nan() || bs.wi.has_nan()) break;
         thp *= bs.weight;
         if (bs.lobe & (LOBE_SPECULAR | LOBE_TRANSMIT)) ++n_spec;
diff --git a/csrc/core/scene_view.h b/csrc/core/scene_view.h
--- a/csrc/core/scene_view.h
+++ b/csrc/core/scene_view.h
@@ -6,6 +6,7 @@
 #include "emitter.h"
 #include "camera.h"
 #include "medium.h"
+#include "shade_load.h"
 
 namespace hippt {
 
@@ -41,10 +42,12 @@
     const BVH8Node* nodes8; int n_nodes8;
     const Prim* prims; const PrimAttr* attrs; const uint32_t* prim_obj; int n_prims;
     const ObjInfo* objs; int n_objs;
+    const uint32_t* prim_shade;
     const BsdfParams* bsdfs; int n_bsdfs;
     const EmitterParams* emitters; int n_emitters;
     const int* emitter_prims;
     const float* emitter_cdf;
+    const LightPrim* light_prims;
     const float* env_rows; const float* env_cols; int env_w, env_h;
     const float* emitter_sel_cdf;
     const TexView* textures; int n_textures;
@@ -61,7 +64,7 @@
     int cache_nodes;
 
     HD EmitterGeom emitter_geom() const {
-        return {prims, attrs, prim_obj, emitter_prims, emitter_cdf, textures,
+        return {light_prims, emitter_cdf, textures,
                 env_rows, env_cols, env_w, env_h,
                 scene_bound.xyz(), scene_bound.w};
     }
@@ -86,6 +89,26 @@
     i = i >= sv.n_emitters ? sv.n_emitters - 1 : i;
     pdf = 1.f / sv.n_emitters;
     return i;
+}
+
+struct EmitterPick {
+#if HIPPT_ON_DEVICE
+    EmitterParams e;
+#else
+    const EmitterParams& e;
+#endif
+    int i;
+    float pdf;
+};
+HD EmitterPick pick_emitter_rec(const SceneView& sv, Sampler& sp) {
+    float pdf;
+    if (sv.emitter_sel_cdf) {
+        const int i = cdf_find(sv.emitter_sel_cdf, sv.n_emitters, sp.next1f());
+        const auto& e = load_emitter_sel(sv.emitters, sv.emitter_sel_cdf, i, pdf);
+        return {e, i, pdf};
+    }
+    const int i = pick_emitter(sv, sp, pdf);
+    return {load_emitter(sv.emitters, i), i, pdf};
 }
 
 #ifdef HIPPT_QBVH
diff --git a/csrc/core/shade_load.h b/csrc/core/shade_load.h
--- /dev/null
+++ b/csrc/core/shade_load.h
@@ -0,0 +1,163 @@
+#pragma once
+#include "geometry.h"
+#include "bsdf.h"
+#include "emitter.h"
+
+namespace hippt {
+
+constexpr uint32_t SHADE_BSDF_MASK = 0xFFFFu;
+constexpr uint32_t SHADE_EMITTER_MASK = 0x7FFFu;
+constexpr int SHADE_EMITTER_SHIFT = 16;
+constexpr int SHADE_MAX_BSDFS = 65536;
+constexpr int SHADE_MAX_EMITTERS = 32767;
+
+HD int shade_bsdf_id(uint32_t w) { return (int)(w & SHADE_BSDF_MASK); }
+HD int shade_emitter_id(uint32_t w) {
+    return (int)((w >> SHADE_EMITTER_SHIFT) & SHADE_EMITTER_MASK) - 1;
+}
+HD bool shade_is_sphere(uint32_t w) { return (w & PRIM_SPHERE_BIT) != 0; }
+
+inline bool build_prim_shade(const uint32_t* prim_obj, int n_prims,
+                             const int32_t* objs, int n_objs,
+                             uint32_t* out, int* bad_prim) {
+    for (int i = 0; i < n_prims; ++i) {
+        const uint32_t oi = prim_obj[i] & PRIM_OBJ_MASK;
+        if ((int)oi >= n_objs) { if (bad_prim) *bad_prim = i; return false; }
+        const int32_t bsdf_id = objs[oi * 8 + 2];
+        const int32_t emitter_id = objs[oi * 8 + 3];
+        if (bsdf_id < 0 || bsdf_id >= SHADE_MAX_BSDFS || emitter_id >= SHADE_MAX_EMITTERS) {
+            if (bad_prim) *bad_prim = i;
+            return false;
+        }
+        const uint32_t em = emitter_id >= 0 ? (uint32_t)(emitter_id + 1) : 0u;
+        out[i] = (prim_obj[i] & PRIM_SPHERE_BIT) | (em << SHADE_EMITTER_SHIFT) |
+                 (uint32_t)bsdf_id;
+    }
+    return true;
+}
+
+#if HIPPT_ON_DEVICE
+#define HIPPT_LANDED_EMITTER(e)                                             \
+    HIPPT_LANDED_VEC4((e).emission), HIPPT_LANDED_VEC4((e).aux),            \
+    "v"((e).type), "v"((e).obj_id), "v"((e).tex_id), "v"((e).prim_base),    \
+    "v"((e).prim_cnt), "v"((e).inv_area), "v"((e).extra0), "v"((e).extra1)
+#endif
+
+#if !HIPPT_ON_DEVICE
+struct HitShade {
+    const PrimAttr& attr;
+    uint32_t word;
+};
+template <class SV>
+HD HitShade load_hit_shade(const SV& sv, int prim_idx) {
+    return {sv.attrs[prim_idx], sv.prim_shade[prim_idx]};
+}
+#else
+struct HitShade {
+    PrimAttr attr;
+    uint32_t word;
+};
+template <class SV>
+HD HitShade load_hit_shade(const SV& sv, int prim_idx) {
+    HitShade h;
+    h.word = sv.prim_shade[prim_idx];
+    h.attr = sv.attrs[prim_idx];
+    asm volatile("" :: "v"(h.word), HIPPT_LANDED_VEC4(h.attr.n0), HIPPT_LANDED_VEC4(h.attr.n1),
+                       HIPPT_LANDED_VEC4(h.attr.n2), HIPPT_LANDED_VEC4(h.attr.uvrest));
+    return h;
+}
+#endif
+
+#if !HIPPT_ON_DEVICE
+HD const BsdfParams& load_bsdf(const BsdfParams* bsdfs, int id) { return bsdfs[id]; }
+HD const EmitterParams& load_emitter(const EmitterParams* emitters, int i) { return emitters[i]; }
+#else
+HD BsdfParams load_bsdf(const BsdfParams* bsdfs, int id) {
+    const BsdfParams b = bsdfs[id];
+    uint32_t t0, t1, t2, t3;
+    __builtin_memcpy(&t0, &b.tex[0], 4);
+    __builtin_memcpy(&t1, &b.tex[2], 4);
+    __builtin_memcpy(&t2, &b.tex[4], 4);
+    __builtin_memcpy(&t3, &b.tex[6], 4);
+    asm volatile("" :: HIPPT_LANDED_VEC4(b.kd), HIPPT_LANDED_VEC4(b.ks), HIPPT_LANDED_VEC4(b.kg),
+                       "v"(b.type), "v"(b.ior), "v"(b.extra0), "v"(b.extra1),
+                       "v"(t0), "v"(t1), "v"(t2), "v"(t3));
+    return b;
+}
+
+HD EmitterParams load_emitter(const EmitterParams* emitters, int i) {
+    const EmitterParams e = emitters[i];
+    asm volatile("" :: HIPPT_LANDED_EMITTER(e));
+    return e;
+}
+#endif
+
+#if !HIPPT_ON_DEVICE
+HD const EmitterParams& load_emitter_sel(const EmitterParams* emitters, const float* sel_cdf,
+                                         int i, float& pdf) {
+    pdf = sel_cdf[i] - (i ? sel_cdf[i - 1] : 0.f);
+    return emitters[i];
+}
+#else
+HD EmitterParams load_emitter_sel(const EmitterParams* emitters, const float* sel_cdf,
+                                  int i, float& pdf) {
+    const float hi = sel_cdf[i];
+    const float lo = sel_cdf[i ? i - 1 : 0];
+    const EmitterParams e = emitters[i];
+    asm volatile("" :: "v"(hi), "v"(lo), HIPPT_LANDED_EMITTER(e));
+    pdf = hi - (i ? lo : 0.f);
+    return e;
+}
+#undef HIPPT_LANDED_EMITTER
+#endif
+
+constexpr int SHADE_PROBE_WORDS = 16 + 1 + 20 + 16;
+
+HD void shade_probe_vec4(uint32_t* out, const Vec4& v) {
+    out[0] = float_as_uint(v.x); out[1] = float_as_uint(v.y);
+    out[2] = float_as_uint(v.z); out[3] = float_as_uint(v.w);
+}
+HD uint32_t shade_probe_tex2(int16_t lo, int16_t hi) {
+    return (uint32_t)(uint16_t)lo | ((uint32_t)(uint16_t)hi << 16);
+}
+template <class SV>
+HD void shade_probe_record(const SV& sv, int prim_idx, uint32_t* out) {
+    for (int k = 0; k < SHADE_PROBE_WORDS; ++k) out[k] = 0u;
+    const HitShade hs = load_hit_shade(sv, prim_idx);
+    shade_probe_vec4(out + 0, hs.attr.n0);
+    shade_probe_vec4(out + 4, hs.attr.n1);
+    shade_probe_vec4(out + 8, hs.attr.n2);
+    shade_probe_vec4(out + 12, hs.attr.uvrest);
+    out[16] = hs.word;
+    const int bsdf_id = shade_bsdf_id(hs.word);
+    if (bsdf_id < sv.n_bsdfs) {
+        const auto& b = load_bsdf(sv.bsdfs, bsdf_id);
+        shade_probe_vec4(out + 17, b.kd);
+        shade_probe_vec4(out + 21, b.ks);
+        shade_probe_vec4(out + 25, b.kg);
+        out[29] = (uint32_t)b.type;
+        out[30] = float_as_uint(b.ior);
+        out[31] = float_as_uint(b.extra0);
+        out[32] = float_as_uint(b.extra1);
+        out[33] = shade_probe_tex2(b.tex[0], b.tex[1]);
+        out[34] = shade_probe_tex2(b.tex[2], b.tex[3]);
+        out[35] = shade_probe_tex2(b.tex[4], b.tex[5]);
+        out[36] = shade_probe_tex2(b.tex[6], b.tex[7]);
+    }
+    const int emitter_id = shade_emitter_id(hs.word);
+    if (emitter_id >= 0 && emitter_id < sv.n_emitters) {
+        const auto& e = load_emitter(sv.emitters, emitter_id);
+        shade_probe_vec4(out + 37, e.emission);
+        shade_probe_vec4(out + 41, e.aux);
+        out[45] = (uint32_t)e.type;
+        out[46] = (uint32_t)e.obj_id;
+        out[47] = (uint32_t)e.tex_id;
+        out[48] = (uint32_t)e.prim_base;
+        out[49] = (uint32_t)e.prim_cnt;
+        out[50] = float_as_uint(e.inv_area);
+        out[51] = float_as_uint(e.extra0);
+        out[52] = float_as_uint(e.extra1);
+    }
+}
+
+}
diff --git a/csrc/hip/kernels.h b/csrc/hip/kernels.h
--- a/csrc/hip/kernels.h
+++ b/csrc/hip/kernels.h
@@ -33,6 +33,7 @@
 int wf_trace_probe(const SceneView& sv, const float* ray_o_tmax, const float* ray_d,
                    int n, int lds_n, int n_cached, float* hit_out, int* occ_out,
                    int* plan_out);
+int shade_probe(const SceneView& sv, const int* prim_idx, int n, uint32_t* out);
 
 int dev_malloc(void** p, size_t n);
 int dev_free(void* p);
diff --git a/csrc/hip/wf_kernels.hip b/csrc/hip/wf_kernels.hip
--- a/csrc/hip/wf_kernels.hip
+++ b/csrc/hip/wf_kernels.hip
@@ -64,8 +64,7 @@
             st.L[i] = make_float4(le.x, le.y, le.z, 0.f);
         }
     } else {
-        uint32_t oi = sv.prim_obj[hit.prim_idx] & PRIM_OBJ_MASK;
-        status = (uint32_t)(sv.objs[oi].bsdf_id & 0x3F);
+        status = (uint32_t)(shade_bsdf_id(sv.prim_shade[hit.prim_idx]) & 0x3F);
     }
     st.status[i] = (status << 24) | (uint32_t)i;
 }
@@ -175,23 +174,22 @@
     Sampler sp(st.rng[i]);
 
     Vec3 pos = ray.at(h4.x);
-    uint32_t po = sv.prim_obj[prim_idx];
-    bool is_sphere = (po & PRIM_SPHERE_BIT) != 0;
-    const ObjInfo& obj = sv.objs[po & PRIM_OBJ_MASK];
-    const Prim prim = sv.prims[prim_idx];
-    Interaction it = get_interaction(prim, sv.attrs[prim_idx], is_sphere, pos, h4.y, h4.z);
-    const BsdfParams& bsdf = sv.bsdfs[obj.bsdf_id];
+    const HitShade hs = load_hit_shade(sv, prim_idx);
+    const bool is_sphere = shade_is_sphere(hs.word);
+    const int emitter_id = shade_emitter_id(hs.word);
+    const auto& bsdf = load_bsdf(sv.bsdfs, shade_bsdf_id(hs.word));
+    Interaction it = get_interaction(sv.prims[prim_idx], hs.attr, is_sphere, pos, h4.y, h4.z);
     if (bsdf.tex[TEX_NORMAL] >= 0)
         it.shading_n = apply_normal_map(sv.textures, bsdf.tex[TEX_NORMAL], it.uv, it.shading_n);
 
-    if (obj.emitter_id >= 0) {
-        const EmitterParams& em = sv.emitters[obj.emitter_id];
+    if (emitter_id >= 0) {
+        const auto& em = load_emitter(sv.emitters, emitter_id);
         Vec3 le = emitter_eval_le(em, it.shading_n, -ray.d, it.uv, sv.textures);
         if (!le.is_zero()) {
             float w = 1.f;
             if (!prev_delta) {
                 float light_pdf = emitter_pdf_hit(em, ray.d, h4.x, it.shading_n, prev_n, sv.emitter_geom()) *
-                                emitter_sel_pdf(sv, obj.emitter_id);
+                                emitter_sel_pdf(sv, emitter_id);
                 w = mis_weight(prev_pdf, light_pdf);
             }
             L += thp * le * w;
@@ -199,17 +197,17 @@
     }
 
     if (!bsdf_is_delta(bsdf) && sv.n_emitters > 0) {
-        float epdf;
-        int ei = pick_emitter(sv, sp, epdf);
-        EmitterSampleRec er = emitter_sample(sv.emitters[ei], sv.emitter_geom(), pos,
-                                             it.shading_n, sp);
+        const EmitterPick pick = pick_emitter_rec(sv, sp);
+        const auto& nee = pick.e;
+        const float epdf = pick.pdf;
+        EmitterSampleRec er = emitter_sample(nee, sv.emitter_geom(), pos, it.shading_n, sp);
         if (er.pdf > 0.f && !er.radiance.is_zero()) {
             Vec3 to_l = er.pos - pos;
             float dist = to_l.length();
             Vec3 wi = to_l * (1.f / fmaxf(dist, 1e-9f));
             Vec3 f = bsdf_eval(bsdf, -ray.d, wi, it, sv.textures);
             if (!f.is_zero()) {
-                float sh_max = (sv.emitters[ei].type == EM_ENVMAP ? ENVMAP_DIST : dist) - 2.f * EPSILON;
+                float sh_max = (nee.type == EM_ENVMAP ? ENVMAP_DIST : dist) - 2.f * EPSILON;
                 float light_pdf = er.pdf * epdf;
                 float w = er.delta ? 1.f
                                    : mis_weight(light_pdf, bsdf_pdf(bsdf, -ray.d, wi, it, sv.textures));
@@ -310,8 +308,7 @@
             st.L[i] = make_float4(L.x, L.y, L.z, l4.w);
         }
     } else {
-        uint32_t oi = sv.prim_obj[hit.prim_idx] & PRIM_OBJ_MASK;
-        status = (uint32_t)(sv.objs[oi].bsdf_id & 0x3F);
+        status = (uint32_t)(shade_bsdf_id(sv.prim_shade[hit.prim_idx]) & 0x3F);
     }
     st.status[i] = (status << 24) | (uint32_t)i;
 }
@@ -427,8 +424,7 @@
             nh.t = MAX_DIST;
             path_shade_hit(sv, ps, sp, tc, nh);
         } else {
-            uint32_t oi = sv.prim_obj[nh.prim_idx] & PRIM_OBJ_MASK;
-            status = (uint32_t)(sv.objs[oi].bsdf_id & 0x3F);
+            status = (uint32_t)(shade_bsdf_id(sv.prim_shade[nh.prim_idx]) & 0x3F);
         }
         st.hit[i] = make_float4(nh.t, nh.u, nh.v, int_as_float(nh.prim_idx));
     }
@@ -743,4 +739,34 @@
     return e;
 }
 
-}
+__global__ __launch_bounds__(256)
+void k_shade_probe(SceneView sv, const int* __restrict__ prim_idx, int n,
+                   uint32_t* __restrict__ out) {
+    int i = blockIdx.x * blockDim.x + threadIdx.x;
+    if (i >= n) return;
+    int pid = prim_idx[i];
+    if (pid < 0 || pid >= sv.n_prims) return;
+    shade_probe_record(sv, pid, out + (size_t)i * SHADE_PROBE_WORDS);
+}
+
+int shade_probe(const SceneView& sv, const int* prim_idx, int n, uint32_t* out) {
+    if (n <= 0 || sv.n_prims <= 0) return (int)hipErrorInvalidValue;
+    DevBuf<int> d_idx;
+    DevBuf<uint32_t> d_out;
+    int e = 0;
+    e |= d_idx.alloc(n);
+    e |= d_out.alloc((size_t)n * SHADE_PROBE_WORDS);
+    if (e) return e;
+    e |= (int)hipMemcpy(d_idx.p, prim_idx, (size_t)n * 4, hipMemcpyHostToDevice);
+    e |= (int)hipMemset(d_out.p, 0, (size_t)n * SHADE_PROBE_WORDS * 4);
+    if (e) return e;
+    hipLaunchKernelGGL(k_shade_probe, dim3((n + 255) / 256), dim3(256), 0, nullptr,
+                       sv, d_idx.p, n, d_out.p);
+    e |= (int)hipGetLastError();
+    e |= (int)hipDeviceSynchronize();
+    if (e) return e;
+    e |= (int)hipMemcpy(out, d_out.p, (size_t)n * SHADE_PROBE_WORDS * 4, hipMemcpyDeviceToHost);
+    return e;
+}
+
+}
diff --git a/hippt/scene/scene.py b/hippt/scene/scene.py
--- a/hippt/scene/scene.py
+++ b/hippt/scene/scene.py
@@ -349,6 +349,8 @@
                                     prim_base, prim_cnt, inv_area)
         self.native.set_emitter_prims(np.asarray(eprims, np.int32),
                                       np.asarray(ecdf, np.float32))
+        self._np["emitter_prims"] = np.asarray(eprims, np.int32)
+        self._np["emitter_cdf"] = np.asarray(ecdf, np.float32)
 
         if len(d.emitters) > 1 and os.environ.get("HIPPT_LIGHT_POWER") != "0":
             powers = []
@@ -442,6 +444,12 @@
                                                           lds_n, n_cached)
         self.last_trace_plan = tuple(plan)
         return t, prim, u, v, occ.astype(bool)
+
+    def shade_probe(self, prim_idx, device: int = -1):
+        prim_idx = np.ascontiguousarray(prim_idx, np.int32).reshape(-1)
+        if device >= 0 and self._uploaded_device != device:
+            self.upload(device)
+        return tuple(np.asarray(a) for a in self.native.shade_probe(prim_idx, device))
 
     def update_camera(self, pos=None, lookat=None, up=None, fov=None):
         c = self.desc.camera
```

Result: faster. 306.8 Msamples/s (median of 6 runs) (+4.3%).
